# NVlabs/intrinsic3d

Hardware: AMD Instinct MI355X
Metric: Gauss-Newton iterations/s at the finest SDF level (higher is better)
Workload: dtype f32

## Files before the change

intrinsic3d_amd/csrc/device/build.hip:

```cpp
#include <type_traits>
#include "kernels.hpp"
#include "reduce_device.hpp"

namespace i3d {

typedef float v4f_row __attribute__((ext_vector_type(4)));
typedef float v2f_row __attribute__((ext_vector_type(2)));
typedef float f2 __attribute__((ext_vector_type(2)));
static __device__ inline void st_row2(float2* p, float a, float b) { v2f_row v; v.x = a; v.y = b; __builtin_nontemporal_store(v, reinterpret_cast<v2f_row*>(p)); }
static __device__ inline void st_row(float4* p, float a, float b, float c, float d) { v4f_row v; v.x = a; v.y = b; v.z = c; v.w = d; __builtin_nontemporal_store(v, reinterpret_cast<v4f_row*>(p)); }

typedef float f4u __attribute__((ext_vector_type(4), aligned(4)));
typedef const __attribute__((address_space(1))) f4u* gf4u_ptr;
typedef const __attribute__((address_space(1))) float* gf_ptr;

constexpr int Q_LDS_STRIDE = 296;
struct PointShared {
    double P[3];
    double B;
    float n[3];
    float inv_len;
    float s;
    float Ls;
    float dLs[3];
// ... 399 lines not shown
#endif
                float jr[9];
#pragma unroll
                for (int i = 0; i < 9; ++i) jr[i] = fc.Jr[i];
                if (!FR_LDS) __builtin_amdgcn_sched_barrier(0);
                float J[P_TOTAL];
#pragma unroll
                for (int i = 0; i < P_TOTAL; ++i) J[i] = 0.0f;
                float Wx = 0.0f, Wy = 0.0f, Wz = 0.0f;
                const float R0 = (float)Rl[0], R1 = (float)Rl[1], R2 = (float)Rl[2], R3 = (float)Rl[3], R4 = (float)Rl[4], R5 = (float)Rl[5], R6 = (float)Rl[6], R7 = (float)Rl[7], R8 = (float)Rl[8];
#pragma unroll
                for (int jp = 0; jp < 4; jp += 2) {
                    const int ja = jp, jb = jp + 1;
                    const f2 x0 = {pv[ja].x0, pv[jb].x0}, y0 = {pv[ja].y0, pv[jb].y0}, iz = {pv[ja].iz, pv[jb].iz};
                    const f2 dfdc = {pv[ja].dfdc, pv[jb].dfdc}, dfdr = {pv[ja].dfdr, pv[jb].dfdr};
                    const f2 r2 = x0 * x0 + y0 * y0, r4 = r2 * r2, r6 = r4 * r2;
                    const f2 dc = 1.0f + k0 * r2 + k1 * r4 + k2 * r6;
                    const f2 dcr = k0 + 2.0f * k1 * r2 + 3.0f * k2 * r4;
                    const f2 xd = x0 * dc + 2.0f * k3 * x0 * y0 + k4 * (r2 + 2.0f * x0 * x0);
                    const f2 yd = y0 * dc + 2.0f * k4 * xd * y0 + k3 * (r2 + 2.0f * y0 * y0);
                    const f2 dxd_dx0 = dc + 2.0f * x0 * x0 * dcr + 2.0f * k3 * y0 + 6.0f * k4 * x0;
                    const f2 dxd_dy0 = 2.0f * x0 * y0 * dcr + 2.0f * k3 * x0 + 2.0f * k4 * y0;
                    const f2 dyd_dx0 = 2.0f * x0 * y0 * dcr + 2.0f * k4 * y0 * dxd_dx0 + 2.0f * k3 * x0;
                    const f2 dyd_dy0 = dc + 2.0f * y0 * y0 * dcr + 2.0f * k4 * (xd + y0 * dxd_dy0) + 6.0f * k3 * y0;
                    const f2 au = dfdc * fxs, av = dfdr * fys;
                    const f2 lx = au * dxd_dx0 + av * dyd_dx0, ly = au * dxd_dy0 + av * dyd_dy0;
                    const f2 L0 = lx * iz, L1 = ly * iz, L2 = -(lx * x0 + ly * y0) * iz;
                    const f2 M0 = L0 * R0 + L1 * R3 + L2 * R6, M1 = L0 * R1 + L1 * R4 + L2 * R7, M2 = L0 * R2 + L1 * R5 + L2 * R8;
                    const f2 c = {cj[ja], cj[jb]};
                    const f2 alb = {q[ja].alb, q[jb].alb}, sv = {q[ja].s, q[jb].s}, il = {q[ja].inv_len, q[jb].inv_len};
                    const f2 n0 = {q[ja].n[0], q[jb].n[0]}, n1 = {q[ja].n[1], q[jb].n[1]}, n2 = {q[ja].n[2], q[jb].n[2]};
                    const f2 v0 = alb * f2{q[ja].dLs[0], q[jb].dLs[0]} + sv * M0, v1 = alb * f2{q[ja].dLs[1], q[jb].dLs[1]} + sv * M1, v2 = alb * f2{q[ja].dLs[2], q[jb].dLs[2]} + sv * M2;
                    const f2 d = n0 * v0 + n1 * v1 + n2 * v2;
                    f2 G0 = (v0 - n0 * d) * il, G1 = (v1 - n1 * d) * il, G2 = (v2 - n2 * d) * il;
                    if (il.x == 0.0f) { G0.x = v0.x; G1.x = v1.x; G2.x = v2.x; }
                    if (il.y == 0.0f) { G0.y = v0.y; G1.y = v1.y; G2.y = v2.y; }
                    const f2 direct = M0 * n0 + M1 * n1 + M2 * n2;
                    const f2 cG0 = c * G0, cG1 = c * G1, cG2 = c * G2, cD = c * (direct - (G0 + G1 + G2)), cLs = c * f2{q[ja].Ls, q[jb].Ls};
                    J[PS[ja][1]] += cG0.x; J[PS[ja][2]] += cG1.x; J[PS[ja][3]] += cG2.x; J[PS[ja][0]] += cD.x; J[P_ALB + ja] = cLs.x;
                    J[PS[jb][1]] += cG0.y; J[PS[jb][2]] += cG1.y; J[PS[jb][3]] += cG2.y; J[PS[jb][0]] += cD.y; J[P_ALB + jb] = cLs.y;
                    const f2 cL0 = c * L0, cL1 = c * L1, cL2 = c * L2;
                    J[P_POSE + 3] -= cL0.x + cL0.y; J[P_POSE + 4] -= cL1.x + cL1.y; J[P_POSE + 5] -= cL2.x + cL2.y;
                    const f2 Px = {(float)q[ja].P[0], (float)q[jb].P[0]}, Py = {(float)q[ja].P[1], (float)q[jb].P[1]}, Pz = {(float)q[ja].P[2], (float)q[jb].P[2]};
                    const f2 wx = c * (Py * M2 - Pz * M1), wy = c * (Pz * M0 - Px * M2), wz = c * (Px * M1 - Py * M0);
                    Wx += wx.x + wx.y; Wy += wy.x + wy.y; Wz += wz.x + wz.y;
                    const f2 cdc = c * dfdc * psf, cdr = c * dfdr * psf;
                    const f2 i0 = cdc * xd, i1 = cdr * yd;
                    J[P_INTR + 0] -= i0.x + i0.y; J[P_INTR + 1] -= i1.x + i1.y; J[P_INTR + 2] -= cdc.x + cdc.y; J[P_INTR + 3] -= cdr.x + cdr.y;
                    const f2 dxk0 = x0 * r2, dxk1 = x0 * r4, dxk2 = x0 * r6, dxk3 = 2.0f * x0 * y0, dxk4 = r2 + 2.0f * x0 * x0;
                    const f2 c2 = 2.0f * k4 * y0;
                    const f2 e0 = c * (au * dxk0 + av * (y0 * r2 + c2 * dxk0)), e1 = c * (au * dxk1 + av * (y0 * r4 + c2 * dxk1)), e2 = c * (au * dxk2 + av * (y0 * r6 + c2 * dxk2));
                    const f2 e3 = c * (au * dxk3 + av * (c2 * dxk3 + (r2 + 2.0f * y0 * y0))), e4 = c * (au * dxk4 + av * (2.0f * xd * y0 + c2 * dxk4));
                    J[P_DIST + 0] -= e0.x + e0.y; J[P_DIST + 1] -= e1.x + e1.y; J[P_DIST + 2] -= e2.x + e2.y; J[P_DIST + 3] -= e3.x + e3.y; J[P_DIST + 4] -= e4.x + e4.y;
                }
                J[P_POSE + 0] = -(Wx * jr[0] + Wy * jr[3] + Wz * jr[6]);
                J[P_POSE + 1] = -(Wx * jr[1] + Wy * jr[4] + Wz * jr[7]);
                J[P_POSE + 2] = -(Wx * jr[2] + Wy * jr[5] + Wz * jr[8]);
                float finz = 0.0f;
#pragma unroll
                for (int i = 0; i < P_TOTAL; ++i) finz = __builtin_fmaf(J[i], 0.0f, finz);
                if (!(finz == 0.0f)) continue;
#pragma unroll
                for (int gq = 0; gq < 7; ++gq)
                    st_row(&r.rows[row_index(a, nout, gq, r.slots)], J[4 * gq], J[4 * gq + 1], J[4 * gq + 2], J[4 * gq + 3]);
                const size_t ro = row_scalar_index(a, nout, r.slots);
                st_row2(&r.row_jt()[row_jt_index(a, nout, r.slots)], J[28], __int_as_float(f | (vox_free ? ROW_FREE_BIT : 0)));
                st_row2(&r.row_wr[ro], roww, (float)res);
                ++nout;
            }
            }
        }
        if (WITH_J) {
            r.nrows[a] = (uint8_t)nout;
        }
        }
    }
#ifdef I3D_COST_MULTI_PROBE
    if (!WITH_J && probe_extra) cost = 0.0;
#endif
    if (!WITH_J) block_partial_d(cost, cost_out, 1, 0);
}

void launch_build(hipStream_t st, GridView g, RowView r, OptParams p, const FrameConst* frames, bool with_jacobian, double* cost_out, double* scratch,
                  const double* cam9, const LmState* lm) {
    if (r.nC <= 0) { if (!with_jacobian && cost_out) (void)hipMemsetAsync(cost_out, 0, sizeof(double), st); return; }
#ifdef I3D_COST_MULTI_PROBE
    const int blocks = with_jacobian ? (r.nC + 255) / 256 : (((r.nC + 255) / 256 + 7) / 8) * 8 * I3D_COST_MULTI_PROBE;
#else
    const int blocks = (r.nC + 255) / 256;
#endif
    double* const cost_dst = cost_out; cost_out = scratch;
    const size_t lds = (size_t)p.K * sizeof(FrameHot), qlds = (size_t)256 * Q_LDS_STRIDE;
    if (with_jacobian) {
#ifdef I3D_BUILD_VALUE_PROBE
        if (BUILD_PROBE_WAVES > 2) {
            if (!set_dynamic_lds((const void*)k_build<true, true, 2>, "k_build<true> value probe", lds, p.K)) return;
            k_build<true, true, 2><<<blocks, 256, lds, st>>>(g, r, p, frames, cost_out, nullptr, nullptr);
            return;
        }
#endif
        if (!set_dynamic_lds((const void*)k_build<true, false, 2>, "k_build<true>", qlds, p.K)) return;
        k_build<true, false, 2><<<blocks, 256, qlds, st>>>(g, r, p, frames, cost_out, nullptr, nullptr);
    } else {
        if (lds <= 48 * 1024) k_build<false, true, 2><<<blocks, 256, lds, st>>>(g, r, p, frames, cost_out, cam9, lm);
        else k_build<false, false, 2><<<blocks, 256, 0, st>>>(g, r, p, frames, cost_out, cam9, lm);
    }
    if (!with_jacobian) launch_reduce_partials(st, scratch, blocks, 1, cost_dst, nullptr, true);
}

template <bool COST>
__global__ void __launch_bounds__(256) k_weight_sums(RowView r, GridView g, double* partials) {
    double s0 = 0, s1 = 0, s2 = 0, s3 = 0, n0 = 0, n3 = 0, na = 0, c0 = 0, c1 = 0, c2 = 0, c3 = 0;
    const int N = g.N;
    for (int a = r.own0 + blockIdx.x * blockDim.x + threadIdx.x; a < r.own1 && a < r.A; a += gridDim.x * blockDim.x) {
        if (!(r.aflags[a] & F_ACTIVE)) continue;
        na += 1.0;
        const int nr = r.nrows[a];
        for (int k = 0; k < nr; ++k) {
            const float2 wr = r.row_wr[row_scalar_index(a, k, r.slots)]; const float w = wr.x;
            s0 += (double)w; if (w != 0.0f) n0 += 1.0;
            if (COST && (__float_as_int(r.row_jt()[row_jt_index(a, k, r.slots)].y) & ROW_FREE_BIT)) c0 += (double)w * ((double)wr.y * (double)wr.y);
        }
        const uint8_t rf = r.regflags[a];
        if (rf & 1) s1 += 1.0;
        if (rf & 2) s2 += 1.0;
        const int s = COST ? r.alist[a] : 0;
        const uint8_t eafree = COST ? r.ea_free[a] : 0;
        const bool er = COST && (rf & 1) && (rf & 8), es = COST && (rf & 2) && (rf & 16);
        int ring[6];
        if (er || eafree) {
#pragma unroll
            for (int d = 0; d < 6; ++d) ring[d] = g.nbr[(size_t)d * N + s];
        }
        if (er || es) {
            const double xs = g.x_sdf[s];
            if (er) {
                const double dxx = g.x_sdf[ring[0]] + g.x_sdf[ring[1]] - 2.0 * xs, dyy = g.x_sdf[ring[2]] + g.x_sdf[ring[3]] - 2.0 * xs, dzz = g.x_sdf[ring[4]] + g.x_sdf[ring[5]] - 2.0 * xs;
                const double lap = dxx + dyy + dzz; c1 += lap * lap;
            }
            if (es) { double e = xs - g.sdf0[s]; if (e == 0.0) e = 0.0000001; c2 += e * e; }
        }
        const double xa = eafree ? g.x_alb[s] : 0.0;
#pragma unroll
        for (int d = 0; d < 6; ++d) {
            const float w = r.ea_w[(size_t)d * r.Acap + a]; s3 += (double)w; if (w != 0.0f) n3 += 1.0;
            if (eafree & (1 << d)) { const double e = xa - g.x_alb[ring[d]]; c3 += (double)w * (e * e); }
        }
    }
    block_partial_d(s0, partials, 13, 0); block_partial_d(s1, partials, 13, 1); block_partial_d(s2, partials, 13, 2); block_partial_d(s3, partials, 13, 3);
    block_partial_d(n0, partials, 13, 4); block_partial_d(0.0, partials, 13, 5); block_partial_d(0.0, partials, 13, 6); block_partial_d(n3, partials, 13, 7);
    block_partial_d(na, partials, 13, 8);
    block_partial_d(c0, partials, 13, 9); block_partial_d(c1, partials, 13, 10); block_partial_d(c2, partials, 13, 11); block_partial_d(c3, partials, 13, 12);
}
void launch_weight_sums(hipStream_t st, RowView r, GridView g, bool with_cost, double* sums13, double* scratch) {
    const int n = r.own1 - r.own0;
    if (n <= 0) return;
    int blocks = (n + 255) / 256; if (blocks > 1024) blocks = 1024;
    if (with_cost) k_weight_sums<true><<<blocks, 256, 0, st>>>(r, g, scratch);
    else k_weight_sums<false><<<blocks, 256, 0, st>>>(r, g, scratch);
    launch_reduce_partials(st, scratch, blocks, 13, sums13, nullptr);
}

}
```

intrinsic3d_amd/csrc/device/gradcol.hip:

```cpp
#include "kernels.hpp"
#include "reduce_device.hpp"
#include "wave_ops.hpp"

namespace i3d {

constexpr int GC_THREADS = 384, GC_NW = GC_THREADS / 64, GC_TC = 16, GC_NPV = 27, GC_NCAM = 34;
constexpr int GC_D_CAMW = 4, GC_D_TAG = GC_D_CAMW + ((GC_NW * (GC_NCAM + 0) + 3) & ~3), GC_D_VAL = GC_D_TAG + GC_NW * GC_TC, GC_D0 = GC_D_VAL + GC_NW * GC_TC * GC_NPV;

__device__ constexpr int8_t GC_TRI_I[21] = {0, 0, 0, 0, 0, 0, 1, 1, 1, 1, 1, 2, 2, 2, 2, 3, 3, 3, 4, 4, 5};
__device__ constexpr int8_t GC_TRI_J[21] = {0, 1, 2, 3, 4, 5, 1, 2, 3, 4, 5, 2, 3, 4, 5, 3, 4, 5, 4, 5, 5};

#ifndef GC_OCC
#define GC_OCC 2
#endif
__global__ void __launch_bounds__(GC_THREADS, GC_OCC) k_eg_gradcol(GridView g, RowView r, OptParams p, GradColBuffers b, int tiles_per_block) {
    extern __shared__ float lds[];
    const int K = p.K; const size_t Acap = r.Acap;
    const int rs = (GC_NPV * K) | 1;
    const int nacc = GC_D0 + rs + GC_NCAM;
    for (int i = threadIdx.x; i < nacc; i += GC_THREADS) lds[i] = (i >= GC_D_TAG && i < GC_D_VAL) ? __int_as_float(-1) : 0.0f;
    __syncthreads();
    const int wave = __builtin_amdgcn_readfirstlane((int)(threadIdx.x >> 6));
    const int o_tag = GC_D_TAG + wave * GC_TC, o_val = GC_D_VAL + wave * (GC_TC * GC_NPV);
    int tcount = 0;
// ... 71 lines not shown
            wave_table_add_quads<GC_NPV, GC_TC, 3>(live && owned, fsel, [&](int q) {
                return q < 6 ? (free_poses ? J[P_POSE + (q < 6 ? q : 0)] * t : 0.0f) : tw0 * J[P_POSE + GC_TRI_I[q < 6 ? 0 : q - 6]] * J[P_POSE + GC_TRI_J[q < 6 ? 0 : q - 6]];
            }, lds, o_tag, o_val, tcount, GC_D0, GC_NPV);
        }
        __syncthreads();
        for (int w = 0; w < GC_NW; ++w) { if (wave == w) wave_table_merge<GC_NPV, GC_TC>(lds, o_tag, o_val, tcount, GC_D0, GC_NPV); __syncthreads(); }
        if (in) {
#pragma unroll
            for (int c = 0; c < P_VOX; ++c) { b.Cg[(size_t)c * Acap + a] = accg[c]; b.Cc[(size_t)c * Acap + a] = accc[c]; }
            const int s = r.alist[a];
            const int N = g.N;
            const bool act = (fl & F_ACTIVE) != 0;
            const uint8_t rf_ld = r.regflags[a], eaf_ld = r.ea_free[a];
            float eaw[6]; int rg[6];
#pragma unroll
            for (int d = 0; d < 6; ++d) { eaw[d] = r.ea_w[(size_t)d * Acap + a]; rg[d] = g.nbr[(size_t)d * N + s]; }
            const double xs = g.x_sdf[s], xa = g.x_alb[s], s0 = g.sdf0[s];
            double xsn[6], xan[6];
#pragma unroll
            for (int d = 0; d < 6; ++d) { const int nb = rg[d] >= 0 ? rg[d] : s; xsn[d] = g.x_sdf[nb]; xan[d] = g.x_alb[nb]; }
            const uint8_t rf = act ? rf_ld : 0;
            float trg = 0.0f, tsg = 0.0f, trc = 0.0f, tsc = 0.0f;
            const uint8_t eafree = (owned && act) ? eaf_ld : 0;
            if (rf & 1) {
                const float rho = (float)p.type_w[1];
                const double dxx = xsn[0] + xsn[1] - 2.0 * xs, dyy = xsn[2] + xsn[3] - 2.0 * xs, dzz = xsn[4] + xsn[5] - 2.0 * xs;
                const double lap = dxx + dyy + dzz;
                trg = rho * (float)lap; trc = rho;
                if (owned && (rf & 8)) cost += 0.5 * p.type_w[1] * lap * lap;
            }
            if (rf & 2) {
                const double e0 = xs - s0;
                if (rf & 4) { const float rho = (float)p.type_w[2]; tsg = rho * (float)e0; tsc = rho; }
                if (owned && (rf & 16)) { const double e = e0 == 0.0 ? 0.0000001 : e0; cost += 0.5 * p.type_w[2] * e * e; }
            }
            b.tregg[a] = trg; b.tregg[Acap + a] = tsg; b.tregc[a] = trc; b.tregc[Acap + a] = tsc;
#pragma unroll
            for (int d = 0; d < 6; ++d) {
                const float w = act ? eaw[d] : 0.0f;
                float tag = 0.0f, tac = 0.0f;
                if (w != 0.0f) {
                    const float rho = w * (float)p.type_w[3]; const double e = xa - xan[d];
                    tag = rho * (float)e; tac = rho;
                    if (eafree & (1 << d)) cost += 0.5 * (double)w * p.type_w[3] * e * e;
                }
                b.tregg[(size_t)(2 + d) * Acap + a] = tag; b.tregc[(size_t)(2 + d) * Acap + a] = tac;
            }
        }
    }
    block_partial_d(cost, b.cost_partials, 1, 0);
#pragma unroll
    for (int i = 0; i < GC_NCAM; ++i) {
        float v = i < 9 ? cam9[i] : camb[i - 9];
        for (int o = 32; o > 0; o >>= 1) v += __shfl_down(v, o, 64);
        if ((threadIdx.x & 63) == 0) lds[GC_D_CAMW + wave * GC_NCAM + i] = v;
    }
    __syncthreads();
    if (threadIdx.x < GC_NCAM) { float v = 0.0f; for (int w = 0; w < GC_NW; ++w) v += lds[GC_D_CAMW + w * GC_NCAM + threadIdx.x]; cam_acc[threadIdx.x] = v; }
    __syncthreads();
    float* const rowg = b.part + (size_t)blockIdx.x * b.part_stride;
    float* const rowc = rowg + b.col_off;
    for (int i = threadIdx.x; i < 6 * K; i += GC_THREADS) { const int f = i / 6; rowg[i] = lds[GC_D0 + GC_NPV * f + (i - 6 * f)]; }
    for (int i = threadIdx.x; i < 21 * K; i += GC_THREADS) { const int f = i / 21; rowc[i] = lds[GC_D0 + GC_NPV * f + 6 + (i - 21 * f)]; }
    if (threadIdx.x < 9) rowg[6 * K + threadIdx.x] = cam_acc[threadIdx.x];
    if (threadIdx.x < 34) {
        const int i = threadIdx.x;
        constexpr int8_t DIAG[9] = {0, 4, 7, 9, 10, 15, 19, 22, 24};
        rowc[21 * K + i] = i < 9 ? cam_acc[9 + DIAG[i]] : cam_acc[i];
    }
}

int launch_eg_gradcol(hipStream_t st, GridView g, RowView r, OptParams p, GradColBuffers b) {
    if (r.nC <= 0) return 0;
    static int num_cu = 0;
    if (!num_cu) { int dev = 0; (void)hipGetDevice(&dev); hipDeviceProp_t pr; (void)hipGetDeviceProperties(&pr, dev); num_cu = pr.multiProcessorCount > 0 ? pr.multiProcessorCount : 256; }
    const int ntiles = (r.nC + GC_THREADS - 1) / GC_THREADS;
    const int want = 2 * num_cu;
    const int blocks = ntiles < want ? ntiles : want;
    const int tiles_per_block = (ntiles + blocks - 1) / blocks;
    const size_t n = (size_t)(GC_D0 + ((GC_NPV * p.K) | 1) + GC_NCAM) * sizeof(float);
    if (!set_dynamic_lds((const void*)k_eg_gradcol, "k_eg_gradcol", n, p.K)) return 0;
    const int used = (ntiles + tiles_per_block - 1) / tiles_per_block;
    k_eg_gradcol<<<used, GC_THREADS, n, st>>>(g, r, p, b, tiles_per_block);
    launch_reduce_partials(st, b.cost_partials, used, 1, b.cost_out, nullptr);
    return used;
}

}
```

intrinsic3d_amd/csrc/device/kernels.hpp:

```cpp
#pragma once
#include "common.hpp"
#include "p2p_device.hpp"

namespace i3d {

struct HashTable { unsigned long long* keys; int* vals; unsigned int mask; };
void launch_sort_keys(hipStream_t st, int N, const int* keys_xyz , unsigned long long* sort_keys, int* iota);
void launch_permute_grid(hipStream_t st, int N, const int* perm, const int* keys_xyz, const double* sdf, const double* sdf_ref,
                         const double* alb, const float* w, const uint8_t* rgb,
                         int* cx, int* cy, int* cz, int* rank, double* sdf0, double* x_sdf, double* x_alb, float* f_sdf, float* f_alb,
                         float* weight, uchar4* color);
void launch_hash_build(hipStream_t st, int N, const int* cx, const int* cy, const int* cz, HashTable t);
void launch_nbr_build(hipStream_t st, int N, const int* cx, const int* cy, const int* cz, HashTable t, int* nbr);
void launch_classify(hipStream_t st, GridView g, OptParams p, int* active_flag);
void launch_compact(hipStream_t st, int N, const int* active_flag, const int* active_scan, const uint8_t* flags, int* aidx, int* alist, uint8_t* aflags);
void launch_partition_blocks(hipStream_t st, GridView g, int A, int* alist, uint8_t* aflags, int* aidx);
void launch_group_rows(hipStream_t st, int A, const uint8_t* nrows, int* gmax);
void launch_anbr(hipStream_t st, int N, int A, int Acap, const int* alist, const int* nbr, const int* aidx, int* anbr);
void launch_scatter_sh(hipStream_t st, int N, const int* rank, const double* sh_visit , float* sh );
void launch_gather_visit(hipStream_t st, int N, const int* rank, const double* x_sdf, const double* x_alb, double* out_sdf, double* out_alb);
void launch_update_fields(hipStream_t st, int N, const int* rank, const double* sdf_ref, const double* alb, const uint8_t* rgb,
                          double* x_sdf, double* x_alb, float* f_sdf, float* f_alb, uchar4* color);

void launch_observe(hipStream_t st, GridView g, RowView r, OptParams p, const FrameConst* frames, const unsigned* cull_mask = nullptr, bool prefilter = false);
constexpr int CULL_BLOCK = 8, CULL_MAX_LEVELS = 12;
struct CullPyramid { int levels, cells; int bw[CULL_MAX_LEVELS], bh[CULL_MAX_LEVELS], off[CULL_MAX_LEVELS]; };
CullPyramid cull_pyramid(int w, int h);
void launch_depth_blocks(hipStream_t st, const FrameConst* frames, int K, int w, int h, float2* out);
void launch_group_cull(hipStream_t st, GridView g, RowView r, OptParams p, const FrameConst* frames, const float2* dblocks, float4* bounds, unsigned* mask);

void launch_build(hipStream_t st, GridView g, RowView r, OptParams p, const FrameConst* frames, bool with_jacobian, double* cost_out , double* scratch,
                  const double* cam9 = nullptr, const LmState* lm = nullptr);
void launch_weight_sums(hipStream_t st, RowView r, GridView g, bool with_cost, double* sums13 , double* scratch);

enum PassMode { PASS_GRAD = 0, PASS_JTJP = 1, PASS_COLNORM = 2 };
struct Seg2 { size_t off0, off1; int n; };
struct PassBuffers {
    float* C;
    float* treg;
    double* shared;
    double* blocks;
    float* part; int part_stride;
};
struct GradColBuffers {
    float* Cg; float* Cc;
    float* tregg; float* tregc;
    float* part; int part_stride;
    int col_off;
    double* cost_partials; double* cost_out;
};
int  launch_eg_gradcol(hipStream_t st, GridView g, RowView r, OptParams p, GradColBuffers b);
int  launch_eg_pass(hipStream_t st, PassMode mode, GridView g, RowView r, OptParams p, const float* u , PassBuffers b, const PcgState* state);
void launch_sum_rows(hipStream_t st, PassMode mode, int K, const float* part, int nrows, int stride, double* shared, double* blocks);
void launch_gather(hipStream_t st, PassMode mode, RowView r, PassBuffers b, float* out );
int  launch_gather_tail(hipStream_t st, RowView r, PassBuffers b, float* out, const float* S, const float* D2, const float* v, double* dot_partials ,
                        bool dot_atomic, const PcgState* state);
void launch_reduce_partials(hipStream_t st, const double* partials, int nblk, int ncomp, double* dst, const PcgState* state, bool assign = false);
void launch_shared_finalize(hipStream_t st, size_t tail_off, int K, OptParams p, const double* shared, float* out , bool tail, const float* S, const float* D2,
                            const float* v, double* dot_out, const PcgState* state);

void launch_fill(hipStream_t st, int n, float* x, float v);
void launch_fill_d(hipStream_t st, int n, double* x, double v);
void launch_int_to_double(hipStream_t st, const int* src, double* dst);
void launch_mul(hipStream_t st, int n, const float* a, const float* b, float* out);
void launch_scale_from_colnorm(hipStream_t st, int n, const float* c, const float* freemask, float* S, float* cm);
void launch_dot(hipStream_t st, int n, const float* a, const float* b, double* out , double* scratch);
void launch_count_above2(hipStream_t st, Seg2 sg, const float* a, const float* m, float tol, double* out, double* scratch);
void launch_count_above(hipStream_t st, int n, const float* a, const float* m, float tol, double* out, double* scratch);
void launch_dot2(hipStream_t st, Seg2 sg, const float* a, const float* b, double* out , double* scratch);
void launch_mul2(hipStream_t st, Seg2 sg, const float* a, const float* b, float* out);
void launch_freemask(hipStream_t st, RowView r, OptParams p, float* mask );

void launch_pcg_init(hipStream_t st, PcgState* state, int fixed_iterations, int max_iterations, const LmState* lm = nullptr);
int  launch_pcg_step(hipStream_t st, int mode, Seg2 sg, const float* p, const float* q, float* x, float* r, const float* b, const float* D2, const float* Minv,
                     float* z, const float* S_for_inline_q, double* partials , PcgState* state);
void launch_pcg_tail_x(hipStream_t st, size_t tail_off, int K, const float* p, float* x, const PcgState* state);
void launch_pcg_tail_a(hipStream_t st, int mode, size_t tail_off, int K, const float* Minv_blocks, const float* p, const float* q, float* x, float* r, const float* b,
                       const float* D2, float* z, const double* partials, int nblk, PcgState* state,
                       double* shared_zero, int nzero, int* host_flags, int seq,
                       const P2PDev& pd);
int  launch_pcg_direction(hipStream_t st, Seg2 sg, size_t tail_off, int ntail, const float* z, float* p, const float* S, float* u, const float* D2,
                          double* d2_partials , const PcgState* state);
void launch_pcg_tail_b(hipStream_t st, size_t tail_off, int K, OptParams p, double* shared, const double* pq_slice, const double* pq_partials, int nblk,
                       const double* pq_partials2, int nblk2, bool rowwise,
                       float* q, const float* S, const float* D2, const float* v, PcgState* state, const P2PDev& pd);
struct TilePlan {
    unsigned* lnbr;
    float* eaw_sym;
    int* halo_idx; int* halo_cnt;
    int* iota; int* ext_e; int* ext_pos;
    float* qh;
    int* ext_off;
    int* overflow;
    int T, hmax;
    int tile_first, ntiles_own;
    const int* ghost_tiles; int n_ghost;
    int det;
    const unsigned short* hp_off;
    const unsigned short* hp_src;
    int pull;
};
inline int tile_plan_pull_cap(int hmax) { return 4 * hmax; }
inline int tile_plan_hmax_of(int T) { return T == 1024 ? 2048 : 1536; }
inline int tile_plan_tiles_of(int A, int T) { return (A + T - 1) / T; }
size_t tile_plan_temp_bytes(size_t nslots);
hipError_t launch_tile_plan(hipStream_t st, RowView r, TilePlan t, int hmax_limit , void* temp, size_t temp_bytes);
void launch_eaw_sym(hipStream_t st, RowView r, TilePlan t, const int* cflag );
int  launch_eg_tile(hipStream_t st, RowView r, OptParams p, const float* u, TilePlan t, double* shared, float* qacc, double* pq_partials ,
                    const PcgState* state, float* cam_partials = nullptr, int cam_stride = 0);
void launch_ext_offsets(hipStream_t st, int n, const int* ext_e, int A, int* ext_off);
void eg_tile_launch_shape(const TilePlan& t, int K, int& blocks, int& tiles_per_block);

struct LadVec;
int  eg_tile_mr_max_systems(int K);
int  launch_eg_tile_mr(hipStream_t st, RowView r, OptParams p, TilePlan t, int nsys, const int* sys, const float* u0, float* qacc0, float* qh0, double* pq0 , float* cam0, int cam_stride,
                       const PcgState* st0 , const LadVec& lv);
int  launch_eg_tile_mr_pair(hipStream_t st, RowView r, OptParams p, TilePlan t, int na, int nb, const int* sys, const float* u0, float* qacc0, float* qh0, double* pq0 , float* cam0,
                            int cam_stride, const PcgState* st0, const LadVec& lv);

struct ShardArgs {
    P2PDev pd; RimLists rim; int seq;
    int n_slice_partials;
    int n_rim_wg;
    const float* zb; float* pb; float* ub; const float* cmb; int chunk;
};
struct LadVec {
    size_t vec;
    size_t qh;
    size_t cam;
    size_t part;
    size_t mblk;
    size_t tail;
    int sysid[LADDER_MAX];
};
struct Step3Args {
    int nq; int chunk4;
    const float4* p; const float4* qacc; float4* x; float4* r; const float4* b; float4* z;
    const float4* cm; const LmState* lm;
    const int* ext_off; const int* ext_pos; const float2* qh; int e0;
    const double* pq_partials; int n_pq; const double* d2_partials; int n_d2;
    int n_slice_wg;
    int K; int fix_poses, fix_intr, fix_dist;
    const float* cam_partials; int n_cam; int cam_stride; const float* Mblk;
    const float* tp; float* tx; float* tr; const float* tb; const float* tD2; float* tz; const float* tS;
    double* step_partials;
    PcgState* cur;
    int sharded; ShardArgs sh;
    int lad_sys;
    const double* redop; int redop_stride;
};
void launch_pcg_init3(hipStream_t st, PcgState* st2 , int fixed_iterations, int max_iterations, const LmState* lm = nullptr);
int  launch_pcg_dir3(hipStream_t st, bool init, Seg2 sg, size_t tail_off, int ntail, const float* z, float* p, const float* S, float* u, const float* D2, const float* cm, const LmState* lm,
                     const double* step_partials, int n_step, double* d2_partials, const PcgState* prev, PcgState* next, int* host_flags, int seq,
                     const ShardArgs* sa = nullptr);
void launch_rim_u(hipStream_t st, const ShardArgs& sa, const PcgState* state);
int  pcg_step3_slice_wgs(int n_entries, int cap = 0);
int  pcg_step3_tail_wgs(int K);
int  launch_pcg_step3(hipStream_t st, int mode , Step3Args a);
void launch_halo_fold(hipStream_t st, RowView r, TilePlan t, float* qacc, const PcgState* state);
void launch_pcg_init_lad(hipStream_t st, PcgState* st2_all , int B, int fixed_iterations, int max_iterations, const LmState* lm);
int  launch_pcg_dir3_lad(hipStream_t st, bool init, int nsys, Seg2 sg, size_t tail_off, int ntail, const float* z0, float* p0, const float* S, float* u0, const float* tD2_0, const float* cm, const LmState* lm,
                         const double* step_partials0, int n_step, double* d2_partials0, PcgState* st2_0, int prev_parity, int* host_flags0, int seq, const LadVec& lv,
                         int n_slice_partials = 0, const double* red4_0 = nullptr );
int  launch_pcg_step3_lad(hipStream_t st, int mode, int nsys, Step3Args a, const LadVec& lv);
void launch_lad_reduce_step(hipStream_t st, int nsys, const double* step_partials0, int n_slice, double* red4_0, const LadVec& lv);
void launch_lad_reduce_op(hipStream_t st, int nsys, const float* cam_partials0, int n_cam, int cam_stride, int NS, const double* pq_partials0, int n_pq, const double* d2_partials0, int n_d2,
                          double* redop0, int redop_stride, const LadVec& lv);

void launch_need_mask(hipStream_t st, RowView r, int slice, unsigned long long* need );
void launch_halo_items(hipStream_t st, int A, int slice, int me, const unsigned long long* need, unsigned long long* items, int* count , int cap);
void launch_tile_flags(hipStream_t st, int A, int T, const int* cflag, int* tileflag );
size_t halo_sort_temp_bytes(int cap);
hipError_t launch_halo_sort(hipStream_t st, void* temp, size_t temp_bytes, const unsigned long long* in, unsigned long long* out, int n);

void launch_candidate(hipStream_t st, GridView g, RowView r, int K, float sign, const float* step, const float* S, const double* x_shared, double* xc_sdf, double* xc_alb,
                      double* xc_shared, double* norms2 , const float* mask, double* scratch, const LmState* lm = nullptr);
void launch_accept(hipStream_t st, GridView g, RowView r, const double* xc_sdf, const double* xc_alb, const LmState* lm = nullptr);
void launch_set_double(hipStream_t st, double* dst, double v);
void launch_lm_init(hipStream_t st, LmState* lm, const double* cost, const double* ngrad, const double* nfree, double radius0, LmRecord* rec, int seq);
void launch_lm_begin(hipStream_t st, LmState* lm, int K, int fix_poses, int fix_intr, int fix_dist, const double* cdiag, const double* tri, float* Mblk,
                     const float* tc, const float* tS, float* tD2, float* tMinv, LmRecord* rec, int seq);
void launch_lm_diag_dev(hipStream_t st, int n, const float* c, const float* S, const LmState* lm, float* D2, float* Minv);
void launch_cand_frames(hipStream_t st, int K, const double* xc, const FrameConst* base, FrameConst* out, const LmState* lm);
void launch_lm_decide(hipStream_t st, LmState* lm, const PcgState* ps, const double* norms2, const double* cand_cost, int attempt, int lm_steps, LmRecord* rec, int seq,
                      int lad_next = -1 , int debug_invalid = 0);
void launch_lm_begin_lad(hipStream_t st, LmState* lm, int B, int K, int fix_poses, int fix_intr, int fix_dist, const double* cdiag, const double* tri, float* Mblk, size_t mblk_stride,
                         const float* tc, const float* tS, float* tD2, size_t tail_stride, LmRecord* rec, int seq);
void launch_mark_compute(hipStream_t st, RowView r, int* flag);
void launch_compact_list(hipStream_t st, int A, const int* flag, const int* scan, int* list);

}
```

intrinsic3d_amd/csrc/device/lm_kernels.hip:

```cpp
#include "kernels.hpp"
#include "frame_math.hpp"

namespace i3d {

static __device__ inline void lm_publish(LmRecord* rec, int seq) {
    if (rec) __hip_atomic_store(&rec->seq, seq, __ATOMIC_RELEASE, __HIP_MEMORY_SCOPE_SYSTEM);
}

__global__ void k_lm_init(LmState* lm, const double* __restrict__ cost, const double* __restrict__ ngrad, const double* __restrict__ nfree, double radius0, LmRecord* rec, int seq) {
    LmState s;
    s.cost = *cost; s.radius = radius0; s.decrease_factor = 2.0; s.ngrad = *ngrad; s.nfree = *nfree;
    s.inv_radius = (float)(1.0 / radius0); s.pad0 = 0;
    s.done = 0; s.termination = 0; s.accepted = 0; s.invalid = 0; s.attempts = 0; s.successful = 0;
    if (s.nfree == 0.0 || s.ngrad == 0.0) { s.done = 1; s.termination = 1; }
    *lm = s;
    if (rec) {
        rec->final_ = s.done; rec->accepted = 0; rec->pcg_it = 0; rec->termination = s.termination; rec->kind = 0;
        rec->cost = s.cost; rec->cand_cost = 0.0; rec->model_change = 0.0; rec->rel = 0.0; rec->radius_after = s.radius; rec->ngrad = s.ngrad; rec->nfree = s.nfree;
        lm_publish(rec, seq);
    }
}
__global__ void k_set_double(double* dst, double v) { *dst = v; }
void launch_set_double(hipStream_t st, double* dst, double v) { k_set_double<<<1, 1, 0, st>>>(dst, v); }
void launch_lm_init(hipStream_t st, LmState* lm, const double* cost, const double* ngrad, const double* nfree, double radius0, LmRecord* rec, int seq) {
    k_lm_init<<<1, 1, 0, st>>>(lm, cost, ngrad, nfree, radius0, rec, seq);
}

static __device__ inline bool spd_invert_dev(int n, const double* m, double* inv) {
    double L[36];
    for (int i = 0; i < n; ++i) for (int j = 0; j <= i; ++j) {
        double s = m[i * n + j];
        for (int k = 0; k < j; ++k) s -= L[i * n + k] * L[j * n + k];
        if (i == j) { if (!(s > 0.0)) return false; L[i * n + i] = sqrt(s); } else L[i * n + j] = s / L[j * n + j];
    }
    for (int col = 0; col < n; ++col) {
        double y[6], x[6];
        for (int i = 0; i < n; ++i) { double s = (i == col) ? 1.0 : 0.0; for (int k = 0; k < i; ++k) s -= L[i * n + k] * y[k]; y[i] = s / L[i * n + i]; }
        for (int i = n - 1; i >= 0; --i) { double s = y[i]; for (int k = i + 1; k < n; ++k) s -= L[k * n + i] * x[k]; x[i] = s / L[i * n + i]; }
        for (int i = 0; i < n; ++i) inv[i * n + col] = x[i];
    }
    return true;
}
static __device__ inline void cam_block_inverse(int n, const double* __restrict__ cdiag, const double* __restrict__ tri, bool fixed, double radius, float* __restrict__ out) {
    if (fixed) { for (int i = 0; i < n * n; ++i) out[i] = 0.0f; return; }
    double S[6], M[36], inv[36];
    for (int i = 0; i < n; ++i) S[i] = 1.0 / (1.0 + sqrt(cdiag[i]));
    int o = 0;
    for (int i = 0; i < n; ++i) for (int j = i; j < n; ++j) { const double v = S[i] * S[j] * tri[o++]; M[i * n + j] = v; M[j * n + i] = v; }
    for (int i = 0; i < n; ++i) { const double cs = cdiag[i] * S[i] * S[i]; M[i * n + i] += fmin(fmax(cs, 1e-6), 1e32) / radius; }
    if (!spd_invert_dev(n, M, inv)) { for (int i = 0; i < n * n; ++i) inv[i] = 0.0; for (int i = 0; i < n; ++i) inv[i * n + i] = 1.0 / M[i * n + i]; }
    for (int i = 0; i < n * n; ++i) out[i] = (float)inv[i];
}

__global__ void __launch_bounds__(64) k_lm_begin(LmState* lm, int K, int fix_poses, int fix_intr, int fix_dist, const double* __restrict__ cdiag , const double* __restrict__ tri ,
                                                 float* __restrict__ Mblk , const float* __restrict__ tc, const float* __restrict__ tS, float* __restrict__ tD2, float* __restrict__ tMinv ,
                                                 LmRecord* rec, int seq) {
    if (lm->done) return;
    const double radius = lm->radius;
    const int gid = blockIdx.x * blockDim.x + threadIdx.x;
    if (radius < 1e-32) {
        if (gid == 0) {
            lm->termination = 1; lm->done = 1;
            if (rec) { rec->final_ = 1; rec->accepted = 0; rec->pcg_it = 0; rec->termination = 1; rec->kind = 2; rec->cost = lm->cost; rec->cand_cost = 0.0; rec->model_change = 0.0; rec->rel = 0.0;
                       rec->radius_after = radius; rec->ngrad = lm->ngrad; rec->nfree = lm->nfree; lm_publish(rec, seq); }
        }
        return;
    }
    const float inv_radius = (float)(1.0 / radius);
    if (gid == 0) lm->inv_radius = inv_radius;
    if (gid < K) cam_block_inverse(6, cdiag + 6 * gid, tri + 21 * gid, fix_poses != 0, radius, Mblk + 36 * (size_t)gid);
    else if (gid == K) cam_block_inverse(4, cdiag + 6 * K, tri + 21 * K, fix_intr != 0, radius, Mblk + 36 * (size_t)K);
    else if (gid == K + 1) cam_block_inverse(5, cdiag + 6 * K + 4, tri + 21 * K + 10, fix_dist != 0, radius, Mblk + 36 * (size_t)K + 16);
    const int NS = 6 * K + 9;
    for (int i = gid; i < NS; i += gridDim.x * blockDim.x) { float d2, mi; lm_diag(tc[i], tS[i], inv_radius, d2, mi); tD2[i] = d2; tMinv[i] = mi; }
}
void launch_lm_begin(hipStream_t st, LmState* lm, int K, int fix_poses, int fix_intr, int fix_dist, const double* cdiag, const double* tri, float* Mblk,
                     const float* tc, const float* tS, float* tD2, float* tMinv, LmRecord* rec, int seq) {
    k_lm_begin<<<(K + 2 + 63) / 64, 64, 0, st>>>(lm, K, fix_poses, fix_intr, fix_dist, cdiag, tri, Mblk, tc, tS, tD2, tMinv, rec, seq);
}

__global__ void __launch_bounds__(64) k_lm_begin_lad(LmState* lm, int B, int K, int fix_poses, int fix_intr, int fix_dist, const double* __restrict__ cdiag, const double* __restrict__ tri,
                                                     float* __restrict__ Mblk, size_t mblk_stride, const float* __restrict__ tc, const float* __restrict__ tS, float* __restrict__ tD2, size_t tail_stride,
                                                     LmRecord* rec, int seq) {
    if (lm->done == 1) return;
    const int j = blockIdx.y, gid = blockIdx.x * blockDim.x + threadIdx.x;
    double radius = lm->radius, dec = lm->decrease_factor;
    if (j == 0 && radius < 1e-32) {
        if (gid == 0) {
            lm->termination = 1; lm->done = 1; lm->lad_n = 0;
            if (rec) { rec->final_ = 1; rec->accepted = 0; rec->pcg_it = 0; rec->termination = 1; rec->kind = 2; rec->cost = lm->cost; rec->cand_cost = 0.0; rec->model_change = 0.0; rec->rel = 0.0;
                       rec->radius_after = radius; rec->ngrad = lm->ngrad; rec->nfree = lm->nfree; lm_publish(rec, seq); }
        }
        return;
    }
    for (int s = 0; s < j; ++s) { radius = radius / dec; dec *= 2.0; }
    const bool dead = radius < 1e-32;
    const float inv_radius = dead ? 0.0f : (float)(1.0 / radius);
    if (gid == 0) { lm->lad_radius[j] = radius; lm->lad_inv_radius[j] = inv_radius; if (j == 0) { lm->lad_n = B; lm->inv_radius = inv_radius; lm->done = 0; } }
    if (dead) return;
    float* const Mb = Mblk + (size_t)j * mblk_stride;
    if (gid < K) cam_block_inverse(6, cdiag + 6 * gid, tri + 21 * gid, fix_poses != 0, radius, Mb + 36 * (size_t)gid);
    else if (gid == K) cam_block_inverse(4, cdiag + 6 * K, tri + 21 * K, fix_intr != 0, radius, Mb + 36 * (size_t)K);
    else if (gid == K + 1) cam_block_inverse(5, cdiag + 6 * K + 4, tri + 21 * K + 10, fix_dist != 0, radius, Mb + 36 * (size_t)K + 16);
    const int NS = 6 * K + 9;
    for (int i = gid; i < NS; i += gridDim.x * blockDim.x) { float d2, mi; lm_diag(tc[i], tS[i], inv_radius, d2, mi); tD2[(size_t)j * tail_stride + i] = d2; }
}
void launch_lm_begin_lad(hipStream_t st, LmState* lm, int B, int K, int fix_poses, int fix_intr, int fix_dist, const double* cdiag, const double* tri, float* Mblk, size_t mblk_stride,
                         const float* tc, const float* tS, float* tD2, size_t tail_stride, LmRecord* rec, int seq) {
    k_lm_begin_lad<<<dim3((K + 2 + 63) / 64, B), 64, 0, st>>>(lm, B, K, fix_poses, fix_intr, fix_dist, cdiag, tri, Mblk, mblk_stride, tc, tS, tD2, tail_stride, rec, seq);
}

__global__ void k_lm_diag_dev(int n, const float* __restrict__ c, const float* __restrict__ S, const LmState* __restrict__ lm, float* __restrict__ D2, float* __restrict__ Minv) {
    if (lm->done) return;
    const float ir = lm->inv_radius;
    for (int i = blockIdx.x * blockDim.x + threadIdx.x; i < n; i += gridDim.x * blockDim.x) { float d2, mi; lm_diag(c[i], S[i], ir, d2, mi); D2[i] = d2; Minv[i] = mi; }
}
void launch_lm_diag_dev(hipStream_t st, int n, const float* c, const float* S, const LmState* lm, float* D2, float* Minv) {
    if (n <= 0) return;
    int b = (n + 255) / 256; b = b > 2048 ? 2048 : b;
    k_lm_diag_dev<<<b, 256, 0, st>>>(n, c, S, lm, D2, Minv);
}

__global__ void __launch_bounds__(64) k_cand_frames(int K, const double* __restrict__ xc, const FrameConst* __restrict__ base, FrameConst* __restrict__ out, const LmState* __restrict__ lm) {
    if (lm->done) return;
    const int f = blockIdx.x * blockDim.x + threadIdx.x;
    if (f >= K) return;
    FrameConst fc = base[f];
    double p[6];
    for (int i = 0; i < 6; ++i) p[i] = xc[6 * f + i];
    fm::frame_from_pose(p, fc);
    out[f] = fc;
}
void launch_cand_frames(hipStream_t st, int K, const double* xc, const FrameConst* base, FrameConst* out, const LmState* lm) {
    if (K > 0) k_cand_frames<<<(K + 63) / 64, 64, 0, st>>>(K, xc, base, out, lm);
}

__global__ void k_lm_decide(LmState* lm, const PcgState* __restrict__ ps, const double* __restrict__ norms2, const double* __restrict__ cand_cost_p, int attempt , int lm_steps,
                            LmRecord* rec, int seq, int lad_next, int debug_invalid) {
    if (lm->done) return;
    const int pcg_it = ps->done == 2 ? ps->it + 1 : ps->it;
    const double xbr = ps->xbr, d2xx = ps->d2xx;
    const double model_change = 0.5 * xbr + 0.5 * d2xx;
    const bool finite = !(isnan(xbr) || isinf(xbr) || isnan(d2xx) || isinf(d2xx));
    double radius = lm->radius, decrease = lm->decrease_factor, cost = lm->cost;
    const double cand = *cand_cost_p;
    int final_ = 0, accepted = 0, termination = lm->termination, invalid = lm->invalid, successful = lm->successful;
    double rel = 0.0;
    if (!finite || !(model_change > 0.0) || debug_invalid) {
        if (++invalid >= 5) { termination = 3; final_ = 1; }
        else radius *= 0.5;
    } else {
        invalid = 0;
        const double step_norm = sqrt(norms2[0]), x_norm = sqrt(norms2[1]);
        const double cost_change = cost - cand;
        if (step_norm <= 1e-8 * (x_norm + 1e-8)) { termination = 1; final_ = 1; }
        else if (fabs(cost_change) <= 1e-6 * cost) { termination = 1; final_ = 1; }
        else {
            rel = cost_change / model_change;
            if (rel > 1e-3) {
                accepted = 1; cost = cand;
                radius = fmin(1e16, radius / fmax(1.0 / 3.0, 1.0 - pow(2.0 * rel - 1.0, 3.0)));
                decrease = 2.0;
                successful += 1; termination = 2; final_ = 1;
            } else { radius = radius / decrease; decrease *= 2.0; }
        }
    }
    if (!final_ && attempt + 1 >= lm_steps) final_ = 1;
    lm->radius = radius; lm->decrease_factor = decrease; lm->cost = cost; lm->invalid = invalid; lm->successful = successful; lm->termination = termination;
    lm->attempts = lm->attempts + 1; lm->accepted = accepted; lm->done = final_;
    if (rec) {
        rec->final_ = final_; rec->accepted = accepted; rec->pcg_it = pcg_it; rec->termination = termination; rec->kind = 1;
        rec->cost = cost; rec->cand_cost = cand; rec->model_change = model_change; rec->rel = rel; rec->radius_after = radius; rec->ngrad = lm->ngrad; rec->nfree = lm->nfree;
        lm_publish(rec, seq);
    }
    if (!final_ && lad_next >= 0 && lad_next < lm->lad_n) {
        LmRecord* const nrec = rec ? rec + 1 : nullptr;
        if (radius != lm->lad_radius[lad_next]) {
            lm->done = 2;
            if (nrec) { nrec->final_ = 0; nrec->accepted = 0; nrec->pcg_it = 0; nrec->termination = termination; nrec->kind = 3; nrec->cost = cost; nrec->cand_cost = 0.0; nrec->model_change = 0.0;
                        nrec->rel = 0.0; nrec->radius_after = radius; nrec->ngrad = lm->ngrad; nrec->nfree = lm->nfree; lm_publish(nrec, seq + 1); }
        } else if (radius < 1e-32) {
            lm->termination = 1; lm->done = 1;
            if (nrec) { nrec->final_ = 1; nrec->accepted = 0; nrec->pcg_it = 0; nrec->termination = 1; nrec->kind = 2; nrec->cost = cost; nrec->cand_cost = 0.0; nrec->model_change = 0.0;
                        nrec->rel = 0.0; nrec->radius_after = radius; nrec->ngrad = lm->ngrad; nrec->nfree = lm->nfree; lm_publish(nrec, seq + 1); }
        }
    }
}
void launch_lm_decide(hipStream_t st, LmState* lm, const PcgState* ps, const double* norms2, const double* cand_cost, int attempt, int lm_steps, LmRecord* rec, int seq, int lad_next, int debug_invalid) {
    k_lm_decide<<<1, 1, 0, st>>>(lm, ps, norms2, cand_cost, attempt, lm_steps, rec, seq, lad_next, debug_invalid);
}

}
```

intrinsic3d_amd/csrc/device/operator.hip:

```cpp
#include "kernels.hpp"
#include "reduce_device.hpp"
#include "wave_ops.hpp"

namespace i3d {

#define GRID_STRIDE(n) const int stride = gridDim.x * blockDim.x; for (int i = blockIdx.x * blockDim.x + threadIdx.x; i < (n); i += stride)
static inline int vblocks(int n) { int b = (n + 255) / 256; return b < 1 ? 1 : (b > 2048 ? 2048 : b); }

__global__ void __launch_bounds__(1024) k_reduce_partials(const double* __restrict__ partials, int nblk, int ncomp, double* dst, const PcgState* __restrict__ state, int assign) {
    if (state && state->done) return;
    for (int k = 0; k < ncomp; ++k) {
        double s = 0.0;
        for (int i0 = threadIdx.x; i0 < nblk; i0 += 8 * 1024) {
            double v[8];
#pragma unroll
            for (int q = 0; q < 8; ++q) v[q] = partials[(size_t)min(i0 + q * 1024, nblk - 1) * ncomp + k];
#pragma unroll
            for (int q = 0; q < 8; ++q) if (i0 + q * 1024 < nblk) s += v[q];
        }
        const double t = block_sum_d(s);
        if (threadIdx.x == 0) dst[k] = assign ? t : dst[k] + t;
    }
}
void launch_reduce_partials(hipStream_t st, const double* partials, int nblk, int ncomp, double* dst, const PcgState* state, bool assign) {
    if (nblk > 0) k_reduce_partials<<<1, 1024, 0, st>>>(partials, nblk, ncomp, dst, state, assign ? 1 : 0);
}

constexpr int EG_THREADS = 1024;

template <int MODE>
__global__ void __launch_bounds__(EG_THREADS) k_eg_pass(GridView g, RowView r, OptParams p, PassBuffers b, int tiles_per_block, const PcgState* __restrict__ state) {
    static_assert(MODE == PASS_GRAD || MODE == PASS_COLNORM, "the operator pass has its own kernel");
    if (state && state->done) return;
    extern __shared__ float lds[];
    const int K = p.K; const size_t Acap = r.Acap;
    constexpr int NPVT = (MODE == PASS_COLNORM) ? 21 : 6, TCT = (MODE == PASS_COLNORM) ? 16 : 32, NWT = EG_THREADS / 64;
    const int rs = ((MODE == PASS_COLNORM) ? 21 * K : 6 * K) | 1;
    constexpr int NCAM = (MODE == PASS_COLNORM) ? 34 : 9;
    constexpr int D_CAMW = 4, D_TAG = D_CAMW + ((NWT * NCAM + 3) & ~3), D_VAL = D_TAG + NWT * TCT, D0 = D_VAL + NWT * TCT * NPVT;
    const int nacc = D0 + rs + NCAM;
    for (int i = threadIdx.x; i < nacc; i += EG_THREADS) lds[i] = (i >= D_TAG && i < D_VAL) ? __int_as_float(-1) : 0.0f;
    __syncthreads();
    const int wave = __builtin_amdgcn_readfirstlane((int)(threadIdx.x >> 6));
    const int o_tag = D_TAG + wave * TCT, o_val = D_VAL + wave * (TCT * NPVT);
    int tcount = 0;
    float* const cam_acc = lds + D0 + rs;
    float cam9[9];
#pragma unroll
    for (int i = 0; i < 9; ++i) cam9[i] = 0.0f;
    float camb[NCAM];
#pragma unroll
    for (int i = 0; i < NCAM; ++i) camb[i] = 0.0f;
    const float tw0 = (float)p.type_w[0];
    const int nC = r.nC;
    const int ntiles = (nC + EG_THREADS - 1) / EG_THREADS;
    const int tile0 = blockIdx.x * tiles_per_block;

    for (int tile = tile0; tile < tile0 + tiles_per_block && tile < ntiles; ++tile) {
        const int ci = tile * EG_THREADS + threadIdx.x;
        const bool in = ci < nC;
        const int a = in ? (r.clist ? r.clist[ci] : ci) : 0;
        const bool owned = in && a >= r.own0 && a < r.own1;
        const uint8_t fl = in ? r.aflags[a] : 0;
        const int nr = (in && (fl & F_ACTIVE)) ? (int)r.nrows[a] : 0;
        int nr_max = nr;
        for (int o = 32; o > 0; o >>= 1) nr_max = max(nr_max, __shfl_xor(nr_max, o, 64));

        float acc[P_VOX];
#pragma unroll
        for (int c = 0; c < P_VOX; ++c) acc[c] = 0.0f;
        const size_t ac = in ? (size_t)a : 0;
        for (int k = 0; k < nr_max; ++k) {
            const float4* __restrict__ row = r.rows + row_index(ac, k, 0, r.slots);
            float4 j4[7];
#pragma unroll
            for (int q = 0; q < 7; ++q) j4[q] = ld_row(row + q * 64);
            const size_t ro = row_scalar_index(ac, k, r.slots);
            const float2 jt = r.row_jt()[row_jt_index(ac, k, r.slots)];
            constexpr int NPV = (MODE == PASS_COLNORM) ? 21 : 6;
            float pv[NPV]; int fsel = 0; bool pvalid = false;
#pragma unroll
            for (int i = 0; i < NPV; ++i) pv[i] = 0.0f;
            if (k < nr) {
                const float rho = tw0;
                const int f = __float_as_int(jt.y) & ~ROW_FREE_BIT;
                float J[P_TOTAL];
#pragma unroll
                for (int q = 0; q < 7; ++q) { J[4 * q] = j4[q].x; J[4 * q + 1] = j4[q].y; J[4 * q + 2] = j4[q].z; J[4 * q + 3] = j4[q].w; }
                J[28] = jt.x;
                if (MODE == PASS_COLNORM) {
#pragma unroll
                    for (int c = 0; c < P_VOX; ++c) acc[c] += rho * J[c] * J[c];
                  if (owned) {
                    int o = 0;
#pragma unroll
                    for (int i = 0; i < 6; ++i) {
#pragma unroll
                        for (int j = i; j < 6; ++j) { pv[o] = rho * J[P_POSE + i] * J[P_POSE + j]; ++o; }
                    }
                    fsel = f; pvalid = true;
#pragma unroll
                    for (int i = 0; i < 9; ++i) camb[i] += rho * J[P_INTR + i] * J[P_INTR + i];
                    o = 9;
#pragma unroll
                    for (int i = 0; i < 4; ++i) {
#pragma unroll
                        for (int j = i; j < 4; ++j) { camb[o] += rho * J[P_INTR + i] * J[P_INTR + j]; ++o; }
                    }
#pragma unroll
                    for (int i = 0; i < 5; ++i) {
#pragma unroll
                        for (int j = i; j < 5; ++j) { camb[o] += rho * J[P_DIST + i] * J[P_DIST + j]; ++o; }
                    }
                  }
                } else {
                    const float2 wr = r.row_wr[ro]; const float t = rho * (sqrtf(wr.x) * wr.y);
#pragma unroll
                    for (int c = 0; c < P_VOX; ++c) acc[c] += J[c] * t;
                    if (!p.fix_poses && owned) {
#pragma unroll
                        for (int i = 0; i < 6; ++i) pv[i] = J[P_POSE + i] * t;
                        fsel = f; pvalid = true;
                    }
                    if (owned) {
#pragma unroll
                        for (int i = 0; i < 9; ++i) cam9[i] += J[P_INTR + i] * t;
                    }
                }
            }
            wave_table_add_quads<NPV, TCT, (MODE == PASS_COLNORM ? 2 : 3)>(pvalid, fsel, [&](int q) { return pv[q]; }, lds, o_tag, o_val, tcount, D0, NPV);
        }
        __syncthreads();
        for (int w = 0; w < NWT; ++w) { if (wave == w) wave_table_merge<NPVT, TCT>(lds, o_tag, o_val, tcount, D0, NPVT); __syncthreads(); }
        if (in) {
#pragma unroll
            for (int c = 0; c < P_VOX; ++c) b.C[(size_t)c * Acap + a] = acc[c];
            const uint8_t rf = (fl & F_ACTIVE) ? r.regflags[a] : 0;
            float tr = 0.0f, ts = 0.0f;
            const int s = r.alist[a];
            const int N = g.N;
            if (rf & 1) {
                const float rho = (float)p.type_w[1];
                if (MODE == PASS_COLNORM) tr = rho;
                else {
                    const double xs = g.x_sdf[s];
                    double nbv[6];
#pragma unroll
                    for (int d = 0; d < 6; ++d) nbv[d] = g.x_sdf[g.nbr[(size_t)d * N + s]];
                    const double dxx = nbv[0] + nbv[1] - 2.0 * xs, dyy = nbv[2] + nbv[3] - 2.0 * xs, dzz = nbv[4] + nbv[5] - 2.0 * xs;
                    tr = rho * (float)(dxx + dyy + dzz);
                }
            }
            if ((rf & 2) && (rf & 4)) {
                const float rho = (float)p.type_w[2];
                if (MODE == PASS_COLNORM) ts = rho;
                else ts = rho * (float)(g.x_sdf[s] - g.sdf0[s]);
            }
            b.treg[a] = tr; b.treg[Acap + a] = ts;
#pragma unroll
            for (int d = 0; d < 6; ++d) {
                const float w = (fl & F_ACTIVE) ? r.ea_w[(size_t)d * Acap + a] : 0.0f;
                float ta = 0.0f;
                if (w != 0.0f) {
                    const float rho = w * (float)p.type_w[3];
                    if (MODE == PASS_COLNORM) ta = rho;
                    else ta = rho * (float)(g.x_alb[s] - g.x_alb[g.nbr[(size_t)d * N + s]]);
                }
                b.treg[(size_t)(2 + d) * Acap + a] = ta;
            }
        }
    }
#pragma unroll
    for (int i = 0; i < NCAM; ++i) {
        float v = (MODE == PASS_COLNORM) ? camb[i] : cam9[i];
        for (int o = 32; o > 0; o >>= 1) v += __shfl_down(v, o, 64);
        if ((threadIdx.x & 63) == 0) lds[D_CAMW + wave * NCAM + i] = v;
    }
    __syncthreads();
    if (threadIdx.x < NCAM) { float v = 0.0f; for (int w = 0; w < NWT; ++w) v += lds[D_CAMW + w * NCAM + threadIdx.x]; cam_acc[threadIdx.x] = v; }
    __syncthreads();
    const int npose = (MODE == PASS_COLNORM) ? 21 * K : 6 * K;
    float* const row = b.part + (size_t)blockIdx.x * b.part_stride;
    for (int i = threadIdx.x; i < npose + NCAM; i += EG_THREADS) row[i] = i < npose ? lds[D0 + i] : cam_acc[i - npose];
}

__global__ void __launch_bounds__(256) k_sum_rows(int mode, int K, const float* __restrict__ part, int nrows, int stride, double* __restrict__ shared, double* __restrict__ blocks) {
    __shared__ double grp[8][33];
    const int col = threadIdx.x & 31, rg = threadIdx.x >> 5;
    const int i = blockIdx.x * 32 + col;
    const int ncol = mode == PASS_COLNORM ? 21 * K + 34 : 6 * K + 9;
    double v = 0.0;
    if (i < ncol) for (int w = rg; w < nrows; w += 8) v += (double)part[(size_t)w * stride + i];
    grp[rg][col] = v;
    __syncthreads();
    if (rg != 0 || i >= ncol) return;
    v = grp[0][col];
    for (int q = 1; q < 8; ++q) v += grp[q][col];
    if (mode != PASS_COLNORM) { shared[i] = v; return; }
    if (i < 21 * K) {
        blocks[i] = v;
        const int f = i / 21, o = i - 21 * f;
        const int di = o == 0 ? 0 : o == 6 ? 1 : o == 11 ? 2 : o == 15 ? 3 : o == 18 ? 4 : o == 20 ? 5 : -1;
        if (di >= 0) shared[6 * f + di] = v;
    } else { const int c = i - 21 * K; if (c < 9) shared[6 * K + c] = v; else blocks[21 * K + (c - 9)] = v; }
}
void launch_sum_rows(hipStream_t st, PassMode mode, int K, const float* part, int nrows, int stride, double* shared, double* blocks) {
    const int ncol = mode == PASS_COLNORM ? 21 * K + 34 : 6 * K + 9;
    k_sum_rows<<<(ncol + 31) / 32, 256, 0, st>>>((int)mode, K, part, nrows, stride, shared, blocks);
}

__global__ void __launch_bounds__(EG_THREADS) k_eg_jtjp(GridView g, RowView r, OptParams p, const float* __restrict__ u, PassBuffers b,
                                                        int reps, int tiles_per_block, const PcgState* __restrict__ state) {
    if (state && state->done) return;
    extern __shared__ float lds[];
    const int K = p.K; const size_t Acap = r.Acap;
    const int nshared = 6 * K + 9;
    const int rs = (6 * K) | 1;
    const int nacc = reps * rs + 9;
    for (int i = threadIdx.x; i < nacc; i += EG_THREADS) lds[i] = 0.0f;
    float* const upose = lds + nacc;
    float* const uvl = upose + nshared + threadIdx.x;
    const size_t tail = 2 * (size_t)r.chunk;
    const int chunk = r.chunk;
    for (int i = threadIdx.x; i < nshared; i += EG_THREADS) upose[i] = u[tail + i];
    __syncthreads();
    float* const cam_acc = lds + reps * rs;
    float* const pose_acc = lds + (threadIdx.x & (reps - 1)) * rs;
    float* const wave_acc = lds + ((threadIdx.x >> 6) & (reps - 1)) * rs;
    float cam9[9];
#pragma unroll
    for (int i = 0; i < 9; ++i) cam9[i] = 0.0f;
    const float tw0 = (float)p.type_w[0];
    const int nC = r.nC;
    const int ntiles = (nC + EG_THREADS - 1) / EG_THREADS;
    const int tile0 = blockIdx.x * tiles_per_block;
    const float* const ui = upose + 6 * K;

    for (int tile = tile0; tile < tile0 + tiles_per_block && tile < ntiles; ++tile) {
        const int ci = tile * EG_THREADS + threadIdx.x;
        const bool in = ci < nC;
        const int a = in ? (r.clist ? r.clist[ci] : ci) : 0;
        const bool owned = in && a >= r.own0 && a < r.own1;
        const uint8_t fl = in ? r.aflags[a] : 0;
        const int nr = (in && (fl & F_ACTIVE)) ? (int)r.nrows[a] : 0;
        int nr_max = nr;
        for (int o = 32; o > 0; o >>= 1) nr_max = max(nr_max, __shfl_xor(nr_max, o, 64));
        const size_t ac = in ? (size_t)a : 0;
        float4 rwA[8], rwB[8];
        auto load_block = [&](float4 (&rw)[8], int k) {
            const float4* __restrict__ row = r.rows + row_index(ac, k, 0, r.slots);
#pragma unroll
            for (int q = 0; q < 7; ++q) rw[q] = ld_row(row + q * 64);
            { const float2 jt = r.row_jt()[row_jt_index(ac, k, r.slots)]; rw[7].x = jt.x; rw[7].y = jt.y; }
        };
        if (nr_max > 0) load_block(rwA, 0);
        if (in) {
#pragma unroll
            for (int c = 0; c < P_VOX; ++c) {
                const int nb = slot_fwd_nbr(c);
                const int la = nb < 0 ? a : r.anbr[(size_t)nb * Acap + a];
                uvl[c * EG_THREADS] = la >= 0 ? u[c < 10 ? vec_sdf(la, chunk) : vec_alb(la, chunk)] : 0.0f;
            }
        }
        if (nr_max > 1) load_block(rwB, 1);
        if (in) {
            const uint8_t rf = (fl & F_ACTIVE) ? r.regflags[a] : 0;
            const float us = uvl[0], ua = uvl[10 * EG_THREADS];
            float rs_[6], ra_[6];
            rs_[0] = uvl[6 * EG_THREADS]; rs_[2] = uvl[1 * EG_THREADS]; rs_[4] = uvl[4 * EG_THREADS];
            ra_[0] = uvl[11 * EG_THREADS]; ra_[2] = uvl[12 * EG_THREADS]; ra_[4] = uvl[13 * EG_THREADS];
#pragma unroll
            for (int q = 1; q < 6; q += 2) {
                const int la = (rf || (fl & F_ACTIVE)) ? r.anbr[(size_t)q * Acap + a] : -1;
                rs_[q] = la >= 0 ? u[vec_sdf(la, chunk)] : 0.0f; ra_[q] = la >= 0 ? u[vec_alb(la, chunk)] : 0.0f;
            }
            float tr = 0.0f, ts = 0.0f;
            if (rf & 1) tr = (float)p.type_w[1] * (((((((-6.0f * us) + rs_[0]) + rs_[1]) + rs_[2]) + rs_[3]) + rs_[4]) + rs_[5]);
            if ((rf & 2) && (rf & 4)) ts = (float)p.type_w[2] * us;
            b.treg[a] = tr; b.treg[Acap + a] = ts;
#pragma unroll
            for (int d = 0; d < 6; ++d) {
                const float w = (fl & F_ACTIVE) ? r.ea_w[(size_t)d * Acap + a] : 0.0f;
                b.treg[(size_t)(2 + d) * Acap + a] = (w != 0.0f) ? w * (float)p.type_w[3] * (ua - ra_[d]) : 0.0f;
            }
        }
        float acc[P_VOX];
#pragma unroll
        for (int c = 0; c < P_VOX; ++c) acc[c] = 0.0f;

        auto consume = [&](const float4 (&rw)[8], int k) {
            float pv[6]; int fsel = 0; bool pvalid = false;
// ... 138 lines not shown
                for (int d = 0; d < 6; ++d) if (ringa[d] >= 0) acc += SQUARED ? tn[d] : -tn[d];
                oalb = acc;
            }
        }
        const int js = vec_sdf(a, r.chunk), ja = js + r.chunk;
        if (TAIL) {
            const float v0 = v[js], v1 = v[ja];
            osdf = S[js] * osdf + D2[js] * v0; oalb = S[ja] * oalb + D2[ja] * v1;
            dotp = (double)v0 * (double)osdf + (double)v1 * (double)oalb;
        }
        out[js] = osdf; out[ja] = oalb;
    }
    if (TAIL && dot_out) {
        if (!dot_atomic) block_partial_d(dotp, dot_out, 1, 0);
        else { const double t = block_sum_d(dotp); if (threadIdx.x == 0 && t != 0.0) atomicAdd(dot_out, t); }
    }
}
void launch_gather(hipStream_t st, PassMode mode, RowView r, PassBuffers b, float* out) {
    const int n = (r.own1 < r.A ? r.own1 : r.A) - r.own0;
    if (n <= 0) return;
    const int blocks = (n + 255) / 256;
    if (mode == PASS_COLNORM) k_gather<true, false><<<blocks, 256, 0, st>>>(r, b, out, nullptr, nullptr, nullptr, nullptr, 0, nullptr);
    else k_gather<false, false><<<blocks, 256, 0, st>>>(r, b, out, nullptr, nullptr, nullptr, nullptr, 0, nullptr);
}
int launch_gather_tail(hipStream_t st, RowView r, PassBuffers b, float* out, const float* S, const float* D2, const float* v, double* dot_partials, bool dot_atomic,
                       const PcgState* state) {
    const int n = (r.own1 < r.A ? r.own1 : r.A) - r.own0;
    if (n <= 0) return 0;
    const int blocks = (n + 255) / 256;
    k_gather<false, true><<<blocks, 256, 0, st>>>(r, b, out, S, D2, v, dot_partials, dot_atomic ? 1 : 0, state);
    return blocks;
}

__global__ void k_shared_finalize(size_t tail_off, int K, OptParams p, const double* __restrict__ shared, float* __restrict__ out, int tail,
                                  const float* __restrict__ S, const float* __restrict__ D2, const float* __restrict__ v, double* dot_out,
                                  const PcgState* __restrict__ state) {
    if (state && state->done) return;
    const int i = blockIdx.x * blockDim.x + threadIdx.x;
    double dotp = 0.0;
    if (i < 6 * K + 9) {
        const bool fixed = i < 6 * K ? p.fix_poses : (i < 6 * K + 4 ? p.fix_intr : p.fix_dist);
        float o = fixed ? 0.0f : (float)shared[i];
        const size_t j = tail_off + i;
        if (tail) { const float vv = v[j]; o = S[j] * o + D2[j] * vv; dotp = (double)vv * (double)o; }
        out[j] = o;
    }
    if (tail && dot_out) { const double t = block_sum_d(dotp); if (threadIdx.x == 0 && t != 0.0) atomicAdd(dot_out, t); }
}
void launch_shared_finalize(hipStream_t st, size_t tail_off, int K, OptParams p, const double* shared, float* out, bool tail, const float* S, const float* D2,
                            const float* v, double* dot_out, const PcgState* state) {
    k_shared_finalize<<<(6 * K + 9 + 255) / 256, 256, 0, st>>>(tail_off, K, p, shared, out, tail ? 1 : 0, S, D2, v, dot_out, state);
}

__global__ void k_fill(int n, float* x, float v) { GRID_STRIDE(n) x[i] = v; }
__global__ void k_fill_d(int n, double* x, double v) { GRID_STRIDE(n) x[i] = v; }
__global__ void k_mul(int n, const float* a, const float* b, float* o) { GRID_STRIDE(n) o[i] = a[i] * b[i]; }
__global__ void k_mul2(int n, size_t seg, const float* a, const float* b, float* o) { GRID_STRIDE(2 * n) { const size_t j = i < n ? (size_t)i : (size_t)(i - n) + seg; o[j] = a[j] * b[j]; } }
__global__ void k_scale(int n, const float* c, const float* m, float* S, float* cm) { GRID_STRIDE(n) { const float v = m[i] != 0.0f ? c[i] : -1.0f; cm[i] = v; S[i] = lm_scale(v); } }
__global__ void __launch_bounds__(256) k_dot(int n, const float* a, const float* b, double* out) {
    double s = 0.0; GRID_STRIDE(n) s += (double)a[i] * (double)b[i];
    block_partial_d(s, out, 1, 0);
}
__global__ void __launch_bounds__(256) k_dot2(int n, size_t seg, const float* a, const float* b, double* out) {
    double s = 0.0; GRID_STRIDE(2 * n) { const size_t j = i < n ? (size_t)i : (size_t)(i - n) + seg; s += (double)a[j] * (double)b[j]; }
    block_partial_d(s, out, 1, 0);
}
__global__ void __launch_bounds__(256) k_count_above(int n, const float* a, const float* m, float tol, double* out) {
    double s = 0.0; GRID_STRIDE(n) s += (fabsf(a[i] * m[i]) > tol) ? 1.0 : 0.0;
    block_partial_d(s, out, 1, 0);
}
__global__ void __launch_bounds__(256) k_count_above2(int n, size_t seg, const float* a, const float* m, float tol, double* out) {
    double s = 0.0; GRID_STRIDE(2 * n) { const size_t j = i < n ? (size_t)i : (size_t)(i - n) + seg; s += (fabsf(a[j] * m[j]) > tol) ? 1.0 : 0.0; }
    block_partial_d(s, out, 1, 0);
}
void launch_fill(hipStream_t st, int n, float* x, float v) { if (n > 0) k_fill<<<vblocks(n), 256, 0, st>>>(n, x, v); }
void launch_fill_d(hipStream_t st, int n, double* x, double v) { if (n > 0) k_fill_d<<<vblocks(n), 256, 0, st>>>(n, x, v); }
__global__ void k_int_to_double(const int* src, double* dst) { *dst = (double)*src; }
void launch_int_to_double(hipStream_t st, const int* src, double* dst) { k_int_to_double<<<1, 1, 0, st>>>(src, dst); }
void launch_mul(hipStream_t st, int n, const float* a, const float* b, float* o) { if (n > 0) k_mul<<<vblocks(n), 256, 0, st>>>(n, a, b, o); }
void launch_mul2(hipStream_t st, Seg2 sg, const float* a, const float* b, float* o) {
    if (sg.n > 0) k_mul2<<<vblocks(2 * sg.n), 256, 0, st>>>(sg.n, sg.off1 - sg.off0, a + sg.off0, b + sg.off0, o + sg.off0);
}
void launch_scale_from_colnorm(hipStream_t st, int n, const float* c, const float* m, float* S, float* cm) { if (n > 0) k_scale<<<vblocks(n), 256, 0, st>>>(n, c, m, S, cm); }
void launch_dot2(hipStream_t st, Seg2 sg, const float* a, const float* b, double* out, double* scratch) {
    if (sg.n <= 0) return;
    const int blocks = vblocks(2 * sg.n) > 1024 ? 1024 : vblocks(2 * sg.n);
    k_dot2<<<blocks, 256, 0, st>>>(sg.n, sg.off1 - sg.off0, a + sg.off0, b + sg.off0, scratch);
    launch_reduce_partials(st, scratch, blocks, 1, out, nullptr);
}
void launch_count_above2(hipStream_t st, Seg2 sg, const float* a, const float* m, float tol, double* out, double* scratch) {
    if (sg.n <= 0) return;
    const int blocks = vblocks(2 * sg.n) > 1024 ? 1024 : vblocks(2 * sg.n);
    k_count_above2<<<blocks, 256, 0, st>>>(sg.n, sg.off1 - sg.off0, a + sg.off0, m + sg.off0, tol, scratch);
    launch_reduce_partials(st, scratch, blocks, 1, out, nullptr);
}
void launch_count_above(hipStream_t st, int n, const float* a, const float* m, float tol, double* out, double* scratch) {
    if (n <= 0) return;
    const int blocks = vblocks(n) > 1024 ? 1024 : vblocks(n);
    k_count_above<<<blocks, 256, 0, st>>>(n, a, m, tol, scratch);
    launch_reduce_partials(st, scratch, blocks, 1, out, nullptr);
}
void launch_dot(hipStream_t st, int n, const float* a, const float* b, double* out, double* scratch) {
    if (n <= 0) return;
    const int blocks = vblocks(n) > 1024 ? 1024 : vblocks(n);
    k_dot<<<blocks, 256, 0, st>>>(n, a, b, scratch);
    launch_reduce_partials(st, scratch, blocks, 1, out, nullptr);
}

__global__ void k_freemask(RowView r, OptParams p, float* __restrict__ mask) {
    const int A = r.A, chunk = r.chunk, nv = 2 * chunk, NP = nv + 6 * p.K + 9;
    GRID_STRIDE(NP) {
        float m;
        if (i < nv) {
            const int a = i < chunk ? i : i - chunk;
            m = (a < A && (r.aflags[a] & (i < chunk ? F_FREE_SDF : F_FREE_ALB))) ? 1.0f : 0.0f;
        }
        else if (i < nv + 6 * p.K) m = p.fix_poses ? 0.0f : 1.0f;
        else if (i < nv + 6 * p.K + 4) m = p.fix_intr ? 0.0f : 1.0f;
        else m = p.fix_dist ? 0.0f : 1.0f;
        mask[i] = m;
    }
}
void launch_freemask(hipStream_t st, RowView r, OptParams p, float* mask) { k_freemask<<<vblocks(2 * r.chunk + 6 * p.K + 9), 256, 0, st>>>(r, p, mask); }

enum { STEP_INIT = 0, STEP_NORMAL = 1, STEP_XONLY = 2, STEP_RESET = 3 };

template <int MODE, bool QINLINE>
__global__ void __launch_bounds__(256) k_pcg_step(int n4, int seg4 , const float4* __restrict__ p, const float4* __restrict__ q, float4* __restrict__ x, float4* __restrict__ r,
                                                  const float4* __restrict__ b, const float4* __restrict__ D2, const float4* __restrict__ Minv, float4* __restrict__ z,
                                                  const float4* __restrict__ S, double* __restrict__ partials , PcgState* state) {
    if (state->done) return;
    const float alpha = (float)state->alpha;
    double s0 = 0.0, s1 = 0.0, s2 = 0.0, s3 = 0.0;
    for (int j = blockIdx.x * blockDim.x + threadIdx.x; j < 2 * n4; j += gridDim.x * blockDim.x) {
        const int i = j < n4 ? j : j - n4 + seg4;
        float xv[4], rv[4];
        if (MODE == STEP_INIT) { const float4 t = r[i]; rv[0] = t.x; rv[1] = t.y; rv[2] = t.z; rv[3] = t.w; }
        else {
            const float4 xo = x[i];
            xv[0] = xo.x; xv[1] = xo.y; xv[2] = xo.z; xv[3] = xo.w;
            if (MODE != STEP_RESET) {
                const float4 pp = p[i];
                xv[0] += alpha * pp.x; xv[1] += alpha * pp.y; xv[2] += alpha * pp.z; xv[3] += alpha * pp.w;
                x[i] = make_float4(xv[0], xv[1], xv[2], xv[3]);
            }
            if (MODE == STEP_XONLY) continue;
            float4 qq = q[i];
            const float4 bb = b[i], dd = D2[i];
            if (QINLINE) {
                const float4 sv = S[i];
                if (MODE == STEP_NORMAL) { const float4 pp = p[i]; qq = make_float4(sv.x * qq.x + dd.x * pp.x, sv.y * qq.y + dd.y * pp.y, sv.z * qq.z + dd.z * pp.z, sv.w * qq.w + dd.w * pp.w); }
                else qq = make_float4(sv.x * qq.x + dd.x * xv[0], sv.y * qq.y + dd.y * xv[1], sv.z * qq.z + dd.z * xv[2], sv.w * qq.w + dd.w * xv[3]);
            }
            if (MODE == STEP_NORMAL) { const float4 ro = r[i]; rv[0] = ro.x - alpha * qq.x; rv[1] = ro.y - alpha * qq.y; rv[2] = ro.z - alpha * qq.z; rv[3] = ro.w - alpha * qq.w; }
            if (MODE == STEP_RESET) { rv[0] = bb.x - qq.x; rv[1] = bb.y - qq.y; rv[2] = bb.z - qq.z; rv[3] = bb.w - qq.w; }
            r[i] = make_float4(rv[0], rv[1], rv[2], rv[3]);
            const float bv[4] = {bb.x, bb.y, bb.z, bb.w}, dv[4] = {dd.x, dd.y, dd.z, dd.w};
#pragma unroll
            for (int k = 0; k < 4; ++k) { const double xd = xv[k]; s1 += xd * ((double)bv[k] + (double)rv[k]); s2 += xd * (double)rv[k]; s3 += (double)dv[k] * xd * xd; }
        }
        const float4 mm = Minv[i];
        const float zv[4] = {mm.x * rv[0], mm.y * rv[1], mm.z * rv[2], mm.w * rv[3]};
        z[i] = make_float4(zv[0], zv[1], zv[2], zv[3]);
#pragma unroll
        for (int k = 0; k < 4; ++k) s0 += (double)rv[k] * (double)zv[k];
    }
    if (MODE == STEP_XONLY) return;
    block_partial_d(s0, partials, 4, 0); block_partial_d(s1, partials, 4, 1); block_partial_d(s2, partials, 4, 2); block_partial_d(s3, partials, 4, 3);
}

__global__ void k_pcg_tail_x(size_t to, int NS, const float* __restrict__ p, float* __restrict__ x, const PcgState* __restrict__ state) {
    if (state->done) return;
    const float alpha = (float)state->alpha;
    for (int i = threadIdx.x; i < NS; i += blockDim.x) x[to + i] += alpha * p[to + i];
}

__global__ void __launch_bounds__(1024) k_pcg_tail_a(int mode, size_t to, int K, const float* __restrict__ Mblk, const float* __restrict__ p, const float* __restrict__ q,
// ... 134 lines not shown
    for (int o = 32; o > 0; o >>= 1) dotp += __shfl_down(dotp, o, 64);
    if ((threadIdx.x & 63) == 0) red[threadIdx.x >> 6] = dotp;
    __syncthreads();
    if (threadIdx.x != 0) return;
    double pq = *pq_slice; for (int w = 0; w < (int)(blockDim.x >> 6); ++w) pq += red[w];
    st->pq = pq;
    if (!(pq > 0.0) || isinf(pq)) { st->done = 2; return; }
    const double alpha = st->rho / pq;
    if (isinf(alpha)) { st->done = 2; return; }
    st->alpha = alpha;
}

__global__ void k_pcg_init(PcgState* st, int fixed_iterations, int max_iterations, const LmState* lm) {
    const bool over = lm && lm->done;
    for (int k = 0; k < 4; ++k) st->acc[k] = 0.0;
    st->rho = 0.0; st->last_rho = 1.0; st->pq = 0.0; st->alpha = 0.0; st->beta = 0.0; st->xbr = 0.0; st->xr = 0.0; st->d2xx = 0.0;
    st->Q0 = 0.0; st->Q1 = 0.0; st->it = 0; st->done = (fixed_iterations == 0 || over) ? 1 : 0; st->fixed_iterations = fixed_iterations; st->max_iterations = max_iterations;
}

void launch_pcg_init(hipStream_t st, PcgState* state, int fixed_iterations, int max_iterations, const LmState* lm) { k_pcg_init<<<1, 1, 0, st>>>(state, fixed_iterations, max_iterations, lm); }
static inline int step_blocks(int n4) { int b = (n4 + 255) / 256; return b < 1 ? 1 : (b > 2048 ? 2048 : b); }
int launch_pcg_step(hipStream_t st, int mode, Seg2 sg, const float* p, const float* q, float* x, float* r, const float* b, const float* D2, const float* Minv,
                    float* z, const float* S_for_inline_q, double* partials, PcgState* state) {
    if (sg.n <= 0) return 0;
    const int n4 = sg.n >> 2, seg4 = (int)((sg.off1 - sg.off0) >> 2);
    const size_t off = sg.off0;
    auto c4 = [off](const float* v) { return reinterpret_cast<const float4*>(v ? v + off : nullptr); };
    auto m4 = [off](float* v) { return reinterpret_cast<float4*>(v + off); };
    const float* S = S_for_inline_q;
    const int blocks = step_blocks(2 * n4);
#define I3D_STEP(MODE, QI) k_pcg_step<MODE, QI><<<blocks, 256, 0, st>>>(n4, seg4, c4(p), c4(q), m4(x), m4(r), c4(b), c4(D2), c4(Minv), m4(z), c4(S), partials, state)
    switch (mode) {
        case STEP_INIT:   I3D_STEP(STEP_INIT, false); break;
        case STEP_NORMAL: if (S) I3D_STEP(STEP_NORMAL, true); else I3D_STEP(STEP_NORMAL, false); break;
        case STEP_XONLY:  I3D_STEP(STEP_XONLY, false); break;
        default:          if (S) I3D_STEP(STEP_RESET, true); else I3D_STEP(STEP_RESET, false); break;
    }
#undef I3D_STEP
    return mode == STEP_XONLY ? 0 : blocks;
}
void launch_pcg_tail_x(hipStream_t st, size_t tail_off, int K, const float* p, float* x, const PcgState* state) { k_pcg_tail_x<<<1, 256, 0, st>>>(tail_off, 6 * K + 9, p, x, state); }
void launch_pcg_tail_a(hipStream_t st, int mode, size_t tail_off, int K, const float* Minv_blocks, const float* p, const float* q, float* x, float* r, const float* b,
                       const float* D2, float* z, const double* partials, int nblk, PcgState* state, double* shared_zero, int nzero, int* host_flags, int seq, const P2PDev& pd) {
    k_pcg_tail_a<<<1, 1024, 0, st>>>(mode, tail_off, K, Minv_blocks, p, q, x, r, b, D2, z, partials, nblk, state, shared_zero, nzero, host_flags, seq, pd);
}
int launch_pcg_direction(hipStream_t st, Seg2 sg, size_t tail_off, int ntail, const float* z, float* p, const float* S, float* u, const float* D2, double* d2_partials,
                         const PcgState* state) {
    if (sg.n <= 0 && ntail <= 0) return 0;
    const int n4 = sg.n >> 2, seg4 = (int)((sg.off1 - sg.off0) >> 2);
    const int blocks = step_blocks(2 * n4 > 0 ? 2 * n4 : 1);
    const size_t o = sg.off0;
    k_pcg_direction<<<blocks, 256, 0, st>>>(n4, seg4, tail_off - o, ntail, z + o, p + o, S + o, u + o, D2 + o, d2_partials, state);
    return d2_partials ? blocks : 0;
}
void launch_pcg_tail_b(hipStream_t st, size_t tail_off, int K, OptParams p, double* shared, const double* pq_slice, const double* pq_partials, int nblk,
                       const double* pq_partials2, int nblk2, bool rowwise, float* q, const float* S, const float* D2, const float* v, PcgState* state, const P2PDev& pd) {
    k_pcg_tail_b<<<1, 1024, 0, st>>>(tail_off, K, p, shared, pq_slice, pq_partials, nblk, pq_partials2, nblk2, rowwise ? 1 : 0, q, S, D2, v, state, pd);
}

__global__ void __launch_bounds__(256) k_candidate(GridView g, RowView r, int K, float sign, const float* __restrict__ step, const float* __restrict__ S,
                                                   const double* __restrict__ xsh, double* xc_sdf, double* xc_alb, double* xc_sh,
                                                   double* norms2, const float* __restrict__ mask, const LmState* __restrict__ lm) {
    if (lm && lm->done) return;
    const int A = r.A, NS = 6 * K + 9, chunk = r.chunk;
    const size_t tail = 2 * (size_t)chunk;
    double d2 = 0.0, x2 = 0.0;
    GRID_STRIDE(A + NS) {
        if (i < A) {
            const int s = r.alist[i]; const int js = vec_sdf(i, chunk), ja = js + chunk;
            const double ds = (double)sign * (double)step[js] * (double)S[js], da = (double)sign * (double)step[ja] * (double)S[ja];
            const double xs = g.x_sdf[s], xa = g.x_alb[s];
            xc_sdf[s] = xs + ds; xc_alb[s] = xa + da;
            if (mask[js] != 0.0f) { d2 += ds * ds; x2 += xs * xs; }
            if (mask[ja] != 0.0f) { d2 += da * da; x2 += xa * xa; }
        } else {
            const int t = i - A; const size_t j = tail + t;
            const double delta = (double)sign * (double)step[j] * (double)S[j];
            const double x = xsh[t]; xc_sh[t] = x + delta;
            if (mask[j] != 0.0f) { d2 += delta * delta; x2 += x * x; }
        }
    }
    block_partial_d(d2, norms2, 2, 0); block_partial_d(x2, norms2, 2, 1);
}
void launch_candidate(hipStream_t st, GridView g, RowView r, int K, float sign, const float* step, const float* S, const double* xsh, double* xc_sdf, double* xc_alb,
                      double* xc_sh, double* norms2, const float* mask, double* scratch, const LmState* lm) {
    int b = vblocks(r.A + 6 * K + 9); if (b > 1024) b = 1024;
    k_candidate<<<b, 256, 0, st>>>(g, r, K, sign, step, S, xsh, xc_sdf, xc_alb, xc_sh, scratch, mask, lm);
    launch_reduce_partials(st, scratch, b, 2, norms2, nullptr, true);
}
__global__ void k_accept(GridView g, RowView r, const double* __restrict__ xc_sdf, const double* __restrict__ xc_alb, const LmState* __restrict__ lm) {
    if (lm && !lm->accepted) return;
    GRID_STRIDE(r.A) { const int s = r.alist[i]; const double a = xc_sdf[s], b = xc_alb[s]; g.x_sdf[s] = a; g.x_alb[s] = b; g.f_sdf[s] = (float)a; g.f_alb[s] = (float)b; }
}
void launch_accept(hipStream_t st, GridView g, RowView r, const double* xc_sdf, const double* xc_alb, const LmState* lm) { if (r.A > 0) k_accept<<<vblocks(r.A), 256, 0, st>>>(g, r, xc_sdf, xc_alb, lm); }

__global__ void k_halo_pack(int n, const int* __restrict__ idx, const float* __restrict__ vec, int chunk, float* __restrict__ buf) {
    const int i = blockIdx.x * blockDim.x + threadIdx.x;
    if (i < n) { const int e = idx[i]; buf[2 * (size_t)i] = vec[e]; buf[2 * (size_t)i + 1] = vec[(size_t)chunk + e]; }
}
__global__ void k_halo_unpack(int n, const int* __restrict__ idx, const float* __restrict__ buf, int chunk, float* __restrict__ vec) {
    const int i = blockIdx.x * blockDim.x + threadIdx.x;
    if (i < n) { const int e = idx[i]; vec[e] = buf[2 * (size_t)i]; vec[(size_t)chunk + e] = buf[2 * (size_t)i + 1]; }
}
__global__ void k_halo_pack_multi(int n, const int* __restrict__ idx, const float* __restrict__ vec0, size_t stride, HaloSys sys, int nsys, int chunk, float* __restrict__ buf) {
    const int i = blockIdx.x * blockDim.x + threadIdx.x;
    if (i >= n * nsys) return;
    const int j = i / nsys, s = i - j * nsys, e = idx[j];
    const float* v = vec0 + (size_t)sys.id[s] * stride;
    buf[2 * (size_t)i] = v[e]; buf[2 * (size_t)i + 1] = v[(size_t)chunk + e];
}
__global__ void k_halo_unpack_multi(int n, const int* __restrict__ idx, const float* __restrict__ buf, size_t stride, HaloSys sys, int nsys, int chunk, float* __restrict__ vec0) {
    const int i = blockIdx.x * blockDim.x + threadIdx.x;
    if (i >= n * nsys) return;
    const int j = i / nsys, s = i - j * nsys, e = idx[j];
    float* v = vec0 + (size_t)sys.id[s] * stride;
    v[e] = buf[2 * (size_t)i]; v[(size_t)chunk + e] = buf[2 * (size_t)i + 1];
}
void launch_halo_pack_multi(hipStream_t st, int n, const int* idx, const float* vec0, size_t stride, HaloSys sys, int nsys, int chunk, float* buf) {
    if (n > 0 && nsys > 0) k_halo_pack_multi<<<(n * nsys + 255) / 256, 256, 0, st>>>(n, idx, vec0, stride, sys, nsys, chunk, buf);
}
void launch_halo_unpack_multi(hipStream_t st, int n, const int* idx, const float* buf, size_t stride, HaloSys sys, int nsys, int chunk, float* vec0) {
    if (n > 0 && nsys > 0) k_halo_unpack_multi<<<(n * nsys + 255) / 256, 256, 0, st>>>(n, idx, buf, stride, sys, nsys, chunk, vec0);
}
void launch_halo_pack(hipStream_t st, int n, const int* idx, const float* vec, int chunk, float* buf) { if (n > 0) k_halo_pack<<<(n + 255) / 256, 256, 0, st>>>(n, idx, vec, chunk, buf); }
void launch_halo_unpack(hipStream_t st, int n, const int* idx, const float* buf, int chunk, float* vec) { if (n > 0) k_halo_unpack<<<(n + 255) / 256, 256, 0, st>>>(n, idx, buf, chunk, vec); }

__global__ void k_mark_compute(RowView r, int* __restrict__ flag) {
    const int a = blockIdx.x * blockDim.x + threadIdx.x;
    if (a >= r.A) return;
    flag[a] = shard_needs_entry(a, r.own0, r.own1, (r.aflags[a] & F_ACTIVE) != 0, r.anbr, r.Acap) ? 1 : 0;
}
void launch_mark_compute(hipStream_t st, RowView r, int* flag) { if (r.A > 0) k_mark_compute<<<(r.A + 255) / 256, 256, 0, st>>>(r, flag); }
__global__ void k_compact_list(int A, const int* __restrict__ flag, const int* __restrict__ scan, int* __restrict__ list) {
    const int a = blockIdx.x * blockDim.x + threadIdx.x;
    if (a < A && flag[a]) list[scan[a]] = a;
}
void launch_compact_list(hipStream_t st, int A, const int* flag, const int* scan, int* list) { if (A > 0) k_compact_list<<<(A + 255) / 256, 256, 0, st>>>(A, flag, scan, list); }

}
```

intrinsic3d_amd/csrc/device/pcg_fused.hip:

```cpp
#include "kernels.hpp"
#include "reduce_device.hpp"
#include <cstring>

namespace i3d {

constexpr int PF_THREADS = 512;
constexpr int PF_MAX_WG = 512;
constexpr int PF_POSES_PER_WG = 10;

template <int NC>
static __device__ inline void reduce_partials_all(const double* __restrict__ P, int nblk, double (&tot)[NC], double* sm ,
                                                  const double* __restrict__ P2 = nullptr, int nblk2 = 0 ) {
    double v[NC];
#pragma unroll
    for (int k = 0; k < NC; ++k) v[k] = 0.0;
    for (int i = threadIdx.x; i < nblk; i += PF_THREADS) {
#pragma unroll
        for (int k = 0; k < NC; ++k) v[k] += P[(size_t)i * NC + k];
    }
    for (int i = threadIdx.x; i < nblk2; i += PF_THREADS) {
#pragma unroll
        for (int k = 0; k < NC; ++k) v[k] += P2[(size_t)i * NC + k];
    }
#pragma unroll
// ... 132 lines not shown
__global__ void __launch_bounds__(PF_THREADS, SH ? 4 : 1) k_pcg_dir3(int init, int n4, int seg4, size_t tail_rel, int ntail, const float* __restrict__ z, float* __restrict__ p,
                                                        const float* __restrict__ S, float* __restrict__ u, const float* __restrict__ D2 ,
                                                        const float* __restrict__ cm, const LmState* __restrict__ lm, const double* __restrict__ step_partials, int n_step, double* __restrict__ d2_partials,
                                                        const PcgState* __restrict__ prev, PcgState* __restrict__ next, int* host_flags, int seq, ShardArgs sa) {
    pcg_dir3_body<SH>(init, n4, seg4, tail_rel, ntail, z, p, S, u, D2 + tail_rel, cm, lm->inv_radius , step_partials, n_step, d2_partials, prev, next, host_flags, seq, sa);
}
template <bool COLL>
__global__ void __launch_bounds__(PF_THREADS, 1) k_pcg_dir3_lad(int init, int n4, int seg4, size_t tail_rel, int ntail, const float* __restrict__ z0, float* __restrict__ p0,
                                                        const float* __restrict__ S, float* __restrict__ u0, const float* __restrict__ tD2_0, const float* __restrict__ cm, const LmState* __restrict__ lm,
                                                        const double* __restrict__ step_partials0, int n_step, double* __restrict__ d2_partials0, PcgState* __restrict__ st2_0 , int prev_parity,
                                                        int* host_flags0, int seq, LadVec lv, int n_slice_partials, const double* __restrict__ red4_0) {
    const int j = lv.sysid[blockIdx.y];
    ShardArgs none; none.n_rim_wg = 0; none.n_slice_partials = n_slice_partials;
    const size_t vo = (size_t)j * lv.vec;
    pcg_dir3_body<COLL ? 2 : 0>(init, n4, seg4, tail_rel, ntail, z0 + vo, p0 + vo, S, u0 + vo, tD2_0 + (size_t)j * lv.tail, cm, lm->lad_inv_radius[j], step_partials0 + (size_t)j * lv.part, n_step,
                                d2_partials0 + (size_t)j * lv.part, st2_0 + 2 * j + prev_parity, st2_0 + 2 * j + (prev_parity ^ 1), host_flags0 + 4 * j, seq, none, COLL ? red4_0 + 4 * j : nullptr);
}

static int dir3_main_wgs(int n_entries, int cap) { int b = (n_entries / 2 + PF_THREADS - 1) / PF_THREADS; b = b < 1 ? 1 : b; return b > cap ? cap : b; }
int launch_pcg_dir3(hipStream_t st, bool init, Seg2 sg, size_t tail_off, int ntail, const float* z, float* p, const float* S, float* u, const float* D2, const float* cm, const LmState* lm,
                    const double* step_partials, int n_step, double* d2_partials, const PcgState* prev, PcgState* next, int* host_flags, int seq, const ShardArgs* sa) {
    const int n4 = sg.n >> 2, seg4 = (int)((sg.off1 - sg.off0) >> 2);
    const size_t o = sg.off0;
    if (!sa) {
        const int blocks = dir3_main_wgs(sg.n, PF_MAX_WG);
        ShardArgs none; std::memset(&none, 0, sizeof(none));
        k_pcg_dir3<0><<<blocks, PF_THREADS, 0, st>>>(init ? 1 : 0, n4, seg4, tail_off - o, ntail, z + o, p + o, S + o, u + o, D2 + o, cm + o, lm, step_partials, n_step, d2_partials, prev, next, host_flags, seq, none);
        return blocks;
    }
    const int cap = sa->pd.wg_cap > 0 ? sa->pd.wg_cap : PF_MAX_WG;
    const int n_main = dir3_main_wgs(sg.n, cap);
    k_pcg_dir3<1><<<sa->n_rim_wg + n_main + 1, PF_THREADS, 0, st>>>(init ? 1 : 0, n4, seg4, tail_off - o, ntail, z + o, p + o, S + o, u + o, D2 + o, cm + o, lm, step_partials, n_step, d2_partials, prev, next,
                                                                       host_flags, seq, *sa);
    return n_main;
}

int launch_pcg_dir3_lad(hipStream_t st, bool init, int nsys, Seg2 sg, size_t tail_off, int ntail, const float* z0, float* p0, const float* S, float* u0, const float* tD2_0, const float* cm, const LmState* lm,
                        const double* step_partials0, int n_step, double* d2_partials0, PcgState* st2_0, int prev_parity, int* host_flags0, int seq, const LadVec& lv,
                        int n_slice_partials, const double* red4_0) {
    const int n4 = sg.n >> 2, seg4 = (int)((sg.off1 - sg.off0) >> 2);
    const size_t o = sg.off0;
    const int blocks = dir3_main_wgs(sg.n, PF_MAX_WG);
    if (red4_0)
        k_pcg_dir3_lad<true><<<dim3(blocks + 1, nsys), PF_THREADS, 0, st>>>(init ? 1 : 0, n4, seg4, tail_off - o, ntail, z0 + o, p0 + o, S + o, u0 + o, tD2_0, cm + o, lm, step_partials0, n_step, d2_partials0,
                                                                            st2_0, prev_parity, host_flags0, seq, lv, n_slice_partials, red4_0);
    else
        k_pcg_dir3_lad<false><<<dim3(blocks, nsys), PF_THREADS, 0, st>>>(init ? 1 : 0, n4, seg4, tail_off - o, ntail, z0 + o, p0 + o, S + o, u0 + o, tD2_0, cm + o, lm, step_partials0, n_step, d2_partials0,
                                                                         st2_0, prev_parity, host_flags0, seq, lv, 0, nullptr);
    return blocks;
}

__global__ void __launch_bounds__(PF_THREADS) k_rim_u(ShardArgs sa, const PcgState* __restrict__ state) {
    if (state->done) return;
    const RimLists& rl = sa.rim; const unsigned e32 = p2p_pass_epoch(sa.seq, P2P_X_RESET_RIM);
    for (int j = blockIdx.x * PF_THREADS + threadIdx.x; j < rl.n_send; j += gridDim.x * PF_THREADS) {
        const int e = rl.send_idx[j], k = rl.send_peer[j];
        p2p_put_rim(sa.pd, 0, e32, k, j - rl.send_off[k], sa.ub[e], sa.ub[(size_t)sa.chunk + e]);
    }
    for (int j = blockIdx.x * PF_THREADS + threadIdx.x; j < rl.n_recv; j += gridDim.x * PF_THREADS) {
        const int e = rl.recv_idx[j], k = rl.recv_peer[j];
        float us, ua; p2p_get_rim(sa.pd, 0, e32, k, j - rl.recv_off[k], us, ua);
        sa.ub[e] = us; sa.ub[(size_t)sa.chunk + e] = ua;
    }
}
void launch_rim_u(hipStream_t st, const ShardArgs& sa, const PcgState* state) { if (sa.rim.n_send > 0 || sa.rim.n_recv > 0) k_rim_u<<<sa.n_rim_wg > 0 ? sa.n_rim_wg : 1, PF_THREADS, 0, st>>>(sa, state); }

enum { S3_INIT = 0, S3_NORMAL = 1, S3_XONLY = 2, S3_RESET = 3 };


struct S3Off { size_t v4, vo, qh2, part, cam, mblk, tail; int st, sys; };
struct S3In { float4 as, aa; int4 o; int o4; float4 x[2], p[2], b[2], cm[2], r[2]; };
template <int MODE> static __device__ inline void s3_load(const Step3Args& a, const S3Off& o, int q, S3In& v) {
    const float4* const qacc = a.qacc + o.v4; const float4* const x = a.x + o.v4; const float4* const p = a.p + o.v4; const float4* const r = a.r + o.v4;
    if (MODE == S3_NORMAL || MODE == S3_RESET) {
        v.as = qacc[q]; v.aa = qacc[q + a.chunk4];
        const int e = a.e0 + 4 * q;
        v.o = *reinterpret_cast<const int4*>(a.ext_off + e);
        v.o4 = a.ext_off[e + 4];
    }
#pragma unroll
    for (int seg = 0; seg < 2; ++seg) {
        const int i = q + seg * a.chunk4;
        v.cm[seg] = a.cm[i];
        if (MODE == S3_INIT) v.r[seg] = r[i];
        else {
            v.x[seg] = x[i];
            if (MODE != S3_RESET) v.p[seg] = p[i];
            if (MODE != S3_XONLY) { v.b[seg] = a.b[i]; if (MODE == S3_NORMAL) v.r[seg] = r[i]; }
        }
    }
}

template <int MODE, int SH>
static __device__ __forceinline__ void pcg_step3_body(const Step3Args& a, const S3Off& o) {
    __shared__ double sm[4 * 8];
    __shared__ double smx[SH == 1 ? P2P_MAX_RANKS : 1];
    __shared__ double camv[64];
    __shared__ double camred[8][64];
    __shared__ float rs[64];
    PcgState* const cur = a.cur + o.st;
    float4* const X = a.x + o.v4; float4* const R = a.r + o.v4; float4* const Z = a.z + o.v4;
    const double* const pq_partials = a.pq_partials + o.part; const double* const d2_partials = a.d2_partials + o.part; double* const step_partials = a.step_partials + o.part;
    const float2* const qh = a.qh + o.qh2; const float* const cam_partials = a.cam_partials + o.cam; const float* const Mblk = a.Mblk + o.mblk;
    const float* const tp = a.tp + o.vo; float* const tx = a.tx + o.vo; float* const tr = a.tr + o.vo; float* const tz = a.tz + o.vo; const float* const tD2 = a.tD2 + o.tail;
    const bool slice_wg = (int)blockIdx.x < a.n_slice_wg;
    const int q0 = blockIdx.x * PF_THREADS + threadIdx.x, qstride = a.n_slice_wg * PF_THREADS;
    S3In in;
    __shared__ int done_s;
    if (threadIdx.x == 0) done_s = cur->done;
    __syncthreads();
    if (done_s) return;
    const float inv_radius = o.sys >= 0 ? a.lm->lad_inv_radius[o.sys] : a.lm->inv_radius;
    float alpha = 0.0f;
    if (MODE == S3_NORMAL || MODE == S3_XONLY) {
        double t1[1];
        if (SH == 2) t1[0] = a.redop[(size_t)(o.sys < 0 ? 0 : o.sys) * a.redop_stride + 6 * a.K + 9] + d2_partials[a.n_d2];
        else reduce_partials_all<1>(pq_partials, a.n_pq, t1, sm, d2_partials, a.n_d2);
        if (SH == 1) {
            const unsigned e32 = p2p_pass_epoch(a.sh.seq, P2P_X_STEP);
            if (blockIdx.x == 0 && threadIdx.x == 0) p2p_put_double_all(a.sh.pd, 1, e32, 0, t1[0]);
            p2p_sum_all<1>(a.sh.pd, 1, e32, t1, smx);
            t1[0] += d2_partials[a.n_d2];
        }
        const double pq = t1[0];
        const double al = cur->rho / pq;
        const bool bad = !(pq > 0.0) || isinf(pq) || isinf(al);
        if (blockIdx.x == 0 && threadIdx.x == 0) { cur->pq = pq; if (bad) cur->done = 2; else cur->alpha = al; }
        if (bad) return;
        alpha = (float)al;
    }
    double s0 = 0.0, s1 = 0.0, s2 = 0.0, s3 = 0.0;
    if (slice_wg) {
        for (int q = q0; q < a.nq; q += qstride) {
            s3_load<MODE>(a, o, q, in);
            float accv[2][4];
            if (MODE == S3_NORMAL || MODE == S3_RESET) {
                const float4 as = in.as, aa = in.aa;
                accv[0][0] = as.x; accv[0][1] = as.y; accv[0][2] = as.z; accv[0][3] = as.w; accv[1][0] = aa.x; accv[1][1] = aa.y; accv[1][2] = aa.z; accv[1][3] = aa.w;
                const int ob[5] = {in.o.x, in.o.y, in.o.z, in.o.w, in.o4};
                for (int j0 = ob[0]; j0 < ob[4]; j0 += 8) {
                    int pos[8]; float2 hv[8];
#pragma unroll
                    for (int u = 0; u < 8; ++u) pos[u] = (j0 + u < ob[4]) ? a.ext_pos[j0 + u] : -1;
#pragma unroll
                    for (int u = 0; u < 8; ++u) hv[u] = pos[u] >= 0 ? qh[pos[u]] : make_float2(0.0f, 0.0f);
#pragma unroll
                    for (int u = 0; u < 8; ++u) {
                        const int j = j0 + u;
                        if (j < ob[4]) {
#pragma unroll
                            for (int k = 0; k < 4; ++k) { const bool mine = j >= ob[k] && j < ob[k + 1]; accv[0][k] += mine ? hv[u].x : 0.0f; accv[1][k] += mine ? hv[u].y : 0.0f; }
                        }
                    }
                }
            }
#pragma unroll
            for (int seg = 0; seg < 2; ++seg) {
                const int i = q + seg * a.chunk4;
                float xv[4], rv[4], svv[4], dv[4], mv[4];
                { const float4 cv = in.cm[seg]; lm_from_colnorm(cv.x, inv_radius, svv[0], dv[0], mv[0]); lm_from_colnorm(cv.y, inv_radius, svv[1], dv[1], mv[1]);
                  lm_from_colnorm(cv.z, inv_radius, svv[2], dv[2], mv[2]); lm_from_colnorm(cv.w, inv_radius, svv[3], dv[3], mv[3]); }
                if (MODE == S3_INIT) { const float4 t = in.r[seg]; rv[0] = t.x; rv[1] = t.y; rv[2] = t.z; rv[3] = t.w; }
                else {
                    const float4 xo = in.x[seg];
                    xv[0] = xo.x; xv[1] = xo.y; xv[2] = xo.z; xv[3] = xo.w;
                    float pv[4] = {0.0f, 0.0f, 0.0f, 0.0f};
                    if (MODE != S3_RESET) {
                        const float4 pp = in.p[seg]; pv[0] = pp.x; pv[1] = pp.y; pv[2] = pp.z; pv[3] = pp.w;
#pragma unroll
                        for (int k = 0; k < 4; ++k) xv[k] += alpha * pv[k];
                        X[i] = make_float4(xv[0], xv[1], xv[2], xv[3]);
                    }
                    if (MODE == S3_XONLY) continue;
                    const float4 bb = in.b[seg];
                    const float bv[4] = {bb.x, bb.y, bb.z, bb.w};
                    float qq[4];
#pragma unroll
                    for (int k = 0; k < 4; ++k) qq[k] = svv[k] * accv[seg][k] + dv[k] * (MODE == S3_NORMAL ? pv[k] : xv[k]);
                    if (MODE == S3_NORMAL) { const float4 ro = in.r[seg]; rv[0] = ro.x - alpha * qq[0]; rv[1] = ro.y - alpha * qq[1]; rv[2] = ro.z - alpha * qq[2]; rv[3] = ro.w - alpha * qq[3]; }
                    else { rv[0] = bv[0] - qq[0]; rv[1] = bv[1] - qq[1]; rv[2] = bv[2] - qq[2]; rv[3] = bv[3] - qq[3]; }
                    R[i] = make_float4(rv[0], rv[1], rv[2], rv[3]);
#pragma unroll
                    for (int k = 0; k < 4; ++k) { const double xd = xv[k]; s1 += xd * ((double)bv[k] + (double)rv[k]); s2 += xd * (double)rv[k]; s3 += (double)dv[k] * xd * xd; }
                }
                const float zv[4] = {mv[0] * rv[0], mv[1] * rv[1], mv[2] * rv[2], mv[3] * rv[3]};
                Z[i] = make_float4(zv[0], zv[1], zv[2], zv[3]);
#pragma unroll
                for (int k = 0; k < 4; ++k) s0 += (double)rv[k] * (double)zv[k];
            }
        }
    } else {
        const int K = a.K, tw = (int)blockIdx.x - a.n_slice_wg, n_pose_wg = (K + PF_POSES_PER_WG - 1) / PF_POSES_PER_WG;
        int col0, ncol;
        if (tw < n_pose_wg) { col0 = 6 * PF_POSES_PER_WG * tw; const int c1 = min(6 * K, col0 + 6 * PF_POSES_PER_WG); ncol = c1 - col0; }
        else { col0 = 6 * K; ncol = 9; }
        const int t = threadIdx.x;
        if (MODE == S3_NORMAL || MODE == S3_RESET) {
            const int g = t / 64, c = t % 64;
            double v = 0.0;
            if (SH != 2 && c < ncol) for (int w = g; w < a.n_cam; w += 8) v += (double)cam_partials[(size_t)w * a.cam_stride + col0 + c];
            camred[g][c] = v;
            __syncthreads();
            if (t < ncol) {
                double s = 0.0; for (int gg = 0; gg < 8; ++gg) s += camred[gg][t];
                if (SH == 2) s = a.redop[(size_t)(o.sys < 0 ? 0 : o.sys) * a.redop_stride + col0 + t];
                if (SH == 1) {
                    const unsigned e32 = p2p_pass_epoch(a.sh.seq, MODE == S3_RESET ? P2P_X_RESET_STEP : P2P_X_STEP);
                    p2p_put_double_all(a.sh.pd, 1, e32, 1 + col0 + t, s);
                    s = 0.0; for (int j = 0; j < a.sh.pd.L.world; ++j) s += p2p_get_double(a.sh.pd, 1, e32, j, 1 + col0 + t);
                }
                camv[t] = s;
            }
            __syncthreads();
        }
        if (t < ncol) {
            const int i = col0 + t;
            const bool fixed = i < 6 * K ? a.fix_poses : (i < 6 * K + 4 ? a.fix_intr : a.fix_dist);
            float ri;
            if (MODE == S3_INIT) ri = tr[i];
            else {
                float xi = tx[i];
                if (MODE != S3_RESET) { xi += alpha * tp[i]; tx[i] = xi; }
                if (MODE == S3_XONLY) ri = 0.0f;
                else {
                    const float vv = MODE == S3_NORMAL ? tp[i] : xi;
                    const float qi = a.tS[i] * (fixed ? 0.0f : (float)camv[t]) + tD2[i] * vv;
                    ri = MODE == S3_NORMAL ? tr[i] - alpha * qi : a.tb[i] - qi;
                    tr[i] = ri;
                    const double xd = xi; s1 += xd * ((double)a.tb[i] + (double)ri); s2 += xd * (double)ri; s3 += (double)tD2[i] * xd * xd;
                }
            }
            rs[t] = ri;
        }
        if (MODE == S3_XONLY) return;
        __syncthreads();
        if (t < ncol) {
            const int i = col0 + t;
            int base, n, row; const float* M;
            if (i < 6 * K) { const int f = i / 6; base = 6 * f; n = 6; row = i - base; M = Mblk + 36 * f; }
            else if (i < 6 * K + 4) { base = 6 * K; n = 4; row = i - base; M = Mblk + 36 * K; }
            else { base = 6 * K + 4; n = 5; row = i - base; M = Mblk + 36 * K + 16; }
            float s = 0.0f;
            for (int j = 0; j < n; ++j) s += M[row * n + j] * rs[base - col0 + j];
            tz[i] = s; s0 += (double)rs[t] * (double)s;
        }
    }
    if (MODE == S3_XONLY) return;
    block_partial_d(s0, step_partials, 4, 0); block_partial_d(s1, step_partials, 4, 1); block_partial_d(s2, step_partials, 4, 2); block_partial_d(s3, step_partials, 4, 3);
}
template <int MODE, int SH>
__global__ void __launch_bounds__(PF_THREADS) k_pcg_step3(Step3Args a) { const S3Off o{0, 0, 0, 0, 0, 0, 0, 0, -1}; pcg_step3_body<MODE, SH>(a, o); }
template <int MODE, bool COLL>
__global__ void __launch_bounds__(PF_THREADS) k_pcg_step3_lad(Step3Args a, LadVec lv) {
    const int j = lv.sysid[blockIdx.y];
    const S3Off o{((size_t)j * lv.vec) >> 2, (size_t)j * lv.vec, ((size_t)j * lv.qh) >> 1, (size_t)j * lv.part, (size_t)j * lv.cam, (size_t)j * lv.mblk, (size_t)j * lv.tail, 2 * j, j};
    pcg_step3_body<MODE, COLL ? 2 : 0>(a, o);
}

int pcg_step3_slice_wgs(int n_entries, int cap) { if (cap <= 0 || cap > PF_MAX_WG) cap = PF_MAX_WG; int b = (n_entries / 4 + PF_THREADS - 1) / PF_THREADS; return b < 1 ? 1 : (b > cap ? cap : b); }
int pcg_step3_tail_wgs(int K) { return (K + PF_POSES_PER_WG - 1) / PF_POSES_PER_WG + 1; }

int launch_pcg_step3(hipStream_t st, int mode, Step3Args a) {
    const int blocks = a.n_slice_wg + pcg_step3_tail_wgs(a.K);
#define I3D_S3(M) do { if (a.sharded) k_pcg_step3<M, 1><<<blocks, PF_THREADS, 0, st>>>(a); else k_pcg_step3<M, 0><<<blocks, PF_THREADS, 0, st>>>(a); } while (0)
    switch (mode) {
        case S3_INIT:   I3D_S3(S3_INIT); break;
        case S3_NORMAL: I3D_S3(S3_NORMAL); break;
        case S3_XONLY:  I3D_S3(S3_XONLY); break;
        default:        I3D_S3(S3_RESET); break;
    }
#undef I3D_S3
    return mode == S3_XONLY ? 0 : blocks;
}

int launch_pcg_step3_lad(hipStream_t st, int mode, int nsys, Step3Args a, const LadVec& lv) {
    const int blocks = a.n_slice_wg + pcg_step3_tail_wgs(a.K);
    const dim3 grid(blocks, nsys);
#define I3D_S3L(M) do { if (a.redop) k_pcg_step3_lad<M, true><<<grid, PF_THREADS, 0, st>>>(a, lv); else k_pcg_step3_lad<M, false><<<grid, PF_THREADS, 0, st>>>(a, lv); } while (0)
    switch (mode) {
        case S3_INIT:   I3D_S3L(S3_INIT); break;
        case S3_NORMAL: I3D_S3L(S3_NORMAL); break;
        case S3_XONLY:  I3D_S3L(S3_XONLY); break;
        default:        I3D_S3L(S3_RESET); break;
    }
#undef I3D_S3L
    return mode == S3_XONLY ? 0 : blocks;
}

__global__ void __launch_bounds__(PF_THREADS) k_lad_reduce_step(const double* __restrict__ step_partials0, int n_slice, double* __restrict__ red4_0, LadVec lv) {
    __shared__ double sm[4 * 8];
    const int j = lv.sysid[blockIdx.x];
    double tot[4];
    reduce_partials_all<4>(step_partials0 + (size_t)j * lv.part, n_slice, tot, sm);
    if (threadIdx.x < 4) red4_0[4 * j + threadIdx.x] = threadIdx.x == 0 ? tot[0] : threadIdx.x == 1 ? tot[1] : threadIdx.x == 2 ? tot[2] : tot[3];
}
void launch_lad_reduce_step(hipStream_t st, int nsys, const double* step_partials0, int n_slice, double* red4_0, const LadVec& lv) {
    k_lad_reduce_step<<<nsys, PF_THREADS, 0, st>>>(step_partials0, n_slice, red4_0, lv);
}
__global__ void __launch_bounds__(PF_THREADS) k_lad_reduce_op(const float* __restrict__ cam_partials0, int n_cam, int cam_stride, int NS, const double* __restrict__ pq_partials0, int n_pq,
                                                              const double* __restrict__ d2_partials0, int n_d2, double* __restrict__ redop0, int redop_stride, LadVec lv) {
    __shared__ double sm[8];
    __shared__ double camred[8][64];
    const int j = lv.sysid[blockIdx.y];
    double* const out = redop0 + (size_t)j * redop_stride;
    const int ncw = (NS + 63) / 64;
    if ((int)blockIdx.x < ncw) {
        const int t = threadIdx.x, g = t / 64, c = t % 64, col = (int)blockIdx.x * 64 + c;
        const float* cp = cam_partials0 + (size_t)j * lv.cam;
        double v = 0.0;
        if (col < NS) for (int w = g; w < n_cam; w += 8) v += (double)cp[(size_t)w * cam_stride + col];
        camred[g][c] = v;
        __syncthreads();
        if (t < 64 && col < NS) { double s = 0.0; for (int gg = 0; gg < 8; ++gg) s += camred[gg][t]; out[col] = s; }
    } else {
        double t1[1];
        reduce_partials_all<1>(pq_partials0 + (size_t)j * lv.part, n_pq, t1, sm, d2_partials0 + (size_t)j * lv.part, n_d2);
        if (threadIdx.x == 0) out[NS] = t1[0];
    }
}
void launch_lad_reduce_op(hipStream_t st, int nsys, const float* cam_partials0, int n_cam, int cam_stride, int NS, const double* pq_partials0, int n_pq, const double* d2_partials0, int n_d2,
                          double* redop0, int redop_stride, const LadVec& lv) {
    k_lad_reduce_op<<<dim3((NS + 63) / 64 + 1, nsys), PF_THREADS, 0, st>>>(cam_partials0, n_cam, cam_stride, NS, pq_partials0, n_pq, d2_partials0, n_d2, redop0, redop_stride, lv);
}

__global__ void k_pcg_init_lad(PcgState* st2_all, int B, int fixed_iterations, int max_iterations, const LmState* lm) {
    const int j = threadIdx.x;
    if (j >= B) return;
    const bool over = lm->done != 0 || lm->lad_radius[j] < 1e-32;
    for (int b = 0; b < 2; ++b) {
        PcgState* st = st2_all + 2 * j + b;
        for (int k = 0; k < 4; ++k) st->acc[k] = 0.0;
        st->rho = 0.0; st->last_rho = 1.0; st->pq = 0.0; st->alpha = 0.0; st->beta = 0.0; st->xbr = 0.0; st->xr = 0.0; st->d2xx = 0.0;
        st->Q0 = 0.0; st->Q1 = 0.0; st->it = 0; st->done = (fixed_iterations == 0 || over) ? 1 : 0; st->fixed_iterations = fixed_iterations; st->max_iterations = max_iterations;
    }
}
void launch_pcg_init_lad(hipStream_t st, PcgState* st2_all, int B, int fixed_iterations, int max_iterations, const LmState* lm) { k_pcg_init_lad<<<1, LADDER_MAX, 0, st>>>(st2_all, B, fixed_iterations, max_iterations, lm); }

__global__ void k_ext_offsets(int n, const int* __restrict__ ext_e, int A, int* __restrict__ ext_off) {
    const int e = blockIdx.x * blockDim.x + threadIdx.x;
    if (e > A) return;
    int lo = 0, hi = n;
    while (lo < hi) { const int mid = (lo + hi) >> 1; if (ext_e[mid] < e) lo = mid + 1; else hi = mid; }
    ext_off[e] = lo;
}
void launch_ext_offsets(hipStream_t st, int n, const int* ext_e, int A, int* ext_off) { k_ext_offsets<<<(A + 1 + 255) / 256, 256, 0, st>>>(n, ext_e, A, ext_off); }

}
```

intrinsic3d_amd/csrc/device/reduce_device.hpp:

```cpp
#pragma once
#include <hip/hip_runtime.h>

namespace i3d {

static __device__ inline double block_sum_d(double v) {
    __shared__ double sm_red[16];
    for (int o = 32; o > 0; o >>= 1) v += __shfl_down(v, o, 64);
    if ((threadIdx.x & 63) == 0) sm_red[threadIdx.x >> 6] = v;
    __syncthreads();
    double t = 0.0;
    if (threadIdx.x == 0) for (int i = 0; i < (int)((blockDim.x + 63) >> 6); ++i) t += sm_red[i];
    __syncthreads();
    return t;
}
static __device__ inline void block_partial_d(double v, double* partials, int ncomp, int comp) {
    const double t = block_sum_d(v);
    if (threadIdx.x == 0) partials[(size_t)blockIdx.x * ncomp + comp] = t;
}

}
```

intrinsic3d_amd/csrc/host/pcg.cpp:

```cpp
#include "solver_internal.hpp"
#include <algorithm>

namespace i3d {

int run_pass(i3d_context* c, PassMode mode, const OptParams& p, const float* u, float* out ) {
    hipStream_t s = c->stream; GridView g = c->grid_view(); RowView r = c->row_view(); const Layout L = layout_of(c);
    const int stride = (int)aux_part_stride(c->K);
    PassBuffers b{c->C.p, c->treg.p, c->d_shared.p, c->d_blocks.p, c->aux_part.p, stride};
    CTX_HIP(c, hipMemsetAsync(c->d_shared.p, 0, sizeof(double) * ((size_t)L.NS + 1), s));
    if (mode == PASS_COLNORM) CTX_HIP(c, hipMemsetAsync(c->d_blocks.p, 0, sizeof(double) * (21 * (size_t)c->K + 25), s));
    if (mode == PASS_JTJP && c->op.tile_ok && !c->sharded()) {
        const int NSP = (L.NS + 3) & ~3; int rows = 0;
        { TimedScope t(c, I3D_K_EG_PASS); rows = launch_eg_tile(s, r, p, u, c->tile_plan(), nullptr, out, nullptr, nullptr, c->cam_part.p, NSP); }
        { TimedScope t(c, I3D_K_GATHER); launch_halo_fold(s, r, c->tile_plan(), out, nullptr); }
        { TimedScope t(c, I3D_K_VECTOR); launch_mul(s, 2 * c->shard.chunk, c->v_mask.p, out, out);
          if (rows > 0) launch_sum_rows(s, PASS_JTJP, c->K, c->cam_part.p, rows, NSP, c->d_shared.p, c->d_blocks.p); }
    } else {
        int rows = 0;
        { TimedScope t(c, mode == PASS_JTJP ? I3D_K_EG_PASS : I3D_K_EG_AUX); rows = launch_eg_pass(s, mode, g, r, p, u, b, nullptr);
          if (rows > AUX_PART_ROWS) return ctx_fail(c, I3D_ERR_CAPACITY, "run_pass: more workgroups than rows of the camera partial buffer");
          if (rows > 0) launch_sum_rows(s, mode, c->K, c->aux_part.p, rows, stride, c->d_shared.p, c->d_blocks.p); }
        { TimedScope t(c, I3D_K_GATHER); launch_gather(s, mode, r, b, out); }
    }
    { int rc = allreduce(c, c->d_shared.p, (size_t)L.NS); if (rc) return rc; }
    if (mode == PASS_COLNORM) { int rc = allreduce(c, c->d_blocks.p, 21 * (size_t)c->K + 25); if (rc) return rc; }
    { TimedScope t(c, I3D_K_VECTOR); launch_shared_finalize(s, L.tail_off, c->K, p, c->d_shared.p, out, false, nullptr, nullptr, nullptr, nullptr, nullptr); }
    return I3D_OK;
}

int run_gradcol(i3d_context* c, const OptParams& p, const std::function<int()>& between) {
    hipStream_t s = c->stream; GridView g = c->grid_view(); RowView r = c->row_view(); const Layout L = layout_of(c);
    const int stride = (int)gc_part_stride(c->K), col_off = (int)gc_col_off(c->K);
    GradColBuffers gb{c->C.p, c->C2.p, c->treg.p, c->treg2.p, c->gc_part.p, stride, col_off, c->d_partials.p, c->d_scal.p + 16};
    CTX_HIP(c, hipMemsetAsync(c->d_scal.p + 16, 0, sizeof(double), s));
    CTX_HIP(c, hipMemsetAsync(c->d_shared.p, 0, sizeof(double) * ((size_t)L.NS + 1), s));
    CTX_HIP(c, hipMemsetAsync(c->d_blocks.p, 0, sizeof(double) * (21 * (size_t)c->K + 25), s));
    int rows = 0;
    { TimedScope t(c, I3D_K_EG_AUX); rows = launch_eg_gradcol(s, g, r, p, gb);
      if (rows > GC_PART_ROWS) return ctx_fail(c, I3D_ERR_CAPACITY, "run_gradcol: more workgroups than rows of the camera partial buffer");
      if (rows > 0) launch_sum_rows(s, PASS_COLNORM, c->K, c->gc_part.p + col_off, rows, stride, c->d_shared.p, c->d_blocks.p); }
    { PassBuffers b{c->C2.p, c->treg2.p, c->d_shared.p, c->d_blocks.p, nullptr, 0};
      TimedScope t(c, I3D_K_GATHER); launch_gather(s, PASS_COLNORM, r, b, c->v_c.p); }
    { TimedScope t(c, I3D_K_VECTOR); launch_shared_finalize(s, L.tail_off, c->K, p, c->d_shared.p, c->v_c.p, false, nullptr, nullptr, nullptr, nullptr, nullptr); }
    { int rc = between(); if (rc) return rc; }
    CTX_HIP(c, hipMemsetAsync(c->d_shared.p, 0, sizeof(double) * ((size_t)L.NS + 1), s));
    { TimedScope t(c, I3D_K_EG_AUX); if (rows > 0) launch_sum_rows(s, PASS_GRAD, c->K, c->gc_part.p, rows, stride, c->d_shared.p, c->d_blocks.p); }
    { PassBuffers b{c->C.p, c->treg.p, c->d_shared.p, c->d_blocks.p, nullptr, 0};
      TimedScope t(c, I3D_K_GATHER); launch_gather(s, PASS_GRAD, r, b, c->v_acc.p); }
    { TimedScope t(c, I3D_K_VECTOR); launch_shared_finalize(s, L.tail_off, c->K, p, c->d_shared.p, c->v_acc.p, false, nullptr, nullptr, nullptr, nullptr, nullptr); }
    return I3D_OK;
}

int dot_dev(i3d_context* c, const float* a, const float* b, double* slot) {
    const Layout L = layout_of(c);
    CTX_HIP(c, hipMemsetAsync(slot, 0, sizeof(double), c->stream));
    { TimedScope t(c, I3D_K_VECTOR); launch_dot2(c->stream, L.own, a, b, slot, c->d_partials.p); }
    { int rc = allreduce(c, slot, 1); if (rc) return rc; }
    { TimedScope t(c, I3D_K_VECTOR); launch_dot(c->stream, L.NS, a + L.tail_off, b + L.tail_off, slot, c->d_partials.p); }
    return I3D_OK;
}

int count_above_dev(i3d_context* c, const float* a, const float* m, float tol, double* slot) {
    const Layout L = layout_of(c);
    CTX_HIP(c, hipMemsetAsync(slot, 0, sizeof(double), c->stream));
    { TimedScope t(c, I3D_K_VECTOR); launch_count_above2(c->stream, L.own, a, m, tol, slot, c->d_partials.p); }
    { int rc = allreduce(c, slot, 1); if (rc) return rc; }
    { TimedScope t(c, I3D_K_VECTOR); launch_count_above(c->stream, L.NS, a + L.tail_off, m + L.tail_off, tol, slot, c->d_partials.p); }
    return I3D_OK;
}

int eval_cost_launch(i3d_context* c, const OptParams& p, bool candidate, const FrameConst* frames, const double* cam9, const LmState* lm) {
    GridView g = c->grid_view();
    if (candidate) { g.x_sdf = c->xc_sdf.p; g.x_alb = c->xc_alb.p; }
    { TimedScope t(c, I3D_K_COST); launch_build(c->stream, g, c->row_view(), p, frames, false, c->d_scal.p + 16, c->d_partials.p, cam9, lm); }
    return allreduce(c, c->d_scal.p + 16, 1);
}

constexpr int PCG_MAX_ITERATIONS = 500;
constexpr int PCG_MAX_PASSES = 520;
constexpr int PCG_RESET_PERIOD = 10;
constexpr int PCG_SEQ_STRIDE = 1024;

constexpr int PART_STEP = 4 * 2048, PART_PQ = 2048, PART_D2 = 2048;
struct Partials { double *step, *pq, *d2; };
static Partials partials_at(double* base) { return Partials{base, base + PART_STEP, base + PART_STEP + PART_PQ}; }

static int wait_pass(i3d_context* c, const int* ring, int want, const char* stalled, bool* done) {
    const double t_wait = now_s();
    while (__atomic_load_n(&ring[0], __ATOMIC_ACQUIRE) != want) {
        if (now_s() - t_wait > 30.0) { CTX_HIP(c, sync_stream(c)); if (__atomic_load_n(&ring[0], __ATOMIC_ACQUIRE) != want) return ctx_fail(c, I3D_ERR_HIP, stalled); }
    }
    *done = __atomic_load_n(&ring[1], __ATOMIC_ACQUIRE) != 0;
    return I3D_OK;
}
static int previous_pass_done(i3d_context* c, int it, int seq, bool* done) {
    if (it < 2) return I3D_OK;
    return wait_pass(c, c->h_flags + 2 * ((seq - 1) & 1), seq - 1, "pcg_solve: the device stopped publishing its state", done);
}

static int begin_passes(const i3d_context* c) { return c->pcg_seq; }
static void end_passes(i3d_context* c, int seq0) { c->pcg_seq = seq0 + PCG_SEQ_STRIDE; }

static void launch_u_from_x(i3d_context* c, const Layout& L, const float* x, float* u) {
    launch_mul2(c->stream, L.own, c->v_S.p, x, u); launch_mul(c->stream, L.NS, c->v_S.p + L.tail_off, x + L.tail_off, u + L.tail_off);
}

int pcg_solve(i3d_context* c, const SolveRoute& route, const i3d_optimizer_config& cfg, const OptParams& p, const PcgState** final_state) {
    hipStream_t s = c->stream;
    const Layout L = layout_of(c);
    const int K = c->K;
    const bool sh = c->sharded();
    GridView g = c->grid_view(); RowView r = c->row_view();
    PassBuffers pb{c->C.p, c->treg.p, c->d_shared.p, c->d_blocks.p, c->aux_part.p, (int)aux_part_stride(c->K)};
    PcgState* st = c->d_pcg.p;
    double* pq_slot = c->d_shared.p + L.NS;
    const size_t to = L.tail_off; const Seg2 own = L.own;
    { TimedScope t(c, I3D_K_VECTOR); launch_fill(s, (int)L.NP, c->v_x.p, 0.0f); launch_pcg_init(s, st, cfg.pcg_fixed_iterations, PCG_MAX_ITERATIONS, c->d_lm.p); }
    CTX_HIP(c, hipMemcpyAsync(c->v_r.p, c->v_b.p, sizeof(float) * L.NP, hipMemcpyDeviceToDevice, s));
    const Partials part = partials_at(c->d_partials.p);
    int n_pq = 0, n_step = 0, n_d2 = 0;
    const bool dev_reduce = route.exchange == Exchange::InKernelReduce;
    const P2PDev& pd = route.reduce_dev;
    auto rows_apply = [&](const float* v, float* out, bool with_dot, bool zero_first) -> int {
        if (zero_first) CTX_HIP(c, hipMemsetAsync(c->d_shared.p, 0, sizeof(double) * ((size_t)L.NS + 1), s));
        if (sh) {
            { int rc = push_halo(c, c->v_u.p); if (rc) return rc; }
            { TimedScope t(c, I3D_K_EG_PASS);
              n_pq = launch_eg_tile(s, r, p, c->v_u.p, c->tile_plan(), c->d_shared.p, c->v_qacc.p, with_dot ? part.pq : nullptr, st); }
            { TimedScope t(c, I3D_K_GATHER); launch_halo_fold(s, r, c->tile_plan(), c->v_qacc.p, st); }
            if (!with_dot) n_pq = 0;
            if (dev_reduce && with_dot) return I3D_OK;
            if (with_dot) { TimedScope t(c, I3D_K_VECTOR); launch_reduce_partials(s, part.pq, n_pq, 1, pq_slot, st); launch_reduce_partials(s, part.d2, n_d2, 1, pq_slot, st); }
            n_pq = 0;
            return allreduce(c, c->d_shared.p, (size_t)L.NS + 1);
        }
        { TimedScope t(c, I3D_K_EG_PASS); launch_eg_pass(s, PASS_JTJP, g, r, p, c->v_u.p, pb, st); }
        { TimedScope t(c, I3D_K_GATHER); n_pq = launch_gather_tail(s, r, pb, out, c->v_S.p, c->v_D2.p, v, with_dot ? part.pq : nullptr, false, st); }
        if (!with_dot) n_pq = 0;
        return I3D_OK;
    };
    auto fold_step = [&]() { if (sh && !dev_reduce) { launch_reduce_partials(s, part.step, n_step, 4, st->acc, st); n_step = 0; } };
    const float* const Sq = sh ? c->v_S.p : nullptr;
    { TimedScope t(c, I3D_K_VECTOR);
      n_step = launch_pcg_step(s, 0 , own, c->v_p.p, c->v_q.p, c->v_x.p, c->v_r.p, c->v_b.p, c->v_D2.p, c->v_Minv.p, c->v_z.p, nullptr, part.step, st);
      fold_step(); }
    int tail_mode = 0;
    const int seq0 = begin_passes(c);
    for (int it = 1;; ++it) {
        if (sh && !dev_reduce) { int rc = allreduce(c, st->acc, 4); if (rc) return rc; }
        if (dev_reduce) { c->comm->count_reduce(4); c->comm->count_reduce((size_t)L.NS + 1); }
        { TimedScope t(c, I3D_K_VECTOR);
          launch_pcg_tail_a(s, tail_mode, to, K, c->Minv_blocks.p, c->v_p.p, tail_mode == 3 ? c->v_tmp.p : c->v_q.p, c->v_x.p, c->v_r.p, c->v_b.p, c->v_D2.p, c->v_z.p,
                            part.step, n_step, st, c->d_shared.p, L.NS + 1, c->d_flags, seq0 + it, pd); }
        { TimedScope t(c, I3D_K_VECTOR);
          n_d2 = launch_pcg_direction(s, own, to, L.NS, c->v_z.p, c->v_p.p, c->v_S.p, c->v_u.p, c->v_D2.p, sh ? part.d2 : nullptr, st); }
        { int rc = rows_apply(c->v_p.p, c->v_q.p, true, false); if (rc) return rc; }
        { TimedScope t(c, I3D_K_VECTOR); launch_pcg_tail_b(s, to, K, p, c->d_shared.p, pq_slot, part.pq, n_pq, part.d2, dev_reduce ? n_d2 : 0, sh,
                                                           c->v_q.p, c->v_S.p, c->v_D2.p, c->v_p.p, st, pd); }
        if (it % PCG_RESET_PERIOD != 0) {
            TimedScope t(c, I3D_K_VECTOR);
            n_step = launch_pcg_step(s, 1, own, c->v_p.p, sh ? c->v_qacc.p : c->v_q.p, c->v_x.p, c->v_r.p, c->v_b.p, c->v_D2.p, c->v_Minv.p, c->v_z.p, Sq, part.step, st);
            fold_step();
            tail_mode = 1;
        } else {
            { TimedScope t(c, I3D_K_VECTOR);
              launch_pcg_step(s, 2, own, c->v_p.p, c->v_q.p, c->v_x.p, c->v_r.p, c->v_b.p, c->v_D2.p, c->v_Minv.p, c->v_z.p, nullptr, part.step, st);
              launch_pcg_tail_x(s, to, K, c->v_p.p, c->v_x.p, st);
              launch_u_from_x(c, L, c->v_x.p, c->v_u.p); }
            { int rc = rows_apply(c->v_x.p, c->v_tmp.p, false, true); if (rc) return rc; }
            { TimedScope t(c, I3D_K_VECTOR);
              launch_shared_finalize(s, to, K, p, c->d_shared.p, c->v_tmp.p, true, c->v_S.p, c->v_D2.p, c->v_x.p, nullptr, st);
              n_step = launch_pcg_step(s, 3, own, c->v_p.p, sh ? c->v_qacc.p : c->v_tmp.p, c->v_x.p, c->v_r.p, c->v_b.p, c->v_D2.p, c->v_Minv.p, c->v_z.p, Sq, part.step, st);
              fold_step(); }
            tail_mode = 3;
        }
        bool done = false;
        { const int rc = previous_pass_done(c, it, seq0 + it, &done); if (rc) return rc; }
        if (done || it > PCG_MAX_PASSES) break;
    }
    end_passes(c, seq0);
    *final_state = st;
    return I3D_OK;
}

static Step3Args step3_args(const i3d_context* c, const Layout& L, const OptParams& p, const TilePlan& tp, float* x, float* r, float* pv, float* z, const float* q, const float* qh,
                            const Partials& part, const float* cam, const float* Mblk, const float* tD2, int wg_cap) {
    const Seg2 own = L.own; const size_t to = L.tail_off;
    Step3Args a; std::memset(&a, 0, sizeof(a));
    auto c4 = [&](const float* v) { return reinterpret_cast<const float4*>(v + own.off0); };
    auto m4 = [&](float* v) { return reinterpret_cast<float4*>(v + own.off0); };
    a.nq = own.n >> 2; a.chunk4 = (int)((own.off1 - own.off0) >> 2);
    a.p = c4(pv); a.qacc = c4(q); a.x = m4(x); a.r = m4(r); a.b = c4(c->v_b.p); a.z = m4(z); a.cm = c4(c->v_cm.p); a.lm = c->d_lm.p;
    a.ext_off = tp.ext_off; a.ext_pos = tp.ext_pos; a.qh = reinterpret_cast<const float2*>(qh); a.e0 = (int)own.off0;
    a.pq_partials = part.pq; a.d2_partials = part.d2; a.n_pq = 0; a.n_d2 = 0;
    a.n_slice_wg = pcg_step3_slice_wgs(own.n, wg_cap);
    a.K = c->K; a.fix_poses = p.fix_poses; a.fix_intr = p.fix_intr; a.fix_dist = p.fix_dist;
    a.cam_partials = cam; a.n_cam = 0; a.cam_stride = (L.NS + 3) & ~3; a.Mblk = Mblk;
    a.tp = pv + to; a.tx = x + to; a.tr = r + to; a.tb = c->v_b.p + to; a.tD2 = tD2; a.tz = z + to; a.tS = c->v_S.p + to;
    a.step_partials = part.step;
    return a;
}

int pcg_solve_fused(i3d_context* c, const SolveRoute& route, const i3d_optimizer_config& cfg, const OptParams& p, const PcgState** final_state) {
    hipStream_t s = c->stream;
    const Layout L = layout_of(c);
    const size_t to = L.tail_off; const Seg2 own = L.own;
    RowView r = c->row_view(); TilePlan tp = c->tile_plan();
    const bool sh = route.exchange == Exchange::InKernel;
    ShardArgs sa; std::memset(&sa, 0, sizeof(sa));
    if (sh) {
        if (!c->comm->fused_exchange(&sa.pd) || L.NS + 2 > sa.pd.L.red_cap) return ctx_fail(c, I3D_ERR_STATE, "pcg_solve_fused: the in-kernel exchanges are not available");
        const ShardState& sd = c->shard; const HaloPlan& h = sd.halo;
        sa.rim = RimLists{h.n_send, h.n_recv, sd.halo_send_idx.p, sd.halo_send_peer.p, sd.halo_recv_idx.p, sd.halo_recv_peer.p, sd.halo_offs.p, sd.halo_offs.p + P2P_MAX_RANKS};
        sa.n_rim_wg = (h.n_send + h.n_recv) > 0 ? std::max(1, std::min(4, (std::max(h.n_send, h.n_recv) + 1023) / 1024)) : 1;
        sa.zb = c->v_z.p; sa.pb = c->v_p.p; sa.ub = c->v_u.p; sa.cmb = c->v_cm.p; sa.chunk = sd.chunk;
    }
    const int wg_cap = sh ? sa.pd.wg_cap : 0;
    PcgState* const st2 = c->d_pcg2.p;
    const int NSP = (L.NS + 3) & ~3;
    const Partials part = partials_at(c->d_partials.p);
    { TimedScope t(c, I3D_K_VECTOR); launch_fill(s, (int)L.NP, c->v_x.p, 0.0f); launch_pcg_init3(s, st2, cfg.pcg_fixed_iterations, PCG_MAX_ITERATIONS, c->d_lm.p); }
    CTX_HIP(c, hipMemcpyAsync(c->v_r.p, c->v_b.p, sizeof(float) * L.NP, hipMemcpyDeviceToDevice, s));
    Step3Args a = step3_args(c, L, p, tp, c->v_x.p, c->v_r.p, c->v_p.p, c->v_z.p, c->v_qacc.p, tp.qh, part, c->cam_part.p, c->Minv_blocks.p, c->v_D2.p + to, wg_cap);
    a.sharded = sh ? 1 : 0; a.lad_sys = -1;
    int n_step = 0;
    { TimedScope t(c, I3D_K_VECTOR); a.cur = st2; n_step = launch_pcg_step3(s, 0 , a); }
    const bool mr1 = c->op.mr1_serial && !sh && route.multi_system;
    auto op = [&](double* pq, const PcgState* cur) -> int {
        if (mr1) { const int sys0[3] = {0, 0, 0}; LadVec z; std::memset(&z, 0, sizeof(z));
                   return launch_eg_tile_mr(s, r, p, tp, 1, sys0, c->v_u.p, c->v_qacc.p, tp.qh, pq, c->cam_part.p, NSP, cur, z); }
        return launch_eg_tile(s, r, p, c->v_u.p, tp, nullptr, c->v_qacc.p, pq, cur, c->cam_part.p, NSP);
    };
    const int seq0 = begin_passes(c);
    int it = 1;
    for (;; ++it) {
        PcgState* const prev = st2 + ((it + 1) & 1); PcgState* const cur = st2 + (it & 1);
        sa.seq = seq0 + it; sa.n_slice_partials = a.n_slice_wg; a.sh = sa;
        { TimedScope t(c, I3D_K_VECTOR);
          a.n_d2 = launch_pcg_dir3(s, it == 1, own, to, L.NS, c->v_z.p, c->v_p.p, c->v_S.p, c->v_u.p, c->v_D2.p, c->v_cm.p, c->d_lm.p, part.step, n_step, part.d2, prev, cur, c->d_flags, seq0 + it,
                                   sh ? &sa : nullptr); }
        if (sh) { c->comm->count_reduce(4); c->comm->count_halo(c->shard.halo.n_send); c->comm->count_reduce((size_t)L.NS + 1); }
        { TimedScope t(c, I3D_K_EG_PASS); a.n_pq = op(part.pq, cur); a.n_cam = a.n_pq; }
        a.cur = cur;
        if (it % PCG_RESET_PERIOD != 0) { TimedScope t(c, I3D_K_VECTOR); n_step = launch_pcg_step3(s, 1, a); }
        else {
            { TimedScope t(c, I3D_K_VECTOR); launch_pcg_step3(s, 2, a); launch_u_from_x(c, L, c->v_x.p, c->v_u.p); }
            if (sh) { TimedScope t(c, I3D_K_COMM); launch_rim_u(s, sa, cur); c->comm->count_halo(c->shard.halo.n_send); }
            { TimedScope t(c, I3D_K_EG_PASS); a.n_cam = op(nullptr, cur); }
            { TimedScope t(c, I3D_K_VECTOR); n_step = launch_pcg_step3(s, 3, a); }
        }
        bool done = false;
        { const int rc = previous_pass_done(c, it, seq0 + it, &done); if (rc) return rc; }
        if (done || it > PCG_MAX_PASSES) break;
    }
    end_passes(c, seq0);
    *final_state = st2 + (it & 1);
    { const int lrc = ctx_launch_check(c); if (lrc) return lrc; }
    return I3D_OK;
}

static size_t lad_redop_stride(int NS) { return ((size_t)NS + 1 + 3) & ~(size_t)3; }
int alloc_ladder(i3d_context* c) {
    const Layout L = layout_of(c);
    const int nsys = c->op.ladder_max;
    LadderState& ld = c->ladder; LadVec& lv = ld.strides;
    const size_t vec = ((size_t)L.NP + 65535) & ~(size_t)65535;
    const size_t qh = 2 * (size_t)tile_plan_tiles_of((int)std::min((size_t)c->Acap, ((size_t)c->shard.chunk + 65535) & ~(size_t)65535), 512) * (size_t)tile_plan_hmax_of(512);
    const size_t cam = (size_t)2048 * (((size_t)L.NS + 3) & ~(size_t)3);
    lv.vec = vec; lv.qh = qh; lv.cam = cam; lv.part = PART_STEP + PART_PQ + PART_D2; lv.mblk = ((size_t)36 * c->K + 41 + 3) & ~(size_t)3; lv.tail = ((size_t)L.NS + 3) & ~(size_t)3;
    const bool fresh = ld.vec.n < (size_t)6 * nsys * vec || !ld.vec.p;
    bool ok = ld.vec.alloc((size_t)6 * nsys * vec) == hipSuccess;
    if (ok && fresh) ok = hipMemsetAsync(ld.vec.p, 0, sizeof(float) * ld.vec.n, c->stream) == hipSuccess;
    ok = ok && ld.qh.alloc((size_t)nsys * qh) == hipSuccess && ld.cam.alloc((size_t)nsys * cam) == hipSuccess && ld.part.alloc((size_t)nsys * lv.part) == hipSuccess
            && ld.mblk.alloc((size_t)nsys * lv.mblk) == hipSuccess && ld.tail.alloc((size_t)nsys * lv.tail) == hipSuccess && ld.st.alloc((size_t)2 * LADDER_MAX) == hipSuccess;
    if (ok && c->sharded()) {
        const size_t n = (size_t)LADDER_MAX * (4 + lad_redop_stride(L.NS));
        const bool fresh_r = ld.red.n < n || !ld.red.p;
        ok = ld.red.alloc(n) == hipSuccess;
        if (ok && fresh_r) ok = hipMemsetAsync(ld.red.p, 0, sizeof(double) * ld.red.n, c->stream) == hipSuccess;
    }
    if (!ok) {
        (void)hipGetLastError();
        ld.vec.release(); ld.qh.release(); ld.cam.release(); ld.part.release();
        std::fprintf(stderr, "[i3d] the slabs of the damping ladder (%d systems x %.1f MB) do not fit the device: this outer iteration runs the serial trust-region loop\n", nsys,
                     (double)(6 * vec + qh + cam) * 4.0 / 1e6);
        return 1;
    }
    return I3D_OK;
}

int pcg_solve_ladder(i3d_context* c, const SolveRoute& route, const i3d_optimizer_config& cfg, const OptParams& p, int B, const PcgState** finals) {
    hipStream_t s = c->stream;
    const Layout L = layout_of(c);
    const int K = c->K; const size_t to = L.tail_off; const Seg2 own = L.own;
    RowView r = c->row_view(); TilePlan tp = c->tile_plan();
    LadderState& ld = c->ladder; LadVec lv = ld.strides;
    float* const X0 = lad_vecp(c, LV_X); float* const R0 = lad_vecp(c, LV_R); float* const P0 = lad_vecp(c, LV_P); float* const Z0 = lad_vecp(c, LV_Z);
    float* const U0 = lad_vecp(c, LV_U); float* const Q0 = lad_vecp(c, LV_Q);
    PcgState* const st2 = ld.st.p;
    const int NSP = (L.NS + 3) & ~3;
    const Partials part0 = partials_at(ld.part.p);
    const bool use_mr = c->sw.ladder_mr;
    const bool mr1 = c->sw.ladder_mr1;
    const int mr_cap = std::min(c->sw.ladder_group, eg_tile_mr_max_systems(K));
    const bool pair = c->sw.ladder_pair;
    const bool mr_ok = use_mr && mr_cap >= 1 && route.multi_system;
    const bool sh = route.exchange == Exchange::Transport;
    double* const red4 = sh ? ld.red.p : nullptr;
    const int rstride = (int)lad_redop_stride(L.NS);
    double* const redop = sh ? ld.red.p + (size_t)LADDER_MAX * 4 : nullptr;
    { TimedScope t(c, I3D_K_VECTOR);
      for (int j = 0; j < B; ++j) { CTX_HIP(c, hipMemsetAsync(X0 + (size_t)j * lv.vec, 0, sizeof(float) * L.NP, s));
                                    CTX_HIP(c, hipMemcpyAsync(R0 + (size_t)j * lv.vec, c->v_b.p, sizeof(float) * L.NP, hipMemcpyDeviceToDevice, s)); }
      launch_pcg_init_lad(s, st2, B, cfg.pcg_fixed_iterations, PCG_MAX_ITERATIONS, c->d_lm.p); }
    Step3Args a = step3_args(c, L, p, tp, X0, R0, P0, Z0, Q0, ld.qh.p, part0, ld.cam.p, ld.mblk.p, ld.tail.p, 0);
    a.sharded = 0; a.lad_sys = 0; a.redop = redop; a.redop_stride = rstride;
    std::vector<int> live(B); for (int j = 0; j < B; ++j) live[j] = j;
    auto set_slots = [&]() { for (int q = 0; q < LADDER_MAX; ++q) lv.sysid[q] = live[q < (int)live.size() ? q : (int)live.size() - 1]; };
    auto rows_apply = [&](int parity, bool with_dot) -> int {
        int n = 0; const int nl = (int)live.size();
        if (sh) { TimedScope t(c, I3D_K_COMM);
                  if (c->comm->push_halo_multi(U0, lv.vec, live.data(), nl, c->shard.halo, s)) return -1; }
        if (mr_ok && (nl > 1 || mr1 || sh)) {
            const int groups = (nl + mr_cap - 1) / mr_cap;
            int at = 0;
            if (groups == 2 && pair && !sh && nl - (nl + 1) / 2 >= 2) {
                const int na = (nl + 1) / 2;
                TimedScope t(c, na == 2 ? I3D_K_EG_MR2 : I3D_K_EG_MR3);
                n = launch_eg_tile_mr_pair(s, r, p, tp, na, nl - na, live.data(), U0, Q0, ld.qh.p, with_dot ? part0.pq : nullptr, ld.cam.p, NSP, st2 + parity, lv);
                if (n > 0) { at = nl; ++ld.streams; ++ld.paired; }
            }
            for (int g = 0; g < groups && at < nl; ++g) {
                const int ng = (nl - at + (groups - g) - 1) / (groups - g);
                TimedScope t(c, ng == 1 ? I3D_K_EG_PASS : (ng == 2 ? I3D_K_EG_MR2 : I3D_K_EG_MR3));
                n = launch_eg_tile_mr(s, r, p, tp, ng, live.data() + at, U0, Q0, ld.qh.p, with_dot ? part0.pq : nullptr, ld.cam.p, NSP, st2 + parity, lv);
                if (n <= 0) return -1;
                at += ng; ++ld.streams;
            }
        } else {
            for (int j : live) {
                TilePlan tj = tp; tj.qh = ld.qh.p + (size_t)j * lv.qh;
                TimedScope t(c, I3D_K_EG_PASS);
                n = launch_eg_tile(s, r, p, U0 + (size_t)j * lv.vec, tj, nullptr, Q0 + (size_t)j * lv.vec, with_dot ? part0.pq + (size_t)j * lv.part : nullptr, st2 + 2 * j + parity,
                                   ld.cam.p + (size_t)j * lv.cam, NSP);
                ++ld.streams;
            }
        }
        ld.system_passes += nl; ++ld.pass_live[nl < 6 ? nl : 6];
        if (sh) {
            { TimedScope t(c, I3D_K_VECTOR); launch_lad_reduce_op(s, nl, ld.cam.p, n, NSP, L.NS, part0.pq, with_dot ? n : 0, part0.d2, with_dot ? a.n_d2 : 0, redop, rstride, lv); }
            if (allreduce(c, redop, (size_t)LADDER_MAX * rstride)) return -1;
        }
        return n;
    };
    auto step_sums = [&](int nl, int n_slice) -> int {
        if (!sh) return I3D_OK;
        { TimedScope t(c, I3D_K_VECTOR); launch_lad_reduce_step(s, nl, part0.step, n_slice, red4, lv); }
        return allreduce(c, red4, (size_t)LADDER_MAX * 4);
    };
    int n_step = 0;
    set_slots();
    { TimedScope t(c, I3D_K_VECTOR); a.cur = st2; n_step = launch_pcg_step3_lad(s, 0 , B, a, lv); }
    for (int j = 0; j < B; ++j) finals[j] = st2 + 2 * j;
    const int seq0 = begin_passes(c);
    int it = 1;
    for (;; ++it) {
        set_slots();
        const int nl = (int)live.size();
        { const int rc = step_sums(nl, a.n_slice_wg); if (rc) return rc; }
        { TimedScope t(c, I3D_K_VECTOR);
          a.n_d2 = launch_pcg_dir3_lad(s, it == 1, nl, own, to, L.NS, Z0, P0, c->v_S.p, U0, ld.tail.p, c->v_cm.p, c->d_lm.p, part0.step, n_step, part0.d2, st2, (it + 1) & 1, c->d_flags, seq0 + it, lv,
                                       a.n_slice_wg, red4); }
        { const int n = rows_apply(it & 1, true); if (n < 0) return ctx_fail(c, I3D_ERR_STATE, "pcg_solve_ladder: the multi-system operator pass could not be launched"); a.n_pq = n; a.n_cam = n; }
        a.cur = st2 + (it & 1);
        if (it % PCG_RESET_PERIOD != 0) { TimedScope t(c, I3D_K_VECTOR); n_step = launch_pcg_step3_lad(s, 1, nl, a, lv); }
        else {
            { TimedScope t(c, I3D_K_VECTOR); launch_pcg_step3_lad(s, 2, nl, a, lv);
              for (int j : live) launch_u_from_x(c, L, X0 + (size_t)j * lv.vec, U0 + (size_t)j * lv.vec); }
            { const int n = rows_apply(it & 1, false); if (n < 0) return ctx_fail(c, I3D_ERR_STATE, "pcg_solve_ladder: the multi-system operator pass could not be launched"); a.n_cam = n; }
            { TimedScope t(c, I3D_K_VECTOR); n_step = launch_pcg_step3_lad(s, 3, nl, a, lv); }
        }
        {
            const int want = seq0 + it;
            std::vector<int> still;
            for (int j : live) {
                bool done = false;
                { const int rc = wait_pass(c, c->h_flags + 4 * j + 2 * (want & 1), want, "pcg_solve_ladder: the device stopped publishing its state", &done); if (rc) return rc; }
                if (!done) still.push_back(j);
                else finals[j] = st2 + 2 * j + (it & 1);
            }
            live.swap(still);
        }
        if (live.empty() || it > PCG_MAX_PASSES) break;
    }
    end_passes(c, seq0);
    for (int j : live) finals[j] = st2 + 2 * j + (it & 1);
    { const int lrc = ctx_launch_check(c); if (lrc) return lrc; }
    return I3D_OK;
}

}
```

intrinsic3d_amd/csrc/host/solver.cpp:

```cpp
#include "solver_internal.hpp"
#include <cstdlib>
#include <algorithm>

namespace i3d {

#ifdef I3D_MR_PHASES
void mr_phase_report_now();
#endif
#ifdef I3D_MR_BLOCKTIME
void mr_blocktime_report_now();
#endif

void read_switches(i3d_context* c) {
    auto env = [](const char* name) { return std::getenv(name); };
    auto is = [&](const char* name, char v) { const char* e = env(name); return e && e[0] == v; };
    auto num = [&](const char* name, int unset) { const char* e = env(name); return e ? std::atoi(e) : unset; };
    auto clamp = [](int v, int lo, int hi) { return v < lo ? lo : (v > hi ? hi : v); };
    SolverSwitches w;
    { const char* e = env("I3D_DETERMINISTIC"); w.deterministic = e ? (e[0] == '1' ? 1 : 0) : -1; }
    w.ladder = clamp(num("I3D_LADDER", LADDER_MAX), 1, LADDER_MAX);
    w.ladder_mr = !is("I3D_LADDER_MR", '0');
    w.ladder_mr1 = is("I3D_LADDER_MR1", '1');
    w.ladder_group = clamp(num("I3D_LADDER_GROUP", 3), 1, 3);
    w.ladder_pair = !is("I3D_LADDER_PAIR", '0');
    w.egt_mr1 = is("I3D_EGT_MR1", '1');
    { const char* e = env("I3D_EGT_TILE"); w.egt_tile = e ? (std::atoi(e) == 512 ? 512 : 1024) : 0; }
    w.hmax_limit = num("I3D_EGT_HMAX_LIMIT", 0);
    w.hmax_limit_1024 = num("I3D_EGT_HMAX_LIMIT_1024", 0);
    w.halo_pull = is("I3D_HALO_PULL", '1');
    w.no_tile = is("I3D_NO_TILE", '1');
    { const char* e = env("I3D_NO_CULL"); w.no_cull = (e && e[0] >= '1' && e[0] <= '3') ? e[0] - '0' : 0; }
    w.gradcol = !is("I3D_GRADCOL", '0');
    w.cost0 = !is("I3D_COST0", '0');
    w.debug_invalid_attempt = num("I3D_DEBUG_INVALID_ATTEMPT", -1);
    { const int v = num("I3D_SH_SLAB", 0); w.sh_slab = v > 0 ? v : 0; }
    c->sw = w;
}

static int wait_record(i3d_context* c, int idx, int seq, LmRecord& out) {
    LmRecord* const r = c->h_lmrec + idx;
    const double t0 = now_s();
    while (__atomic_load_n(&r->seq, __ATOMIC_ACQUIRE) != seq) {
        if (now_s() - t0 > 60.0) {
            CTX_HIP(c, sync_stream(c));
            if (__atomic_load_n(&r->seq, __ATOMIC_ACQUIRE) != seq) return ctx_fail(c, I3D_ERR_HIP, "lm_solve: the device stopped publishing the state of the trust-region loop");
        }
    }
    out = *r;
    return I3D_OK;
}

static SolveRoute solve_route(i3d_context* c) {
    const int NS = 6 * c->K + 9;
    const bool sh = c->sharded();
    SolveRoute rt; std::memset(&rt.reduce_dev, 0, sizeof(rt.reduce_dev));
    rt.multi_system = multi_system_ok(c);
    bool in_kernel = false;
    if (c->op.tile_ok && sh) { P2PDev probe; in_kernel = c->comm->fused_exchange(&probe) && NS + 2 <= probe.L.red_cap; }
    const bool three = c->op.tile_ok && (!sh || in_kernel);
    bool ladder = c->op.ladder_max > 1 && c->op.tile_ok && (sh ? !in_kernel : true) && rt.multi_system;
    if (ladder && alloc_ladder(c) != I3D_OK) {
        ladder = false;
    }
    rt.loop = ladder ? PcgLoop::Ladder : (three ? PcgLoop::ThreeLaunch : PcgLoop::SixLaunch);
    rt.exchange = !sh ? Exchange::None : (three ? Exchange::InKernel : Exchange::Transport);
    if (sh && rt.loop == PcgLoop::SixLaunch) {
        const bool ok = c->comm->device_reduce(&rt.reduce_dev) && NS + 1 <= rt.reduce_dev.L.red_cap;
        if (ok) rt.exchange = Exchange::InKernelReduce; else rt.reduce_dev.on = 0;
    }
    return rt;
}

static int lm_solve(i3d_context* c, const i3d_optimizer_config& cfg, OptParams& p, i3d_iteration_stats* st, double initial_radius) {
    hipStream_t s = c->stream;
    const Layout L = layout_of(c);
    const int N = c->N, K = c->K, NP = (int)L.NP, NS = L.NS;
    GridView g = c->grid_view(); RowView r = c->row_view();
    LadderState& ld = c->ladder;
    if (cfg.lm_steps > LM_REC_SLOTS - 2) return ctx_fail(c, I3D_ERR_CAPACITY, "optimize: more than 62 LM steps per outer iteration");
    const SolveRoute route = solve_route(c);
    { TimedScope t(c, I3D_K_VECTOR); launch_freemask(s, r, p, c->v_mask.p); }
    CTX_HIP(c, hipMemcpyAsync(c->xc_sdf.p, c->x_sdf.p, sizeof(double) * (size_t)N, hipMemcpyDeviceToDevice, s));
    CTX_HIP(c, hipMemcpyAsync(c->xc_alb.p, c->x_alb.p, sizeof(double) * (size_t)N, hipMemcpyDeviceToDevice, s));
    const bool one_stream = one_stream_gradcol(c);
    auto after_colnorm = [&]() -> int {
        CTX_HIP(c, hipMemcpyAsync(c->d_cam_c.p, c->d_shared.p, sizeof(double) * (size_t)NS, hipMemcpyDeviceToDevice, s));
        CTX_HIP(c, hipMemcpyAsync(c->d_cam_H.p, c->d_blocks.p, sizeof(double) * ((size_t)21 * K + 25), hipMemcpyDeviceToDevice, s));
        { int rc2 = allgather(c, c->v_c.p); if (rc2) return rc2; }
        { TimedScope t(c, I3D_K_VECTOR); launch_scale_from_colnorm(s, NP, c->v_c.p, c->v_mask.p, c->v_S.p, c->v_cm.p); }
        return I3D_OK;
    };
    int rc = I3D_OK;
    if (one_stream) { rc = run_gradcol(c, p, after_colnorm); if (rc) return rc; }
    else {
        rc = run_pass(c, PASS_COLNORM, p, nullptr, c->v_c.p); if (rc) return rc;
        rc = after_colnorm(); if (rc) return rc;
        rc = run_pass(c, PASS_GRAD, p, nullptr, c->v_acc.p); if (rc) return rc;
    }
    { TimedScope t(c, I3D_K_VECTOR); launch_mul(s, NP, c->v_S.p, c->v_acc.p, c->v_b.p); }
    if (!c->sw.cost0) { rc = eval_cost_launch(c, p, false, c->d_frames.p); if (rc) return rc; }
    else if (!one_stream) { TimedScope t(c, I3D_K_VECTOR); launch_set_double(s, c->d_scal.p + 16, c->cost_at_build); }
    rc = count_above_dev(c, c->v_acc.p, c->v_mask.p, 1e-10f, c->d_scal.p + 8); if (rc) return rc;
    rc = dot_dev(c, c->v_mask.p, c->v_mask.p, c->d_scal.p + 9); if (rc) return rc;
    {
        double* xs = c->h_pinned;
        for (int i = 0; i < 6 * K; ++i) xs[i] = c->poses[i];
        for (int i = 0; i < 4; ++i) xs[6 * K + i] = c->intr[i];
        for (int i = 0; i < 5; ++i) xs[6 * K + 4 + i] = c->dist[i];
        CTX_HIP(c, hipMemcpyAsync(c->d_xshared.p, xs, sizeof(double) * NS, hipMemcpyHostToDevice, s));
    }
    const int seq0 = c->lm_seq; c->lm_seq += LM_REC_SLOTS;
    LmState* const lm = c->d_lm.p;
    launch_lm_init(s, lm, c->d_scal.p + 16, c->d_scal.p + 8, c->d_scal.p + 9, initial_radius, c->d_lmrec, seq0);

    int attempts = 0; bool ended = false, accepted = false;
    auto consume = [&](const LmRecord& rec) {
        if (rec.kind == 0) {
            if (st) { st->cost_initial = rec.cost; st->cost_final = rec.cost; st->free_parameters = (int64_t)(rec.nfree + 0.5); st->termination = rec.final_ ? 1 : 0; st->final_radius = initial_radius; }
            c->last_sizes[5] = (long long)(rec.nfree + 0.5);
        } else if (rec.kind == 2) { if (st) st->termination = 1; }
        else {
            if (st) {
                st->lm_iterations = attempts + 1;
                if (attempts < 50) { st->pcg_iterations[attempts] = rec.pcg_it; st->step_accepted[attempts] = rec.accepted; }
                st->final_radius = rec.radius_after; st->termination = rec.termination;
                if (rec.accepted) { st->cost_final = rec.cost; st->successful_steps += 1; }
            }
            if (cfg.verbose) std::printf("  [i3d LM] it %d cand %.9e model %.3e rho %.4f radius -> %.3e cg %d%s\n", attempts + 1, rec.cand_cost, rec.model_change, rec.rel, rec.radius_after, rec.pcg_it,
                                         rec.accepted ? " accepted" : "");
            accepted = rec.accepted != 0;
            ++attempts;
        }
        if (rec.final_) ended = true;
    };
    auto queue_decision = [&](const float* x, const PcgState* ps, int attempt, int lad_next) -> int {
        { TimedScope t(c, I3D_K_VECTOR);
          launch_candidate(s, g, r, K, -1.0f, x, c->v_S.p, c->d_xshared.p, c->xc_sdf.p, c->xc_alb.p, c->d_xcshared.p, c->d_scal.p + 4, c->v_mask.p, c->d_partials.p, lm);
          launch_cand_frames(s, K, c->d_xcshared.p, c->d_frames.p, c->d_frames_cand.p, lm); }
        const int rc2 = eval_cost_launch(c, p, true, c->d_frames_cand.p, c->d_xcshared.p + 6 * K, lm); if (rc2) return rc2;
        { TimedScope t(c, I3D_K_VECTOR);
          launch_lm_decide(s, lm, ps, c->d_scal.p + 4, c->d_scal.p + 16, attempt, cfg.lm_steps, c->d_lmrec + 1 + attempt, seq0 + 1 + attempt, lad_next,
                           c->sw.debug_invalid_attempt == attempt ? 1 : 0);
          launch_accept(s, g, r, c->xc_sdf.p, c->xc_alb.p, lm); }
        return I3D_OK;
    };
    if (route.loop == PcgLoop::Ladder) {
        const LadVec& lv = ld.strides;
        { LmRecord rec; rc = wait_record(c, 0, seq0, rec); if (rc) return rc; consume(rec); }
        const bool warm = ld.hint > 0;
        int k = 0, prevB = 0; bool after_resync = false;
        while (k < cfg.lm_steps && !ended) {
            int B = after_resync ? 1 : (prevB == 0 ? (warm ? std::max(ld.hint, ld.hint_prev) : 2) : (warm ? 2 : 2 * prevB));
            B = std::max(1, std::min(B, std::min(c->op.ladder_max, cfg.lm_steps - k)));
            after_resync = false; prevB = B;
            { TimedScope t(c, I3D_K_VECTOR);
              launch_lm_begin_lad(s, lm, B, K, p.fix_poses, p.fix_intr, p.fix_dist, c->d_cam_c.p, c->d_cam_H.p, ld.mblk.p, lv.mblk, c->v_c.p + L.tail_off, c->v_S.p + L.tail_off, ld.tail.p, lv.tail,
                                  c->d_lmrec + 1 + k, seq0 + 1 + k); }
            const PcgState* fin[LADDER_MAX] = {nullptr};
            rc = pcg_solve_ladder(c, route, cfg, p, B, fin); if (rc) return rc;
            ++ld.batches;
            for (int j = 0; j < B && c->sharded(); ++j) { rc = allgather(c, lad_vecp(c, LV_X, j)); if (rc) return rc; }
            for (int j = 0; j < B; ++j) { rc = queue_decision(lad_vecp(c, LV_X, j), fin[j], k + j, j + 1); if (rc) return rc; }
            int decided = 0;
            for (int j = 0; j < B && !ended; ++j) {
                LmRecord rec; rc = wait_record(c, 1 + k + j, seq0 + 1 + k + j, rec); if (rc) return rc;
                if (rec.kind == 3) {
                    __atomic_store_n(&c->h_lmrec[1 + k + j].seq, 0, __ATOMIC_RELEASE);
                    ++ld.resyncs; after_resync = true; break;
                }
                consume(rec); ++decided;
            }
            if (ended && decided < B) ld.wasted += B - decided;
            k += decided;
        }
        if (attempts > 0) { ld.hint_prev = ld.hint; ld.hint = attempts; }
        ended = true;
    }
    const bool three = route.loop == PcgLoop::ThreeLaunch;
    int k = 0;
    for (; route.loop != PcgLoop::Ladder && k < cfg.lm_steps; ++k) {
        { TimedScope t(c, I3D_K_VECTOR);
          launch_lm_begin(s, lm, K, p.fix_poses, p.fix_intr, p.fix_dist, c->d_cam_c.p, c->d_cam_H.p, c->Minv_blocks.p, c->v_c.p + L.tail_off, c->v_S.p + L.tail_off, c->v_D2.p + L.tail_off, c->v_Minv.p + L.tail_off,
                          c->d_lmrec + 1 + k, seq0 + 1 + k);
          if (!three) launch_lm_diag_dev(s, (int)L.tail_off, c->v_c.p, c->v_S.p, lm, c->v_D2.p, c->v_Minv.p); }
        const PcgState* ps = nullptr;
        rc = three ? pcg_solve_fused(c, route, cfg, p, &ps) : pcg_solve(c, route, cfg, p, &ps); if (rc) return rc;
        { LmRecord rec; rc = wait_record(c, k, seq0 + k, rec); if (rc) return rc; consume(rec); }
        if (ended) break;
        { int rc2 = allgather(c, c->v_x.p); if (rc2) return rc2; }
        rc = queue_decision(c->v_x.p, ps, k, -1); if (rc) return rc;
    }
    if (!ended) { LmRecord rec; rc = wait_record(c, k, seq0 + k, rec); if (rc) return rc; consume(rec); }
    if (st) st->num_attempts = std::min(attempts, 50);
    CTX_HIP(c, hipMemcpyAsync(c->h_pinned, c->d_xcshared.p, sizeof(double) * NS, hipMemcpyDeviceToHost, s));
    CTX_HIP(c, sync_stream(c));
    if (c->sharded() && c->comm->health(s)) return ctx_fail(c, I3D_ERR_COMM, "lm_solve: a peer-to-peer exchange timed out (a rank stopped taking part)");
    if (accepted) {
        for (int i = 0; i < 6 * K; ++i) c->poses[i] = c->h_pinned[i];
        for (int i = 0; i < 4; ++i) c->intr[i] = c->h_pinned[6 * K + i];
        for (int i = 0; i < 5; ++i) c->dist[i] = c->h_pinned[6 * K + 4 + i];
    }
    { const int lrc = ctx_launch_check(c); if (lrc) return lrc; }
    return I3D_OK;
}

int optimize(i3d_context* c, const i3d_optimizer_config& cfg, i3d_iteration_stats* stats) {
    if (!c->have_grid || cfg.iterations < 1) return ctx_fail(c, I3D_ERR_INVALID_ARGUMENT, "optimize: no grid or iterations < 1");
    CTX_HIP(c, hipSetDevice(c->device));
    double carried_radius = 1e4;
    for (int itr = 0; itr < cfg.iterations; ++itr) {
        i3d_iteration_stats local; std::memset(&local, 0, sizeof(local));
        i3d_iteration_stats* st = stats ? &stats[itr] : &local;
        std::memset(st, 0, sizeof(*st));
        OptParams p;
        const double t0 = now_s();
        int rc = assemble(c, cfg, itr, p, st); if (rc) return rc;
        const double t1 = now_s();
        st->time_add = (c->t_add_end >= 0.0 && c->t_add_end <= t1 - t0) ? c->t_add_end : t1 - t0; st->time_build = (t1 - t0) - st->time_add;
        if (c->n_active > 0) { rc = lm_solve(c, cfg, p, st, cfg.carry_trust_radius ? carried_radius : 1e4); if (rc) return rc;
                               if (st->final_radius > 0.0) carried_radius = st->final_radius; }
        const double t2 = now_s();
        st->time_solve = t2 - t1;
        if (cfg.verbose) std::printf("[i3d] itr %d rows %lld/%lld/%lld/%lld valid %lld cost %.9e -> %.9e (add %.3f ms, solve %.3f ms)\n", itr,
                                     (long long)st->rows[0], (long long)st->rows[1], (long long)st->rows[2], (long long)st->rows[3], (long long)st->valid_voxels,
                                     st->cost_initial, st->cost_final, st->time_add * 1e3, st->time_solve * 1e3);
// ... 14 lines not shown
```

intrinsic3d_amd/csrc/host/solver_internal.hpp:

```cpp
#pragma once
#include "context.hpp"
#include <chrono>
#include <functional>

namespace i3d {

inline double now_s() { return std::chrono::duration<double>(std::chrono::steady_clock::now().time_since_epoch()).count(); }

constexpr int AUX_PART_ROWS = 320;
inline size_t aux_part_stride(int K) { return ((size_t)21 * K + 34 + 3) & ~(size_t)3; }
constexpr int GC_PART_ROWS = 1024;
inline size_t gc_col_off(int K) { return ((size_t)6 * K + 9 + 3) & ~(size_t)3; }
inline size_t gc_part_stride(int K) { return gc_col_off(K) + aux_part_stride(K); }
constexpr int LM_REC_SLOTS = 64;

inline hipError_t sync_stream(i3d_context* c) { ++c->n_syncs; return hipStreamSynchronize(c->stream); }

struct Layout { int A, K, NS, chunk, world, rank, slice; Seg2 own; size_t tail_off, NP; };
inline Layout layout_of(const i3d_context* c) {
    Layout L; L.A = c->A; L.K = c->K; L.NS = 6 * c->K + 9; L.chunk = c->shard.chunk; L.world = c->comm ? c->comm->world : 1; L.rank = c->comm ? c->comm->rank : 0;
    L.slice = L.chunk / L.world;
    L.own = Seg2{(size_t)L.rank * L.slice, (size_t)L.chunk + (size_t)L.rank * L.slice, L.slice};
    L.tail_off = 2 * (size_t)L.chunk; L.NP = L.tail_off + L.NS;
    return L;
}
inline bool one_stream_gradcol(const i3d_context* c) { return !c->sharded() && c->sw.gradcol; }
inline bool cost_from_sums(const i3d_context* c) { return c->sw.cost0 && !one_stream_gradcol(c); }

inline int allreduce(i3d_context* c, double* dev, size_t n) {
    if (!c->sharded()) return I3D_OK;
    TimedScope t(c, I3D_K_COMM);
    return c->comm->allreduce_sum(dev, n, c->stream) ? ctx_fail(c, I3D_ERR_COMM, "all-reduce failed") : I3D_OK;
}
inline int allgather(i3d_context* c, float* vec) {
    if (!c->sharded()) return I3D_OK;
    const size_t slice = (size_t)(c->shard.chunk / c->comm->world);
    TimedScope t(c, I3D_K_COMM);
    if (c->comm->allgather(vec, slice, c->stream) || c->comm->allgather(vec + c->shard.chunk, slice, c->stream)) return ctx_fail(c, I3D_ERR_COMM, "all-gather failed");
    return I3D_OK;
}
inline int push_halo(i3d_context* c, float* vec) {
    if (!c->sharded()) return I3D_OK;
    TimedScope t(c, I3D_K_COMM);
    return c->comm->push_halo(vec, c->shard.halo, c->stream) ? ctx_fail(c, I3D_ERR_COMM, "halo exchange failed") : I3D_OK;
}

inline int read_doubles(i3d_context* c, const double* dptr, size_t n, double* out) {
    CTX_HIP(c, hipMemcpyAsync(c->h_pinned, dptr, n * sizeof(double), hipMemcpyDeviceToHost, c->stream));
    CTX_HIP(c, sync_stream(c));
    std::memcpy(out, c->h_pinned, n * sizeof(double));
    return I3D_OK;
}

inline bool multi_system_ok(const i3d_context* c) { return c->plan_T() == 512 && c->tile_plan().hp_off != nullptr && c->slots == 5; }

enum class PcgLoop { SixLaunch, ThreeLaunch, Ladder };
enum class Exchange {
    None,
    Transport,
    InKernelReduce,
    InKernel
};
struct SolveRoute {
    PcgLoop loop = PcgLoop::SixLaunch; Exchange exchange = Exchange::None;
    bool multi_system = false;
    P2PDev reduce_dev;
};

int run_pass(i3d_context* c, PassMode mode, const OptParams& p, const float* u, float* out);
int run_gradcol(i3d_context* c, const OptParams& p, const std::function<int()>& between);
int dot_dev(i3d_context* c, const float* a, const float* b, double* slot);
int count_above_dev(i3d_context* c, const float* a, const float* m, float tol, double* slot);
int eval_cost_launch(i3d_context* c, const OptParams& p, bool candidate, const FrameConst* frames, const double* cam9 = nullptr, const LmState* lm = nullptr);
int alloc_ladder(i3d_context* c);
enum { LV_X = 0, LV_R, LV_P, LV_Z, LV_U, LV_Q };
inline float* lad_vecp(const i3d_context* c, int kind, int sys = 0) { return c->ladder.vec.p + ((size_t)kind * c->op.ladder_max + sys) * c->ladder.strides.vec; }
int pcg_solve(i3d_context* c, const SolveRoute& route, const i3d_optimizer_config& cfg, const OptParams& p, const PcgState** final_state);
int pcg_solve_fused(i3d_context* c, const SolveRoute& route, const i3d_optimizer_config& cfg, const OptParams& p, const PcgState** final_state);
int pcg_solve_ladder(i3d_context* c, const SolveRoute& route, const i3d_optimizer_config& cfg, const OptParams& p, int B, const PcgState** finals);

}
```

Measured before the change: 43.87.

## Fold small reductions and copies into LM init/decide kernels to cut launches

Partial-sum reductions for candidate cost and norms are now done inside the single LM decide kernel, which is widened to 1024 threads. The count-above and mask-norm tests are fused into one multi-segment kernel whose partials are reduced inside LM init. Redundant device copies (cam colnorm copies, PCG x/r init memsets in the unsharded case) are skipped, and per-system u_from_x launches are batched into one ladder kernel. The aim is to remove many tiny kernel launches and memcpy operations per Gauss-Newton iteration. In exchange, the single-block LM kernels do more work serially, and the changes rely on other kernels initialising the buffers whose copies are now skipped.

```diff
diff --git a/intrinsic3d_amd/csrc/device/build.hip b/intrinsic3d_amd/csrc/device/build.hip
--- a/intrinsic3d_amd/csrc/device/build.hip
+++ b/intrinsic3d_amd/csrc/device/build.hip
@@ -505,7 +505,8 @@
 }
 
 void launch_build(hipStream_t st, GridView g, RowView r, OptParams p, const FrameConst* frames, bool with_jacobian, double* cost_out, double* scratch,
-                  const double* cam9, const LmState* lm) {
+                  const double* cam9, const LmState* lm, int* n_partials) {
+    if (n_partials) *n_partials = 0;
     if (r.nC <= 0) { if (!with_jacobian && cost_out) (void)hipMemsetAsync(cost_out, 0, sizeof(double), st); return; }
 #ifdef I3D_COST_MULTI_PROBE
     const int blocks = with_jacobian ? (r.nC + 255) / 256 : (((r.nC + 255) / 256 + 7) / 8) * 8 * I3D_COST_MULTI_PROBE;
@@ -528,7 +529,9 @@
         if (lds <= 48 * 1024) k_build<false, true, 2><<<blocks, 256, lds, st>>>(g, r, p, frames, cost_out, cam9, lm);
         else k_build<false, false, 2><<<blocks, 256, 0, st>>>(g, r, p, frames, cost_out, cam9, lm);
     }
-    if (!with_jacobian) launch_reduce_partials(st, scratch, blocks, 1, cost_dst, nullptr, true);
+    if (with_jacobian) return;
+    if (n_partials) *n_partials = blocks;
+    else launch_reduce_partials(st, scratch, blocks, 1, cost_dst, nullptr, true);
 }
 
 template <bool COST>
diff --git a/intrinsic3d_amd/csrc/device/gradcol.hip b/intrinsic3d_amd/csrc/device/gradcol.hip
--- a/intrinsic3d_amd/csrc/device/gradcol.hip
+++ b/intrinsic3d_amd/csrc/device/gradcol.hip
@@ -177,7 +177,7 @@
     if (!set_dynamic_lds((const void*)k_eg_gradcol, "k_eg_gradcol", n, p.K)) return 0;
     const int used = (ntiles + tiles_per_block - 1) / tiles_per_block;
     k_eg_gradcol<<<used, GC_THREADS, n, st>>>(g, r, p, b, tiles_per_block);
-    launch_reduce_partials(st, b.cost_partials, used, 1, b.cost_out, nullptr);
+    launch_reduce_partials(st, b.cost_partials, used, 1, b.cost_out, nullptr, true);
     return used;
 }
 
diff --git a/intrinsic3d_amd/csrc/device/kernels.hpp b/intrinsic3d_amd/csrc/device/kernels.hpp
--- a/intrinsic3d_amd/csrc/device/kernels.hpp
+++ b/intrinsic3d_amd/csrc/device/kernels.hpp
@@ -30,7 +30,7 @@
 void launch_group_cull(hipStream_t st, GridView g, RowView r, OptParams p, const FrameConst* frames, const float2* dblocks, float4* bounds, unsigned* mask);
 
 void launch_build(hipStream_t st, GridView g, RowView r, OptParams p, const FrameConst* frames, bool with_jacobian, double* cost_out , double* scratch,
-                  const double* cam9 = nullptr, const LmState* lm = nullptr);
+                  const double* cam9 = nullptr, const LmState* lm = nullptr, int* n_partials = nullptr);
 void launch_weight_sums(hipStream_t st, RowView r, GridView g, bool with_cost, double* sums13 , double* scratch);
 
 enum PassMode { PASS_GRAD = 0, PASS_JTJP = 1, PASS_COLNORM = 2 };
@@ -51,7 +51,8 @@
 };
 int  launch_eg_gradcol(hipStream_t st, GridView g, RowView r, OptParams p, GradColBuffers b);
 int  launch_eg_pass(hipStream_t st, PassMode mode, GridView g, RowView r, OptParams p, const float* u , PassBuffers b, const PcgState* state);
-void launch_sum_rows(hipStream_t st, PassMode mode, int K, const float* part, int nrows, int stride, double* shared, double* blocks);
+void launch_sum_rows(hipStream_t st, PassMode mode, int K, const float* part, int nrows, int stride, double* shared, double* blocks,
+                     double* shared2 = nullptr, double* blocks2 = nullptr);
 void launch_gather(hipStream_t st, PassMode mode, RowView r, PassBuffers b, float* out );
 int  launch_gather_tail(hipStream_t st, RowView r, PassBuffers b, float* out, const float* S, const float* D2, const float* v, double* dot_partials ,
                         bool dot_atomic, const PcgState* state);
@@ -65,9 +66,9 @@
 void launch_mul(hipStream_t st, int n, const float* a, const float* b, float* out);
 void launch_scale_from_colnorm(hipStream_t st, int n, const float* c, const float* freemask, float* S, float* cm);
 void launch_dot(hipStream_t st, int n, const float* a, const float* b, double* out , double* scratch);
-void launch_count_above2(hipStream_t st, Seg2 sg, const float* a, const float* m, float tol, double* out, double* scratch);
+void launch_count_above2(hipStream_t st, Seg2 sg, const float* a, const float* m, float tol, double* out, double* scratch, bool assign = false);
 void launch_count_above(hipStream_t st, int n, const float* a, const float* m, float tol, double* out, double* scratch);
-void launch_dot2(hipStream_t st, Seg2 sg, const float* a, const float* b, double* out , double* scratch);
+void launch_dot2(hipStream_t st, Seg2 sg, const float* a, const float* b, double* out , double* scratch, bool assign = false);
 void launch_mul2(hipStream_t st, Seg2 sg, const float* a, const float* b, float* out);
 void launch_freemask(hipStream_t st, RowView r, OptParams p, float* mask );
 
@@ -163,6 +164,7 @@
                          const double* step_partials0, int n_step, double* d2_partials0, PcgState* st2_0, int prev_parity, int* host_flags0, int seq, const LadVec& lv,
                          int n_slice_partials = 0, const double* red4_0 = nullptr );
 int  launch_pcg_step3_lad(hipStream_t st, int mode, int nsys, Step3Args a, const LadVec& lv);
+void launch_u_from_x_lad(hipStream_t st, int nsys, Seg2 sg, size_t tail_off, int ntail, const float* S, const float* x0, float* u0, const LadVec& lv);
 void launch_lad_reduce_step(hipStream_t st, int nsys, const double* step_partials0, int n_slice, double* red4_0, const LadVec& lv);
 void launch_lad_reduce_op(hipStream_t st, int nsys, const float* cam_partials0, int n_cam, int cam_stride, int NS, const double* pq_partials0, int n_pq, const double* d2_partials0, int n_d2,
                           double* redop0, int redop_stride, const LadVec& lv);
@@ -173,17 +175,20 @@
 size_t halo_sort_temp_bytes(int cap);
 hipError_t launch_halo_sort(hipStream_t st, void* temp, size_t temp_bytes, const unsigned long long* in, unsigned long long* out, int n);
 
-void launch_candidate(hipStream_t st, GridView g, RowView r, int K, float sign, const float* step, const float* S, const double* x_shared, double* xc_sdf, double* xc_alb,
-                      double* xc_shared, double* norms2 , const float* mask, double* scratch, const LmState* lm = nullptr);
+int  launch_candidate(hipStream_t st, GridView g, RowView r, int K, float sign, const float* step, const float* S, const double* x_shared, double* xc_sdf, double* xc_alb,
+                      double* xc_shared, double* norms2, const float* mask, double* scratch, const LmState* lm = nullptr);
 void launch_accept(hipStream_t st, GridView g, RowView r, const double* xc_sdf, const double* xc_alb, const LmState* lm = nullptr);
 void launch_set_double(hipStream_t st, double* dst, double v);
-void launch_lm_init(hipStream_t st, LmState* lm, const double* cost, const double* ngrad, const double* nfree, double radius0, LmRecord* rec, int seq);
+void launch_lm_tests(hipStream_t st, Seg2 sg, size_t tail_off, int ntail, const float* g, const float* mask, float tol, double* part, int* b2, int* b1);
+void launch_lm_init(hipStream_t st, LmState* lm, const double* cost, double* ngrad, double* nfree, double radius0, LmRecord* rec, int seq,
+                    const double* test_part = nullptr, int b2 = 0, int b1 = 0);
 void launch_lm_begin(hipStream_t st, LmState* lm, int K, int fix_poses, int fix_intr, int fix_dist, const double* cdiag, const double* tri, float* Mblk,
                      const float* tc, const float* tS, float* tD2, float* tMinv, LmRecord* rec, int seq);
 void launch_lm_diag_dev(hipStream_t st, int n, const float* c, const float* S, const LmState* lm, float* D2, float* Minv);
 void launch_cand_frames(hipStream_t st, int K, const double* xc, const FrameConst* base, FrameConst* out, const LmState* lm);
+struct DecideSums { const double* cost_partials; int n_cost; double* cost_dst; const double* norm_partials; int n_norm; double* norms_dst; };
 void launch_lm_decide(hipStream_t st, LmState* lm, const PcgState* ps, const double* norms2, const double* cand_cost, int attempt, int lm_steps, LmRecord* rec, int seq,
-                      int lad_next = -1 , int debug_invalid = 0);
+                      int lad_next = -1 , int debug_invalid = 0, const DecideSums* sums = nullptr);
 void launch_lm_begin_lad(hipStream_t st, LmState* lm, int B, int K, int fix_poses, int fix_intr, int fix_dist, const double* cdiag, const double* tri, float* Mblk, size_t mblk_stride,
                          const float* tc, const float* tS, float* tD2, size_t tail_stride, LmRecord* rec, int seq);
 void launch_mark_compute(hipStream_t st, RowView r, int* flag);
diff --git a/intrinsic3d_amd/csrc/device/lm_kernels.hip b/intrinsic3d_amd/csrc/device/lm_kernels.hip
--- a/intrinsic3d_amd/csrc/device/lm_kernels.hip
+++ b/intrinsic3d_amd/csrc/device/lm_kernels.hip
@@ -1,5 +1,7 @@
 #include "kernels.hpp"
 #include "frame_math.hpp"
+#include "reduce_device.hpp"
+#include <cstring>
 
 namespace i3d {
 
@@ -7,7 +9,42 @@
     if (rec) __hip_atomic_store(&rec->seq, seq, __ATOMIC_RELEASE, __HIP_MEMORY_SCOPE_SYSTEM);
 }
 
-__global__ void k_lm_init(LmState* lm, const double* __restrict__ cost, const double* __restrict__ ngrad, const double* __restrict__ nfree, double radius0, LmRecord* rec, int seq) {
+constexpr int LM_TEST_PART = 1024;
+__global__ void __launch_bounds__(256) k_lm_tests(int n, size_t seg, int ntail, size_t tail_rel, const float* __restrict__ g, const float* __restrict__ m, float tol, int b2, int b1,
+                                                  double* __restrict__ part) {
+    const int bx = (int)blockIdx.x;
+    const int which = bx < b2 ? 0 : (bx < b2 + b1 ? 1 : (bx < 2 * b2 + b1 ? 2 : 3));
+    const int vb = bx - (which == 0 ? 0 : which == 1 ? b2 : which == 2 ? b2 + b1 : 2 * b2 + b1);
+    const int stride = ((which & 1) ? b1 : b2) * (int)blockDim.x;
+    double s = 0.0;
+    if (!(which & 1)) {
+        for (int i = vb * (int)blockDim.x + (int)threadIdx.x; i < 2 * n; i += stride) {
+            const size_t j = i < n ? (size_t)i : (size_t)(i - n) + seg;
+            s += which == 0 ? ((fabsf(g[j] * m[j]) > tol) ? 1.0 : 0.0) : (double)m[j] * (double)m[j];
+        }
+    } else {
+        for (int i = vb * (int)blockDim.x + (int)threadIdx.x; i < ntail; i += stride) {
+            const size_t j = tail_rel + i;
+            s += which == 1 ? ((fabsf(g[j] * m[j]) > tol) ? 1.0 : 0.0) : (double)m[j] * (double)m[j];
+        }
+    }
+    const double t = block_sum_d(s);
+    if (threadIdx.x == 0) part[(size_t)which * LM_TEST_PART + vb] = t;
+}
+static inline int lm_test_blocks(int n) { int b = (n + 255) / 256; return b < 1 ? 1 : (b > 1024 ? 1024 : b); }
+void launch_lm_tests(hipStream_t st, Seg2 sg, size_t tail_off, int ntail, const float* g, const float* mask, float tol, double* part, int* b2_out, int* b1_out) {
+    const int b2 = lm_test_blocks(2 * sg.n), b1 = lm_test_blocks(ntail);
+    k_lm_tests<<<2 * (b2 + b1), 256, 0, st>>>(sg.n, sg.off1 - sg.off0, ntail, tail_off - sg.off0, g + sg.off0, mask + sg.off0, tol, b2, b1, part);
+    *b2_out = b2; *b1_out = b1;
+}
+
+__global__ void __launch_bounds__(1024) k_lm_init(LmState* lm, const double* __restrict__ cost, const double* ngrad, const double* nfree, double radius0, LmRecord* rec, int seq,
+                                                  const double* __restrict__ test_part, int b2, int b1, double* ngrad_dst, double* nfree_dst) {
+    if (test_part) {
+        reduce_partials_wg(test_part, b2, 1, ngrad_dst, 1); reduce_partials_wg(test_part + LM_TEST_PART, b1, 1, ngrad_dst, 0);
+        reduce_partials_wg(test_part + 2 * LM_TEST_PART, b2, 1, nfree_dst, 1); reduce_partials_wg(test_part + 3 * LM_TEST_PART, b1, 1, nfree_dst, 0);
+    }
+    if (threadIdx.x != 0) return;
     LmState s;
     s.cost = *cost; s.radius = radius0; s.decrease_factor = 2.0; s.ngrad = *ngrad; s.nfree = *nfree;
     s.inv_radius = (float)(1.0 / radius0); s.pad0 = 0;
@@ -22,8 +59,8 @@
 }
 __global__ void k_set_double(double* dst, double v) { *dst = v; }
 void launch_set_double(hipStream_t st, double* dst, double v) { k_set_double<<<1, 1, 0, st>>>(dst, v); }
-void launch_lm_init(hipStream_t st, LmState* lm, const double* cost, const double* ngrad, const double* nfree, double radius0, LmRecord* rec, int seq) {
-    k_lm_init<<<1, 1, 0, st>>>(lm, cost, ngrad, nfree, radius0, rec, seq);
+void launch_lm_init(hipStream_t st, LmState* lm, const double* cost, double* ngrad, double* nfree, double radius0, LmRecord* rec, int seq, const double* test_part, int b2, int b1) {
+    k_lm_init<<<1, test_part ? 1024 : 1, 0, st>>>(lm, cost, ngrad, nfree, radius0, rec, seq, test_part, b2, b1, ngrad, nfree);
 }
 
 static __device__ inline bool spd_invert_dev(int n, const double* m, double* inv) {
@@ -135,8 +172,11 @@
     if (K > 0) k_cand_frames<<<(K + 63) / 64, 64, 0, st>>>(K, xc, base, out, lm);
 }
 
-__global__ void k_lm_decide(LmState* lm, const PcgState* __restrict__ ps, const double* __restrict__ norms2, const double* __restrict__ cand_cost_p, int attempt , int lm_steps,
-                            LmRecord* rec, int seq, int lad_next, int debug_invalid) {
+__global__ void __launch_bounds__(1024) k_lm_decide(LmState* lm, const PcgState* __restrict__ ps, const double* norms2, const double* cand_cost_p, int attempt , int lm_steps,
+                                                    LmRecord* rec, int seq, int lad_next, int debug_invalid, DecideSums red) {
+    if (red.n_cost > 0) reduce_partials_wg(red.cost_partials, red.n_cost, 1, red.cost_dst, 1);
+    if (red.n_norm > 0) reduce_partials_wg(red.norm_partials, red.n_norm, 2, red.norms_dst, 1);
+    if (threadIdx.x != 0) return;
     if (lm->done) return;
     const int pcg_it = ps->done == 2 ? ps->it + 1 : ps->it;
     const double xbr = ps->xbr, d2xx = ps->d2xx;
@@ -186,8 +226,13 @@
         }
     }
 }
-void launch_lm_decide(hipStream_t st, LmState* lm, const PcgState* ps, const double* norms2, const double* cand_cost, int attempt, int lm_steps, LmRecord* rec, int seq, int lad_next, int debug_invalid) {
-    k_lm_decide<<<1, 1, 0, st>>>(lm, ps, norms2, cand_cost, attempt, lm_steps, rec, seq, lad_next, debug_invalid);
-}
-
-}
+void launch_lm_decide(hipStream_t st, LmState* lm, const PcgState* ps, const double* norms2, const double* cand_cost, int attempt, int lm_steps, LmRecord* rec, int seq, int lad_next, int debug_invalid,
+                      const DecideSums* sums) {
+    DecideSums red; std::memset(&red, 0, sizeof(red));
+    if (sums) red = *sums;
+    if (!red.cost_partials || !red.cost_dst) red.n_cost = 0;
+    if (!red.norm_partials || !red.norms_dst) red.n_norm = 0;
+    k_lm_decide<<<1, (red.n_cost > 0 || red.n_norm > 0) ? 1024 : 1, 0, st>>>(lm, ps, norms2, cand_cost, attempt, lm_steps, rec, seq, lad_next, debug_invalid, red);
+}
+
+}
diff --git a/intrinsic3d_amd/csrc/device/operator.hip b/intrinsic3d_amd/csrc/device/operator.hip
--- a/intrinsic3d_amd/csrc/device/operator.hip
+++ b/intrinsic3d_amd/csrc/device/operator.hip
@@ -9,18 +9,7 @@
 
 __global__ void __launch_bounds__(1024) k_reduce_partials(const double* __restrict__ partials, int nblk, int ncomp, double* dst, const PcgState* __restrict__ state, int assign) {
     if (state && state->done) return;
-    for (int k = 0; k < ncomp; ++k) {
-        double s = 0.0;
-        for (int i0 = threadIdx.x; i0 < nblk; i0 += 8 * 1024) {
-            double v[8];
-#pragma unroll
-            for (int q = 0; q < 8; ++q) v[q] = partials[(size_t)min(i0 + q * 1024, nblk - 1) * ncomp + k];
-#pragma unroll
-            for (int q = 0; q < 8; ++q) if (i0 + q * 1024 < nblk) s += v[q];
-        }
-        const double t = block_sum_d(s);
-        if (threadIdx.x == 0) dst[k] = assign ? t : dst[k] + t;
-    }
+    reduce_partials_wg(partials, nblk, ncomp, dst, assign);
 }
 void launch_reduce_partials(hipStream_t st, const double* partials, int nblk, int ncomp, double* dst, const PcgState* state, bool assign) {
     if (nblk > 0) k_reduce_partials<<<1, 1024, 0, st>>>(partials, nblk, ncomp, dst, state, assign ? 1 : 0);
@@ -184,7 +173,8 @@
     for (int i = threadIdx.x; i < npose + NCAM; i += EG_THREADS) row[i] = i < npose ? lds[D0 + i] : cam_acc[i - npose];
 }
 
-__global__ void __launch_bounds__(256) k_sum_rows(int mode, int K, const float* __restrict__ part, int nrows, int stride, double* __restrict__ shared, double* __restrict__ blocks) {
+__global__ void __launch_bounds__(256) k_sum_rows(int mode, int K, const float* __restrict__ part, int nrows, int stride, double* __restrict__ shared, double* __restrict__ blocks,
+                                                  double* __restrict__ shared2, double* __restrict__ blocks2) {
     __shared__ double grp[8][33];
     const int col = threadIdx.x & 31, rg = threadIdx.x >> 5;
     const int i = blockIdx.x * 32 + col;
@@ -196,17 +186,19 @@
     if (rg != 0 || i >= ncol) return;
     v = grp[0][col];
     for (int q = 1; q < 8; ++q) v += grp[q][col];
-    if (mode != PASS_COLNORM) { shared[i] = v; return; }
+    auto to_shared = [&](int k) { shared[k] = v; if (shared2) shared2[k] = v; };
+    auto to_blocks = [&](int k) { blocks[k] = v; if (blocks2) blocks2[k] = v; };
+    if (mode != PASS_COLNORM) { to_shared(i); return; }
     if (i < 21 * K) {
-        blocks[i] = v;
+        to_blocks(i);
         const int f = i / 21, o = i - 21 * f;
         const int di = o == 0 ? 0 : o == 6 ? 1 : o == 11 ? 2 : o == 15 ? 3 : o == 18 ? 4 : o == 20 ? 5 : -1;
-        if (di >= 0) shared[6 * f + di] = v;
-    } else { const int c = i - 21 * K; if (c < 9) shared[6 * K + c] = v; else blocks[21 * K + (c - 9)] = v; }
-}
-void launch_sum_rows(hipStream_t st, PassMode mode, int K, const float* part, int nrows, int stride, double* shared, double* blocks) {
+        if (di >= 0) to_shared(6 * f + di);
+    } else { const int c = i - 21 * K; if (c < 9) to_shared(6 * K + c); else to_blocks(21 * K + (c - 9)); }
+}
+void launch_sum_rows(hipStream_t st, PassMode mode, int K, const float* part, int nrows, int stride, double* shared, double* blocks, double* shared2, double* blocks2) {
     const int ncol = mode == PASS_COLNORM ? 21 * K + 34 : 6 * K + 9;
-    k_sum_rows<<<(ncol + 31) / 32, 256, 0, st>>>((int)mode, K, part, nrows, stride, shared, blocks);
+    k_sum_rows<<<(ncol + 31) / 32, 256, 0, st>>>((int)mode, K, part, nrows, stride, shared, blocks, shared2, blocks2);
 }
 
 __global__ void __launch_bounds__(EG_THREADS) k_eg_jtjp(GridView g, RowView r, OptParams p, const float* __restrict__ u, PassBuffers b,
@@ -511,17 +503,17 @@
     if (sg.n > 0) k_mul2<<<vblocks(2 * sg.n), 256, 0, st>>>(sg.n, sg.off1 - sg.off0, a + sg.off0, b + sg.off0, o + sg.off0);
 }
 void launch_scale_from_colnorm(hipStream_t st, int n, const float* c, const float* m, float* S, float* cm) { if (n > 0) k_scale<<<vblocks(n), 256, 0, st>>>(n, c, m, S, cm); }
-void launch_dot2(hipStream_t st, Seg2 sg, const float* a, const float* b, double* out, double* scratch) {
+void launch_dot2(hipStream_t st, Seg2 sg, const float* a, const float* b, double* out, double* scratch, bool assign) {
     if (sg.n <= 0) return;
     const int blocks = vblocks(2 * sg.n) > 1024 ? 1024 : vblocks(2 * sg.n);
     k_dot2<<<blocks, 256, 0, st>>>(sg.n, sg.off1 - sg.off0, a + sg.off0, b + sg.off0, scratch);
-    launch_reduce_partials(st, scratch, blocks, 1, out, nullptr);
-}
-void launch_count_above2(hipStream_t st, Seg2 sg, const float* a, const float* m, float tol, double* out, double* scratch) {
+    launch_reduce_partials(st, scratch, blocks, 1, out, nullptr, assign);
+}
+void launch_count_above2(hipStream_t st, Seg2 sg, const float* a, const float* m, float tol, double* out, double* scratch, bool assign) {
     if (sg.n <= 0) return;
     const int blocks = vblocks(2 * sg.n) > 1024 ? 1024 : vblocks(2 * sg.n);
     k_count_above2<<<blocks, 256, 0, st>>>(sg.n, sg.off1 - sg.off0, a + sg.off0, m + sg.off0, tol, scratch);
-    launch_reduce_partials(st, scratch, blocks, 1, out, nullptr);
+    launch_reduce_partials(st, scratch, blocks, 1, out, nullptr, assign);
 }
 void launch_count_above(hipStream_t st, int n, const float* a, const float* m, float tol, double* out, double* scratch) {
     if (n <= 0) return;
@@ -822,11 +814,12 @@
     }
     block_partial_d(d2, norms2, 2, 0); block_partial_d(x2, norms2, 2, 1);
 }
-void launch_candidate(hipStream_t st, GridView g, RowView r, int K, float sign, const float* step, const float* S, const double* xsh, double* xc_sdf, double* xc_alb,
-                      double* xc_sh, double* norms2, const float* mask, double* scratch, const LmState* lm) {
+int launch_candidate(hipStream_t st, GridView g, RowView r, int K, float sign, const float* step, const float* S, const double* xsh, double* xc_sdf, double* xc_alb,
+                     double* xc_sh, double* norms2, const float* mask, double* scratch, const LmState* lm) {
     int b = vblocks(r.A + 6 * K + 9); if (b > 1024) b = 1024;
     k_candidate<<<b, 256, 0, st>>>(g, r, K, sign, step, S, xsh, xc_sdf, xc_alb, xc_sh, scratch, mask, lm);
-    launch_reduce_partials(st, scratch, b, 2, norms2, nullptr, true);
+    if (norms2) launch_reduce_partials(st, scratch, b, 2, norms2, nullptr, true);
+    return b;
 }
 __global__ void k_accept(GridView g, RowView r, const double* __restrict__ xc_sdf, const double* __restrict__ xc_alb, const LmState* __restrict__ lm) {
     if (lm && !lm->accepted) return;
diff --git a/intrinsic3d_amd/csrc/device/pcg_fused.hip b/intrinsic3d_amd/csrc/device/pcg_fused.hip
--- a/intrinsic3d_amd/csrc/device/pcg_fused.hip
+++ b/intrinsic3d_amd/csrc/device/pcg_fused.hip
@@ -238,7 +238,7 @@
     for (int seg = 0; seg < 2; ++seg) {
         const int i = q + seg * a.chunk4;
         v.cm[seg] = a.cm[i];
-        if (MODE == S3_INIT) v.r[seg] = r[i];
+        if (MODE == S3_INIT) v.r[seg] = a.b[i];
         else {
             v.x[seg] = x[i];
             if (MODE != S3_RESET) v.p[seg] = p[i];
@@ -265,7 +265,21 @@
     __shared__ int done_s;
     if (threadIdx.x == 0) done_s = cur->done;
     __syncthreads();
-    if (done_s) return;
+    if (done_s) {
+        if (MODE == S3_INIT) {
+            const float4 zero = make_float4(0.0f, 0.0f, 0.0f, 0.0f);
+            if (slice_wg) {
+                for (int q = q0; q < a.nq; q += qstride) {
+#pragma unroll
+                    for (int seg = 0; seg < 2; ++seg) { const int i = q + seg * a.chunk4; X[i] = zero; R[i] = a.b[i]; }
+                }
+            } else {
+                const int NS = 6 * a.K + 9, ntw = (int)gridDim.x - a.n_slice_wg;
+                for (int i = ((int)blockIdx.x - a.n_slice_wg) * PF_THREADS + (int)threadIdx.x; i < NS; i += ntw * PF_THREADS) { tx[i] = 0.0f; tr[i] = a.tb[i]; }
+            }
+        }
+        return;
+    }
     const float inv_radius = o.sys >= 0 ? a.lm->lad_inv_radius[o.sys] : a.lm->inv_radius;
     float alpha = 0.0f;
     if (MODE == S3_NORMAL || MODE == S3_XONLY) {
@@ -316,7 +330,7 @@
                 float xv[4], rv[4], svv[4], dv[4], mv[4];
                 { const float4 cv = in.cm[seg]; lm_from_colnorm(cv.x, inv_radius, svv[0], dv[0], mv[0]); lm_from_colnorm(cv.y, inv_radius, svv[1], dv[1], mv[1]);
                   lm_from_colnorm(cv.z, inv_radius, svv[2], dv[2], mv[2]); lm_from_colnorm(cv.w, inv_radius, svv[3], dv[3], mv[3]); }
-                if (MODE == S3_INIT) { const float4 t = in.r[seg]; rv[0] = t.x; rv[1] = t.y; rv[2] = t.z; rv[3] = t.w; }
+                if (MODE == S3_INIT) { const float4 t = in.r[seg]; rv[0] = t.x; rv[1] = t.y; rv[2] = t.z; rv[3] = t.w; R[i] = t; X[i] = make_float4(0.0f, 0.0f, 0.0f, 0.0f); }
                 else {
                     const float4 xo = in.x[seg];
                     xv[0] = xo.x; xv[1] = xo.y; xv[2] = xo.z; xv[3] = xo.w;
@@ -373,7 +387,7 @@
             const int i = col0 + t;
             const bool fixed = i < 6 * K ? a.fix_poses : (i < 6 * K + 4 ? a.fix_intr : a.fix_dist);
             float ri;
-            if (MODE == S3_INIT) ri = tr[i];
+            if (MODE == S3_INIT) { ri = a.tb[i]; tr[i] = ri; tx[i] = 0.0f; }
             else {
                 float xi = tx[i];
                 if (MODE != S3_RESET) { xi += alpha * tp[i]; tx[i] = xi; }
@@ -492,6 +506,24 @@
 }
 void launch_pcg_init_lad(hipStream_t st, PcgState* st2_all, int B, int fixed_iterations, int max_iterations, const LmState* lm) { k_pcg_init_lad<<<1, LADDER_MAX, 0, st>>>(st2_all, B, fixed_iterations, max_iterations, lm); }
 
+__global__ void __launch_bounds__(256) k_u_from_x_lad(int n4, int seg4, size_t tail_rel, int ntail, const float* __restrict__ S, const float* __restrict__ x0, float* __restrict__ u0, LadVec lv) {
+    const size_t vo = (size_t)lv.sysid[blockIdx.y] * lv.vec;
+    const float* const x = x0 + vo; float* const u = u0 + vo;
+    const float4* S4 = reinterpret_cast<const float4*>(S); const float4* x4 = reinterpret_cast<const float4*>(x); float4* u4 = reinterpret_cast<float4*>(u);
+    for (int j = blockIdx.x * blockDim.x + threadIdx.x; j < 2 * n4; j += gridDim.x * blockDim.x) {
+        const int i = j < n4 ? j : j - n4 + seg4;
+        const float4 s = S4[i], v = x4[i];
+        u4[i] = make_float4(s.x * v.x, s.y * v.y, s.z * v.z, s.w * v.w);
+    }
+    if (blockIdx.x == gridDim.x - 1) for (int t = threadIdx.x; t < ntail; t += blockDim.x) u[tail_rel + t] = S[tail_rel + t] * x[tail_rel + t];
+}
+void launch_u_from_x_lad(hipStream_t st, int nsys, Seg2 sg, size_t tail_off, int ntail, const float* S, const float* x0, float* u0, const LadVec& lv) {
+    const int n4 = sg.n >> 2, seg4 = (int)((sg.off1 - sg.off0) >> 2);
+    const size_t o = sg.off0;
+    int blocks = (2 * n4 + 255) / 256; blocks = blocks < 1 ? 1 : (blocks > 2048 ? 2048 : blocks);
+    k_u_from_x_lad<<<dim3(blocks, nsys), 256, 0, st>>>(n4, seg4, tail_off - o, ntail, S + o, x0 + o, u0 + o, lv);
+}
+
 __global__ void k_ext_offsets(int n, const int* __restrict__ ext_e, int A, int* __restrict__ ext_off) {
     const int e = blockIdx.x * blockDim.x + threadIdx.x;
     if (e > A) return;
diff --git a/intrinsic3d_amd/csrc/device/reduce_device.hpp b/intrinsic3d_amd/csrc/device/reduce_device.hpp
--- a/intrinsic3d_amd/csrc/device/reduce_device.hpp
+++ b/intrinsic3d_amd/csrc/device/reduce_device.hpp
@@ -17,5 +17,19 @@
     const double t = block_sum_d(v);
     if (threadIdx.x == 0) partials[(size_t)blockIdx.x * ncomp + comp] = t;
 }
+static __device__ inline void reduce_partials_wg(const double* __restrict__ partials, int nblk, int ncomp, double* dst, int assign) {
+    for (int k = 0; k < ncomp; ++k) {
+        double s = 0.0;
+        for (int i0 = threadIdx.x; i0 < nblk; i0 += 8 * 1024) {
+            double v[8];
+#pragma unroll
+            for (int q = 0; q < 8; ++q) v[q] = partials[(size_t)min(i0 + q * 1024, nblk - 1) * ncomp + k];
+#pragma unroll
+            for (int q = 0; q < 8; ++q) if (i0 + q * 1024 < nblk) s += v[q];
+        }
+        const double t = block_sum_d(s);
+        if (threadIdx.x == 0) dst[k] = assign ? t : dst[k] + t;
+    }
+}
 
 }
diff --git a/intrinsic3d_amd/csrc/host/pcg.cpp b/intrinsic3d_amd/csrc/host/pcg.cpp
--- a/intrinsic3d_amd/csrc/host/pcg.cpp
+++ b/intrinsic3d_amd/csrc/host/pcg.cpp
@@ -28,22 +28,24 @@
     return I3D_OK;
 }
 
-int run_gradcol(i3d_context* c, const OptParams& p, const std::function<int()>& between) {
+int run_gradcol(i3d_context* c, const OptParams& p, const std::function<int(bool)>& between) {
     hipStream_t s = c->stream; GridView g = c->grid_view(); RowView r = c->row_view(); const Layout L = layout_of(c);
     const int stride = (int)gc_part_stride(c->K), col_off = (int)gc_col_off(c->K);
     GradColBuffers gb{c->C.p, c->C2.p, c->treg.p, c->treg2.p, c->gc_part.p, stride, col_off, c->d_partials.p, c->d_scal.p + 16};
-    CTX_HIP(c, hipMemsetAsync(c->d_scal.p + 16, 0, sizeof(double), s));
-    CTX_HIP(c, hipMemsetAsync(c->d_shared.p, 0, sizeof(double) * ((size_t)L.NS + 1), s));
-    CTX_HIP(c, hipMemsetAsync(c->d_blocks.p, 0, sizeof(double) * (21 * (size_t)c->K + 25), s));
     int rows = 0;
     { TimedScope t(c, I3D_K_EG_AUX); rows = launch_eg_gradcol(s, g, r, p, gb);
       if (rows > GC_PART_ROWS) return ctx_fail(c, I3D_ERR_CAPACITY, "run_gradcol: more workgroups than rows of the camera partial buffer");
-      if (rows > 0) launch_sum_rows(s, PASS_COLNORM, c->K, c->gc_part.p + col_off, rows, stride, c->d_shared.p, c->d_blocks.p); }
+      if (rows > 0) launch_sum_rows(s, PASS_COLNORM, c->K, c->gc_part.p + col_off, rows, stride, c->d_shared.p, c->d_blocks.p, c->d_cam_c.p, c->d_cam_H.p); }
+    if (rows <= 0) {
+        CTX_HIP(c, hipMemsetAsync(c->d_scal.p + 16, 0, sizeof(double), s));
+        CTX_HIP(c, hipMemsetAsync(c->d_shared.p, 0, sizeof(double) * ((size_t)L.NS + 1), s));
+        CTX_HIP(c, hipMemsetAsync(c->d_blocks.p, 0, sizeof(double) * (21 * (size_t)c->K + 25), s));
+    }
     { PassBuffers b{c->C2.p, c->treg2.p, c->d_shared.p, c->d_blocks.p, nullptr, 0};
       TimedScope t(c, I3D_K_GATHER); launch_gather(s, PASS_COLNORM, r, b, c->v_c.p); }
     { TimedScope t(c, I3D_K_VECTOR); launch_shared_finalize(s, L.tail_off, c->K, p, c->d_shared.p, c->v_c.p, false, nullptr, nullptr, nullptr, nullptr, nullptr); }
-    { int rc = between(); if (rc) return rc; }
-    CTX_HIP(c, hipMemsetAsync(c->d_shared.p, 0, sizeof(double) * ((size_t)L.NS + 1), s));
+    { int rc = between(rows > 0); if (rc) return rc; }
+    if (rows <= 0) CTX_HIP(c, hipMemsetAsync(c->d_shared.p, 0, sizeof(double) * ((size_t)L.NS + 1), s));
     { TimedScope t(c, I3D_K_EG_AUX); if (rows > 0) launch_sum_rows(s, PASS_GRAD, c->K, c->gc_part.p, rows, stride, c->d_shared.p, c->d_blocks.p); }
     { PassBuffers b{c->C.p, c->treg.p, c->d_shared.p, c->d_blocks.p, nullptr, 0};
       TimedScope t(c, I3D_K_GATHER); launch_gather(s, PASS_GRAD, r, b, c->v_acc.p); }
@@ -53,8 +55,8 @@
 
 int dot_dev(i3d_context* c, const float* a, const float* b, double* slot) {
     const Layout L = layout_of(c);
-    CTX_HIP(c, hipMemsetAsync(slot, 0, sizeof(double), c->stream));
-    { TimedScope t(c, I3D_K_VECTOR); launch_dot2(c->stream, L.own, a, b, slot, c->d_partials.p); }
+    if (L.own.n <= 0) CTX_HIP(c, hipMemsetAsync(slot, 0, sizeof(double), c->stream));
+    { TimedScope t(c, I3D_K_VECTOR); launch_dot2(c->stream, L.own, a, b, slot, c->d_partials.p, true); }
     { int rc = allreduce(c, slot, 1); if (rc) return rc; }
     { TimedScope t(c, I3D_K_VECTOR); launch_dot(c->stream, L.NS, a + L.tail_off, b + L.tail_off, slot, c->d_partials.p); }
     return I3D_OK;
@@ -62,17 +64,17 @@
 
 int count_above_dev(i3d_context* c, const float* a, const float* m, float tol, double* slot) {
     const Layout L = layout_of(c);
-    CTX_HIP(c, hipMemsetAsync(slot, 0, sizeof(double), c->stream));
-    { TimedScope t(c, I3D_K_VECTOR); launch_count_above2(c->stream, L.own, a, m, tol, slot, c->d_partials.p); }
+    if (L.own.n <= 0) CTX_HIP(c, hipMemsetAsync(slot, 0, sizeof(double), c->stream));
+    { TimedScope t(c, I3D_K_VECTOR); launch_count_above2(c->stream, L.own, a, m, tol, slot, c->d_partials.p, true); }
     { int rc = allreduce(c, slot, 1); if (rc) return rc; }
     { TimedScope t(c, I3D_K_VECTOR); launch_count_above(c->stream, L.NS, a + L.tail_off, m + L.tail_off, tol, slot, c->d_partials.p); }
     return I3D_OK;
 }
 
-int eval_cost_launch(i3d_context* c, const OptParams& p, bool candidate, const FrameConst* frames, const double* cam9, const LmState* lm) {
+int eval_cost_launch(i3d_context* c, const OptParams& p, bool candidate, const FrameConst* frames, const double* cam9, const LmState* lm, int* n_partials) {
     GridView g = c->grid_view();
     if (candidate) { g.x_sdf = c->xc_sdf.p; g.x_alb = c->xc_alb.p; }
-    { TimedScope t(c, I3D_K_COST); launch_build(c->stream, g, c->row_view(), p, frames, false, c->d_scal.p + 16, c->d_partials.p, cam9, lm); }
+    { TimedScope t(c, I3D_K_COST); launch_build(c->stream, g, c->row_view(), p, frames, false, c->d_scal.p + 16, c->d_partials.p, cam9, lm, n_partials); }
     return allreduce(c, c->d_scal.p + 16, 1);
 }
 
@@ -219,8 +221,8 @@
     PcgState* const st2 = c->d_pcg2.p;
     const int NSP = (L.NS + 3) & ~3;
     const Partials part = partials_at(c->d_partials.p);
-    { TimedScope t(c, I3D_K_VECTOR); launch_fill(s, (int)L.NP, c->v_x.p, 0.0f); launch_pcg_init3(s, st2, cfg.pcg_fixed_iterations, PCG_MAX_ITERATIONS, c->d_lm.p); }
-    CTX_HIP(c, hipMemcpyAsync(c->v_r.p, c->v_b.p, sizeof(float) * L.NP, hipMemcpyDeviceToDevice, s));
+    { TimedScope t(c, I3D_K_VECTOR); if (c->sharded()) launch_fill(s, (int)L.NP, c->v_x.p, 0.0f); launch_pcg_init3(s, st2, cfg.pcg_fixed_iterations, PCG_MAX_ITERATIONS, c->d_lm.p); }
+    if (c->sharded()) CTX_HIP(c, hipMemcpyAsync(c->v_r.p, c->v_b.p, sizeof(float) * L.NP, hipMemcpyDeviceToDevice, s));
     Step3Args a = step3_args(c, L, p, tp, c->v_x.p, c->v_r.p, c->v_p.p, c->v_z.p, c->v_qacc.p, tp.qh, part, c->cam_part.p, c->Minv_blocks.p, c->v_D2.p + to, wg_cap);
     a.sharded = sh ? 1 : 0; a.lad_sys = -1;
     int n_step = 0;
@@ -310,8 +312,8 @@
     const int rstride = (int)lad_redop_stride(L.NS);
     double* const redop = sh ? ld.red.p + (size_t)LADDER_MAX * 4 : nullptr;
     { TimedScope t(c, I3D_K_VECTOR);
-      for (int j = 0; j < B; ++j) { CTX_HIP(c, hipMemsetAsync(X0 + (size_t)j * lv.vec, 0, sizeof(float) * L.NP, s));
-                                    CTX_HIP(c, hipMemcpyAsync(R0 + (size_t)j * lv.vec, c->v_b.p, sizeof(float) * L.NP, hipMemcpyDeviceToDevice, s)); }
+      for (int j = 0; j < B && c->sharded(); ++j) { CTX_HIP(c, hipMemsetAsync(X0 + (size_t)j * lv.vec, 0, sizeof(float) * L.NP, s));
+                                                    CTX_HIP(c, hipMemcpyAsync(R0 + (size_t)j * lv.vec, c->v_b.p, sizeof(float) * L.NP, hipMemcpyDeviceToDevice, s)); }
       launch_pcg_init_lad(s, st2, B, cfg.pcg_fixed_iterations, PCG_MAX_ITERATIONS, c->d_lm.p); }
     Step3Args a = step3_args(c, L, p, tp, X0, R0, P0, Z0, Q0, ld.qh.p, part0, ld.cam.p, ld.mblk.p, ld.tail.p, 0);
     a.sharded = 0; a.lad_sys = 0; a.redop = redop; a.redop_stride = rstride;
@@ -376,7 +378,7 @@
         if (it % PCG_RESET_PERIOD != 0) { TimedScope t(c, I3D_K_VECTOR); n_step = launch_pcg_step3_lad(s, 1, nl, a, lv); }
         else {
             { TimedScope t(c, I3D_K_VECTOR); launch_pcg_step3_lad(s, 2, nl, a, lv);
-              for (int j : live) launch_u_from_x(c, L, X0 + (size_t)j * lv.vec, U0 + (size_t)j * lv.vec); }
+              launch_u_from_x_lad(s, nl, own, to, L.NS, c->v_S.p, X0, U0, lv); }
             { const int n = rows_apply(it & 1, false); if (n < 0) return ctx_fail(c, I3D_ERR_STATE, "pcg_solve_ladder: the multi-system operator pass could not be launched"); a.n_cam = n; }
             { TimedScope t(c, I3D_K_VECTOR); n_step = launch_pcg_step3_lad(s, 3, nl, a, lv); }
         }
diff --git a/intrinsic3d_amd/csrc/host/solver.cpp b/intrinsic3d_amd/csrc/host/solver.cpp
--- a/intrinsic3d_amd/csrc/host/solver.cpp
+++ b/intrinsic3d_amd/csrc/host/solver.cpp
@@ -83,9 +83,11 @@
     CTX_HIP(c, hipMemcpyAsync(c->xc_sdf.p, c->x_sdf.p, sizeof(double) * (size_t)N, hipMemcpyDeviceToDevice, s));
     CTX_HIP(c, hipMemcpyAsync(c->xc_alb.p, c->x_alb.p, sizeof(double) * (size_t)N, hipMemcpyDeviceToDevice, s));
     const bool one_stream = one_stream_gradcol(c);
-    auto after_colnorm = [&]() -> int {
-        CTX_HIP(c, hipMemcpyAsync(c->d_cam_c.p, c->d_shared.p, sizeof(double) * (size_t)NS, hipMemcpyDeviceToDevice, s));
-        CTX_HIP(c, hipMemcpyAsync(c->d_cam_H.p, c->d_blocks.p, sizeof(double) * ((size_t)21 * K + 25), hipMemcpyDeviceToDevice, s));
+    auto after_colnorm = [&](bool cam_kept) -> int {
+        if (!cam_kept) {
+            CTX_HIP(c, hipMemcpyAsync(c->d_cam_c.p, c->d_shared.p, sizeof(double) * (size_t)NS, hipMemcpyDeviceToDevice, s));
+            CTX_HIP(c, hipMemcpyAsync(c->d_cam_H.p, c->d_blocks.p, sizeof(double) * ((size_t)21 * K + 25), hipMemcpyDeviceToDevice, s));
+        }
         { int rc2 = allgather(c, c->v_c.p); if (rc2) return rc2; }
         { TimedScope t(c, I3D_K_VECTOR); launch_scale_from_colnorm(s, NP, c->v_c.p, c->v_mask.p, c->v_S.p, c->v_cm.p); }
         return I3D_OK;
@@ -94,14 +96,19 @@
     if (one_stream) { rc = run_gradcol(c, p, after_colnorm); if (rc) return rc; }
     else {
         rc = run_pass(c, PASS_COLNORM, p, nullptr, c->v_c.p); if (rc) return rc;
-        rc = after_colnorm(); if (rc) return rc;
+        rc = after_colnorm(false); if (rc) return rc;
         rc = run_pass(c, PASS_GRAD, p, nullptr, c->v_acc.p); if (rc) return rc;
     }
     { TimedScope t(c, I3D_K_VECTOR); launch_mul(s, NP, c->v_S.p, c->v_acc.p, c->v_b.p); }
     if (!c->sw.cost0) { rc = eval_cost_launch(c, p, false, c->d_frames.p); if (rc) return rc; }
     else if (!one_stream) { TimedScope t(c, I3D_K_VECTOR); launch_set_double(s, c->d_scal.p + 16, c->cost_at_build); }
-    rc = count_above_dev(c, c->v_acc.p, c->v_mask.p, 1e-10f, c->d_scal.p + 8); if (rc) return rc;
-    rc = dot_dev(c, c->v_mask.p, c->v_mask.p, c->d_scal.p + 9); if (rc) return rc;
+    int tests_b2 = 0, tests_b1 = 0;
+    const bool tests_fused = !c->sharded() && L.own.n > 0;
+    if (tests_fused) { TimedScope t(c, I3D_K_VECTOR); launch_lm_tests(s, L.own, L.tail_off, NS, c->v_acc.p, c->v_mask.p, 1e-10f, c->d_partials.p, &tests_b2, &tests_b1); }
+    else {
+        rc = count_above_dev(c, c->v_acc.p, c->v_mask.p, 1e-10f, c->d_scal.p + 8); if (rc) return rc;
+        rc = dot_dev(c, c->v_mask.p, c->v_mask.p, c->d_scal.p + 9); if (rc) return rc;
+    }
     {
         double* xs = c->h_pinned;
         for (int i = 0; i < 6 * K; ++i) xs[i] = c->poses[i];
@@ -111,7 +118,7 @@
     }
     const int seq0 = c->lm_seq; c->lm_seq += LM_REC_SLOTS;
     LmState* const lm = c->d_lm.p;
-    launch_lm_init(s, lm, c->d_scal.p + 16, c->d_scal.p + 8, c->d_scal.p + 9, initial_radius, c->d_lmrec, seq0);
+    launch_lm_init(s, lm, c->d_scal.p + 16, c->d_scal.p + 8, c->d_scal.p + 9, initial_radius, c->d_lmrec, seq0, tests_fused ? c->d_partials.p : nullptr, tests_b2, tests_b1);
 
     int attempts = 0; bool ended = false, accepted = false;
     auto consume = [&](const LmRecord& rec) {
@@ -134,13 +141,20 @@
         if (rec.final_) ended = true;
     };
     auto queue_decision = [&](const float* x, const PcgState* ps, int attempt, int lad_next) -> int {
+        const bool fused = !c->sharded();
+        double* const norm_part = c->d_partials.p + ((size_t)c->Acap / 256 + 8);
+        DecideSums red; std::memset(&red, 0, sizeof(red));
         { TimedScope t(c, I3D_K_VECTOR);
-          launch_candidate(s, g, r, K, -1.0f, x, c->v_S.p, c->d_xshared.p, c->xc_sdf.p, c->xc_alb.p, c->d_xcshared.p, c->d_scal.p + 4, c->v_mask.p, c->d_partials.p, lm);
+          const int n_norm = launch_candidate(s, g, r, K, -1.0f, x, c->v_S.p, c->d_xshared.p, c->xc_sdf.p, c->xc_alb.p, c->d_xcshared.p, fused ? nullptr : c->d_scal.p + 4, c->v_mask.p,
+                                              fused ? norm_part : c->d_partials.p, lm);
+          if (fused) { red.norm_partials = norm_part; red.n_norm = n_norm; red.norms_dst = c->d_scal.p + 4; }
           launch_cand_frames(s, K, c->d_xcshared.p, c->d_frames.p, c->d_frames_cand.p, lm); }
-        const int rc2 = eval_cost_launch(c, p, true, c->d_frames_cand.p, c->d_xcshared.p + 6 * K, lm); if (rc2) return rc2;
+        const int rc2 = eval_cost_launch(c, p, true, c->d_frames_cand.p, c->d_xcshared.p + 6 * K, lm, fused ? &red.n_cost : nullptr); if (rc2) return rc2;
+        if (fused) { red.cost_partials = c->d_partials.p; red.cost_dst = c->d_scal.p + 16; }
         { TimedScope t(c, I3D_K_VECTOR);
           launch_lm_decide(s, lm, ps, c->d_scal.p + 4, c->d_scal.p + 16, attempt, cfg.lm_steps, c->d_lmrec + 1 + attempt, seq0 + 1 + attempt, lad_next,
-                           c->sw.debug_invalid_attempt == attempt ? 1 : 0);
+                           c->sw.debug_invalid_attempt == attempt ? 1 : 0,
+                           &red);
           launch_accept(s, g, r, c->xc_sdf.p, c->xc_alb.p, lm); }
         return I3D_OK;
     };
diff --git a/intrinsic3d_amd/csrc/host/solver_internal.hpp b/intrinsic3d_amd/csrc/host/solver_internal.hpp
--- a/intrinsic3d_amd/csrc/host/solver_internal.hpp
+++ b/intrinsic3d_amd/csrc/host/solver_internal.hpp
@@ -68,10 +68,10 @@
 };
 
 int run_pass(i3d_context* c, PassMode mode, const OptParams& p, const float* u, float* out);
-int run_gradcol(i3d_context* c, const OptParams& p, const std::function<int()>& between);
+int run_gradcol(i3d_context* c, const OptParams& p, const std::function<int(bool)>& between);
 int dot_dev(i3d_context* c, const float* a, const float* b, double* slot);
 int count_above_dev(i3d_context* c, const float* a, const float* m, float tol, double* slot);
-int eval_cost_launch(i3d_context* c, const OptParams& p, bool candidate, const FrameConst* frames, const double* cam9 = nullptr, const LmState* lm = nullptr);
+int eval_cost_launch(i3d_context* c, const OptParams& p, bool candidate, const FrameConst* frames, const double* cam9 = nullptr, const LmState* lm = nullptr, int* n_partials = nullptr);
 int alloc_ladder(i3d_context* c);
 enum { LV_X = 0, LV_R, LV_P, LV_Z, LV_U, LV_Q };
 inline float* lad_vecp(const i3d_context* c, int kind, int sys = 0) { return c->ladder.vec.p + ((size_t)kind * c->op.ladder_max + sys) * c->ladder.strides.vec; }
```

Result: no change. 44.13, median of 6 (+0.6%).
